# oxylusengine/Oxylus

Hardware: AMD Instinct MI355X
Metric: meshlets/s culled (higher is better)
Workload: dtype f32; 1 GPU; configs[2]: 10M meshlets + 4096^2 prior-frame HiZ (13 mips, built from an 8192^2 depth): HiZ build + early/late occlusion cull + per-triangle cull + compaction into the indirect-draw buffers (unordered_output = 1: slots allocated by atomic_add as in the reference, lists compared sorted); meshlets_per_gpu=10000000, mesh_instances=10000, meshlets_per_mesh=1000, tris_per_meshlet=64, verts_per_meshlet=64, index_form=(id << 8) | corner (visbuffer.slang:9-14), inner_reps=48, small_triangle_cull=False, async_triangles=False, unordered_output=1

## Files before the change

include/oxcull_debug.h:

```cpp
#ifndef OXCULL_DEBUG_H
#define OXCULL_DEBUG_H
#include "oxcull.h"
#ifdef __cplusplus
extern "C" {
#endif

oxc_status oxc_stream_read_probe(oxc_ctx* ctx, const void* dptr, uint64_t bytes, void* hip_stream);

enum {
  OXC_K_PREPARE = 0,
  OXC_K_MESHES_SCAN = 1,
  OXC_K_MESHES_EXPAND = 2,
  OXC_K_MESHLETS_TEST = 3,
  OXC_K_MESHLETS_EMIT = 4,
  OXC_K_TRIANGLES_TEST = 5,
  OXC_K_TRIANGLES_EMIT = 6,
  OXC_K_HIZ = 7,
  OXC_K_MESHLETS_TEST_LATE = 8,
  OXC_K_MESHLETS_EMIT_LATE = 9,
  OXC_K_TRIANGLES_TEST_LATE = 10,
  OXC_K_TRIANGLES_EMIT_LATE = 11,
  OXC_K_DRAW_VISBUFFER = 12,
  OXC_K_MESHLET_BOUNDS = 13,
  OXC_K_MULTIVIEW_SETUP = 14,
  OXC_K_VSM_UPDATE = 15,
  OXC_K_COUNT = 16
};
typedef struct oxc_kernel_times {
  double total_ms[16];
  uint32_t launches[16];
  double empty_pair_ms;
} oxc_kernel_times;
oxc_status oxc_profile_begin(oxc_ctx* ctx);
oxc_status oxc_profile_end(oxc_ctx* ctx, oxc_kernel_times* out);

oxc_status oxc_debug_decode_bounds(oxc_ctx* ctx, const void* bounds_dptr, uint32_t n, float* out10_dptr,
                                   void* hip_stream);

oxc_status oxc_debug_project_aabb(oxc_ctx* ctx, const float* mvp16_host, float near_clip, const void* boxes6_dptr, uint32_t n, float* out7_dptr,
                                  void* hip_stream);

oxc_status oxc_debug_read_u32(oxc_ctx* ctx, const void* dptr, uint32_t n, uint32_t* host_out, void* hip_stream);
uint32_t oxc_debug_shared_tests_mode(const oxc_ctx* ctx);
uint32_t oxc_debug_tri_loads_mode(const oxc_ctx* ctx);

enum { OXC_TUNE_ASYNC_MTEST_BLOCKS_PER_CU = 0, OXC_TUNE_ASYNC_TRI_BLOCKS_PER_CU = 1, OXC_TUNE_RASTER_BIG_CAPACITY = 2,
       OXC_TUNE_TRI_BLOCKS_PER_CU = 3 ,
       OXC_TUNE_TRI_LOADS = 7 ,
       OXC_TUNE_MV_EXPAND_ASYNC = 5 ,
       OXC_TUNE_VSM_DRAW_STATS = 8 ,
       OXC_TUNE_VSM_DRAW_CAPACITY = 9 ,
       OXC_TUNE_VSM_RESOLVE_STATS = 10 ,
       OXC_TUNE_CONTACT_SHADOWS_STATS = 11 ,
       OXC_TUNE_AMBIENT_OCCLUSION_STATS = 12  };
oxc_status oxc_debug_set_tuning(oxc_ctx* ctx, uint32_t knob, uint32_t value);

oxc_status oxc_debug_count_occlusion_candidates(oxc_ctx* ctx, void* counters_dptr);

oxc_status oxc_debug_raster_stats(oxc_ctx* ctx, uint32_t* host_out4, void* hip_stream);

oxc_status oxc_debug_vsm_draw_stats(oxc_ctx* ctx, uint32_t* host_out8, void* hip_stream);

oxc_status oxc_debug_vsm_resolve_stats(oxc_ctx* ctx, uint32_t* host_out8, void* hip_stream);

oxc_status oxc_debug_contact_shadows_stats(oxc_ctx* ctx, uint32_t* host_out12, void* hip_stream);

oxc_status oxc_debug_ambient_occlusion_stats(oxc_ctx* ctx, uint32_t* host_out15, void* hip_stream);

#ifdef __cplusplus
}
#endif
#endif
```

oxylus_amd/csrc/oxcull_abi.cpp:

```cpp
#include <hip/hip_runtime.h>

#include <algorithm>
#include <cmath>
#include <cstdio>
#include <cstdlib>
#include <dlfcn.h>
#include <cstring>
#include <new>
#include <string>
#include <vector>

#include "oxcull.h"
#include "oxcull_debug.h"
#include "oxcull_kernels.hpp"
#include "oxcull_types.hpp"

using namespace oxc;

namespace {
constexpr uint32_t kSlots = 8192;
constexpr uint32_t kMaxPackedInstances = 1u << 24;

inline uint32_t cdiv(uint32_t a, uint32_t b) { return (a + b - 1) / b; }
inline uint64_t align_up(uint64_t v, uint64_t a) { return (v + a - 1) / a * a; }
}

struct oxc_ctx {
  int device = 0;
  uint32_t num_cus = 256;
  std::string last_error;
  struct Lane {
    void* arena = nullptr;
    uint64_t arena_bytes = 0;
    uint32_t cap_mesh_instances = 0, cap_meshlets = 0;
    InstCache* cache = nullptr;
    InstCache* cache_alt = nullptr;
    InstCache* view_cache = nullptr;
    uint32_t cap_views = 0;
    uint32_t* mesh_counts = nullptr;
    uint32_t* mesh_offsets = nullptr;
    uint64_t* bits = nullptr;
    uint32_t* m_chunk_counts = nullptr;
    uint32_t* m_supers = nullptr;
    uint32_t* m_tickets = nullptr;
    uint32_t* m_supers_late = nullptr;
    uint32_t* m_tickets_late = nullptr;
    uint64_t* camera_test_bits = nullptr;
    uint2* step_info = nullptr;
    uint64_t* tri_masks = nullptr;
    uint32_t* t_chunk_counts = nullptr;
    uint32_t* t_supers = nullptr;
    uint32_t* t_supers_alt = nullptr;
  };
  Lane lane[kMaxBatch];
  BatchElem* batch_dev = nullptr;
  void* mv_arena = nullptr;
  uint64_t mv_arena_bytes = 0;
  float* bounds_scratch = nullptr;
  uint32_t bounds_scratch_cap = 0;
  void* raster_scratch = nullptr;
  uint32_t raster_capacity = 0;
  uint32_t raster_capacity_request = 0;
  void* raster_rows = nullptr;
  uint32_t raster_rows_cap = 0;
  void* vsm_scratch = nullptr;
  uint64_t vsm_scratch_bytes = 0;
  void* vsm_draw_scratch = nullptr;
  uint64_t vsm_draw_scratch_bytes = 0;
  uint32_t vsm_draw_capacity = 0;
  uint32_t vsm_draw_capacity_request = 0;
  bool vsm_draw_stats = false;
  uint32_t* vsm_resolve_stats = nullptr;
  bool vsm_resolve_stats_on = false;
  uint32_t* contact_shadows_stats = nullptr;
  bool contact_shadows_stats_on = false;
  uint32_t* ambient_occlusion_stats = nullptr;
  bool ambient_occlusion_stats_on = false;
  void* comm = nullptr;
  uint32_t comm_rank = 0, comm_world = 0;
  uint32_t* slots = nullptr;
  uint32_t slot_cursor = 0;
  uint32_t seed_cursor = 0;
  uint32_t* sink = nullptr;
  std::vector<uint32_t> seeded_total = std::vector<uint32_t>(kSlots, 0u);
  hipStream_t last_stream = nullptr;
  bool has_last_stream = false;
  hipEvent_t order_event = nullptr;
  hipStream_t side = nullptr;
  hipEvent_t fork_event = nullptr;
  hipStream_t mv_side = nullptr;
  hipEvent_t mv_fork = nullptr, mv_join = nullptr;
  uint32_t tri_loads = 0;
  uint32_t mv_expand_async = 4;
  struct TriPending {
    hipEvent_t done = nullptr;
    bool valid = false;
    bool late = false;
    const uint32_t* vis = nullptr;
    const void* visible = nullptr;
    unsigned long long capture_id = 0;
  };
  static constexpr uint32_t kTriRing = 4;
  TriPending tri[kTriRing];
  struct SharedTests {
    bool valid = false;
    uint32_t N = 0, n_host = 0, M = 0, flags = 0, mask_bits = 0;
    const void *meshlet_instances = nullptr, *mask = nullptr, *meshes = nullptr, *transforms = nullptr, *mesh_instances = nullptr, *vis = nullptr;
    oxc_cull_camera camera = {};
    uint64_t armed_for_call = ~0ull;
    unsigned long long capture_id = 0;
    uint32_t* late_slot = nullptr;
    uint32_t* late_t_supers = nullptr;
    InstCache* rows = nullptr;
    bool same_inputs(const SharedTests& o) const {
      return N == o.N && n_host == o.n_host && M == o.M && flags == o.flags && mask_bits == o.mask_bits && meshlet_instances == o.meshlet_instances && mask == o.mask && meshes == o.meshes &&
             transforms == o.transforms && mesh_instances == o.mesh_instances && vis == o.vis && std::memcmp(&camera, &o.camera, sizeof camera) == 0;
    }
  };
  SharedTests shared;
  uint32_t last_share_mode = 0;
  uint32_t last_tri_loads = 0;
  uint64_t call_seq = 0;
  uint32_t async_mtest_per_cu = kAsyncMeshletBlocksPerCU, async_tri_per_cu = kAsyncTriangleBlocksPerCU;
  uint32_t tri_blocks_per_cu = kTriangleBlocksPerCU;
  uint32_t* dbg_occlusion = nullptr;
  bool profiling = false;
  struct Rec {
    int id;
    hipEvent_t a, b;
  };
  std::vector<Rec> recs;
};

namespace {

oxc_status fail(oxc_ctx* ctx, oxc_status st, const char* what, hipError_t e = hipSuccess) {
  if (ctx) {
    ctx->last_error = what;
    if (e != hipSuccess) {
      ctx->last_error += ": ";
      ctx->last_error += hipGetErrorString(e);
    }
  }
  return st;
}

#define OXC_ORDER(ctx, stream)                                            \
  do {                                                                    \
    oxc_status _o = order_stream(ctx, static_cast<hipStream_t>(stream)); \
    if (_o != OXC_OK) return _o;                                          \
  } while (0)

#define OXC_HIP(ctx, expr)                                        \
  do {                                                            \
    hipError_t _e = (expr);                                       \
    if (_e != hipSuccess) return fail(ctx, OXC_HIP_ERROR, #expr, _e); \
  } while (0)

bool stream_is_capturing(hipStream_t s);
unsigned long long stream_capture_id(hipStream_t s);

oxc_status order_stream(oxc_ctx* ctx, hipStream_t s) {
  if (ctx->has_last_stream && ctx->last_stream != s && !stream_is_capturing(s) && !stream_is_capturing(ctx->last_stream)) {
    if (!ctx->order_event) OXC_HIP(ctx, hipEventCreateWithFlags(&ctx->order_event, hipEventDisableTiming));
    if (hipEventRecord(ctx->order_event, ctx->last_stream) == hipSuccess)
      OXC_HIP(ctx, hipStreamWaitEvent(s, ctx->order_event, 0));
    else
      (void)hipGetLastError();
  }
  ctx->last_stream = s;
  ctx->has_last_stream = true;
  return OXC_OK;
}

unsigned long long stream_capture_id(hipStream_t s) {
  hipStreamCaptureStatus st = hipStreamCaptureStatusNone;
  unsigned long long id = 0;
  if (hipStreamGetCaptureInfo(s, &st, &id) != hipSuccess) {
    (void)hipGetLastError();
    return 0;
  }
  return st == hipStreamCaptureStatusNone ? 0ull : (id ? id : ~0ull);
}

bool stream_is_capturing(hipStream_t s) {
  hipStreamCaptureStatus st = hipStreamCaptureStatusNone;
  if (hipStreamIsCapturing(s, &st) != hipSuccess) {
    (void)hipGetLastError();
    return false;
  }
  return st != hipStreamCaptureStatusNone;
}

oxc_status ensure_capacity(oxc_ctx* ctx, uint32_t mesh_instances, uint32_t meshlets, uint32_t views = 0, uint32_t lane_index = 0, hipStream_t s = nullptr) {
  oxc_ctx::Lane* L = &ctx->lane[lane_index];
  if (mesh_instances <= L->cap_mesh_instances && meshlets <= L->cap_meshlets && views <= L->cap_views && L->arena) return OXC_OK;
  if (stream_is_capturing(s))
    return fail(ctx, OXC_INVALID_ARG, "scratch memory must grow but the stream is being captured: call oxc_reserve (or one un-captured call of this size) first");
  const uint32_t Vw = std::max(views, L->cap_views);
  uint32_t M = std::max(std::max(mesh_instances, L->cap_mesh_instances), 1u);
  uint32_t N = std::max(std::max(meshlets, L->cap_meshlets), 1u);
  const uint32_t m_chunks = cdiv(N, 64u), t_chunks = cdiv(N, kTriChunk);
  uint64_t off = 0;
  auto carve = [&](uint64_t bytes) {
    uint64_t o = off;
    off = align_up(off + bytes, 256);
    return o;
  };
  const uint64_t o_cache = carve((uint64_t)M * sizeof(InstCache));
  const uint64_t o_cache_alt = carve((uint64_t)M * sizeof(InstCache));
  const uint64_t o_vcache = carve((uint64_t)M * Vw * sizeof(InstCache) + 64);
  const uint64_t o_counts = carve((uint64_t)M * 4);
  const uint64_t o_offsets = carve((uint64_t)M * 4);
  const uint64_t o_bits = carve((uint64_t)cdiv(N, 64) * 8);
  const uint64_t o_mcc = carve((uint64_t)m_chunks * 4);
  const uint64_t o_msup = carve((uint64_t)cdiv(m_chunks, kChunksPerSuper) * 4 * kSuperStride);
  const uint64_t o_mtick = carve((uint64_t)kTicketCounters * 4 * kSuperStride);
  const uint64_t o_msup_late = carve((uint64_t)cdiv(m_chunks, kChunksPerSuper) * 4 * kSuperStride);
  const uint64_t o_mtick_late = carve((uint64_t)kTicketCounters * 4 * kSuperStride);
  const uint64_t o_fb = carve((uint64_t)cdiv(N, 64) * 8);
  const uint64_t o_si = carve((uint64_t)m_chunks * 8);
  const uint64_t o_tm = carve((uint64_t)N * 16);
  const uint64_t o_tcc = carve((uint64_t)t_chunks * 4);
  const uint64_t o_tsup = carve((uint64_t)cdiv(t_chunks, kChunksPerSuper) * 4 * kSuperStride);
  const uint64_t o_tsup_alt = carve((uint64_t)cdiv(t_chunks, kChunksPerSuper) * 4 * kSuperStride);
  OXC_HIP(ctx, hipDeviceSynchronize());
  for (auto& tp : ctx->tri) tp.valid = false;
  if (lane_index == 0) ctx->shared.valid = false;
  if (L->arena) OXC_HIP(ctx, hipFree(L->arena));
  L->arena = nullptr;
  hipError_t e = hipMalloc(&L->arena, off);
  if (e != hipSuccess) {
    L->cap_mesh_instances = L->cap_meshlets = 0;
    return fail(ctx, OXC_OUT_OF_MEMORY, "hipMalloc(scratch arena)", e);
  }
  L->arena_bytes = off;
  char* b = static_cast<char*>(L->arena);
  L->cache = reinterpret_cast<InstCache*>(b + o_cache);
  L->cache_alt = reinterpret_cast<InstCache*>(b + o_cache_alt);
  L->view_cache = reinterpret_cast<InstCache*>(b + o_vcache);
  L->cap_views = Vw;
  L->mesh_counts = reinterpret_cast<uint32_t*>(b + o_counts);
  L->mesh_offsets = reinterpret_cast<uint32_t*>(b + o_offsets);
  L->bits = reinterpret_cast<uint64_t*>(b + o_bits);
  L->m_chunk_counts = reinterpret_cast<uint32_t*>(b + o_mcc);
  L->m_supers = reinterpret_cast<uint32_t*>(b + o_msup);
  L->m_tickets = reinterpret_cast<uint32_t*>(b + o_mtick);
  L->m_supers_late = reinterpret_cast<uint32_t*>(b + o_msup_late);
  L->m_tickets_late = reinterpret_cast<uint32_t*>(b + o_mtick_late);
  L->camera_test_bits = reinterpret_cast<uint64_t*>(b + o_fb);
  L->step_info = reinterpret_cast<uint2*>(b + o_si);
  L->tri_masks = reinterpret_cast<uint64_t*>(b + o_tm);
  L->t_chunk_counts = reinterpret_cast<uint32_t*>(b + o_tcc);
  L->t_supers = reinterpret_cast<uint32_t*>(b + o_tsup);
  L->t_supers_alt = reinterpret_cast<uint32_t*>(b + o_tsup_alt);
  L->cap_mesh_instances = M;
  L->cap_meshlets = N;
  return OXC_OK;
}

uint32_t* next_slot(oxc_ctx* ctx) {
  uint32_t* s = ctx->slots + (size_t)(ctx->slot_cursor % (kSlots / 2)) * SLOT_U32S;
  ctx->slot_cursor++;
  return s;
}
uint32_t* next_seed_slot(oxc_ctx* ctx) {
  uint32_t* s = ctx->slots + (size_t)(kSlots / 2 + ctx->seed_cursor % (kSlots / 2)) * SLOT_U32S;
  ctx->seed_cursor++;
  return s;
}

template <class Pred>
oxc_status wait_triangles(oxc_ctx* ctx, hipStream_t s, Pred needed, bool retire = false) {
  const unsigned long long cid = stream_capture_id(s);
  for (auto& tp : ctx->tri) {
    if (!tp.valid) continue;
    if (tp.capture_id != cid) {
      if (cid == 0 && !(ctx->side && stream_capture_id(ctx->side) == tp.capture_id)) tp.valid = false;
      continue;
    }
    if (!needed(tp)) continue;
    OXC_HIP(ctx, hipStreamWaitEvent(s, tp.done, 0));
    if (retire) tp.valid = false;
  }
  return OXC_OK;
}
oxc_status join_triangles(oxc_ctx* ctx, hipStream_t s) {
  return wait_triangles(ctx, s, [](const oxc_ctx::TriPending&) { return true; }, true);
}
#define OXC_JOIN(ctx, stream)                                               \
  do {                                                                      \
    oxc_status _j = join_triangles(ctx, static_cast<hipStream_t>(stream));  \
    if (_j != OXC_OK) return _j;                                            \
  } while (0)

struct KernelTimer {
  oxc_ctx* ctx;
  hipStream_t s;
  oxc_ctx::Rec r;
  bool on;
  KernelTimer(oxc_ctx* c, int id, hipStream_t st) : ctx(c), s(st), on(c->profiling) {
    if (!on) return;
    r.id = id;
    if (hipEventCreate(&r.a) != hipSuccess || hipEventCreate(&r.b) != hipSuccess) {
      on = false;
      return;
    }
    (void)hipEventRecord(r.a, s);
  }
  ~KernelTimer() {
    if (!on) return;
    (void)hipEventRecord(r.b, s);
    ctx->recs.push_back(r);
  }
};

bool image_ok(const oxc_image& im) { return im.dptr && im.width && im.height && im.levels >= 1 && im.levels <= 13; }

}

struct CallInfo {
  uint32_t stages, M, N, views;
  bool do_meshes, do_meshlets, do_tris, occl, late;
};

static oxc_status check_call(oxc_ctx* ctx, const oxc_prepared_frame* f, const oxc_cull_geometry_context* c, CallInfo& ci) {
  if (!f || !c || c->struct_size != sizeof(oxc_cull_geometry_context)) return fail(ctx, OXC_INVALID_ARG, "cull_geometry: bad frame/context struct");
  const uint32_t stages = c->stages ? c->stages : (uint32_t)OXC_STAGE_ALL;
  const uint32_t M = f->mesh_instance_count, N = f->max_meshlet_instance_count;
  const bool do_meshes = c->init_cull_meshes && (stages & OXC_STAGE_MESHES);
  const bool do_meshlets = (stages & OXC_STAGE_MESHLETS) != 0;
  const bool do_tris = (stages & OXC_STAGE_TRIANGLES) != 0;
  if (c->cull_camera.mesh_instance_count != M) return fail(ctx, OXC_INVALID_ARG, "cull_geometry: cull_camera.mesh_instance_count != frame.mesh_instance_count");
  if (M && (!f->meshes_buffer.dptr || !f->transforms_world_buffer.dptr || !f->mesh_instances_buffer.dptr))
    return fail(ctx, OXC_INVALID_ARG, "cull_geometry: meshes/transforms/mesh_instances buffer missing");
  if (f->mesh_instances_buffer.bytes < (uint64_t)M * sizeof(GpuMeshInstance)) return fail(ctx, OXC_INVALID_ARG, "cull_geometry: mesh_instances_buffer too small");
  if (N && (!f->meshlet_instances_buffer.dptr || f->meshlet_instances_buffer.bytes < (uint64_t)N * 8))
    return fail(ctx, OXC_INVALID_ARG, "cull_geometry: meshlet_instances_buffer missing or < 8*N bytes");
  if (do_meshlets && N && (!f->visible_meshlet_instances_indices_buffer.dptr || f->visible_meshlet_instances_indices_buffer.bytes < (uint64_t)N * 4))
    return fail(ctx, OXC_INVALID_ARG, "cull_geometry: visible_meshlet_instances_indices_buffer missing or < 4*N bytes");
  if (do_tris && N) {
    if (c->wide_triangle_index > 2u) return fail(ctx, OXC_INVALID_ARG, "cull_geometry: wide_triangle_index must be 0, 1 or 2");
    const uint64_t tris_per_meshlet = c->wide_triangle_index ? 128u : 64u, index_bytes = c->wide_triangle_index == 2u ? 8u : 4u;
    if (!f->reordered_indices_buffer.dptr || f->reordered_indices_buffer.bytes < (uint64_t)N * tris_per_meshlet * 3 * index_bytes)
      return fail(ctx, OXC_INVALID_ARG, "cull_geometry: reordered_indices_buffer missing or < N*64*3*4 bytes (N*128*3*4 with wide_triangle_index = 1, N*128*3*8 with 2)");
    if (c->wide_triangle_index != 2u && N > (c->wide_triangle_index ? kMaxPackedInstances / 2 : kMaxPackedInstances))
      return fail(ctx, OXC_INVALID_ARG, "cull_geometry: too many meshlet instances for the packed index (2^24, visbuffer.slang:9-14; 2^23 with wide_triangle_index = 1; pairs, wide_triangle_index = 2, have no limit)");
  }
  const bool occl = (c->cull_flags & OXC_CULL_TEST_OCCLUSION) != 0;
  const bool late = (c->cull_flags & OXC_CULL_LATE_PASS) != 0;
  if (c->use_hiz && do_meshlets) {
    if (!image_ok(c->hiz_attachment)) return fail(ctx, OXC_INVALID_ARG, "cull_geometry: use_hiz without a hiz_attachment");
    if (occl && N && (!f->meshlet_instance_visibility_mask_buffer.dptr || f->meshlet_instance_visibility_mask_buffer.bytes < (uint64_t)cdiv(N, 32u) * 4u))
      return fail(ctx, OXC_INVALID_ARG, "cull_geometry: visibility mask buffer missing or < ceil(N/32)*4 bytes");
  }
  if (c->small_triangle_cull > 1u) return fail(ctx, OXC_INVALID_ARG, "cull_geometry: small_triangle_cull must be 0 or 1");
  if (c->share_pass_tests > 1u || c->unordered_output > 1u) return fail(ctx, OXC_INVALID_ARG, "cull_geometry: share_pass_tests must be 0 or 1, unordered_output 0 or 1");
  if (c->implicit_meshlet_instances > 1u || c->_reserved1 != 0u) return fail(ctx, OXC_INVALID_ARG, "cull_geometry: implicit_meshlet_instances must be 0 or 1, _reserved1 0");
  if (c->meshlet_instance_runs_buffer.dptr && c->meshlet_instance_runs_buffer.bytes < (uint64_t)M * 8u)
    return fail(ctx, OXC_INVALID_ARG, "cull_geometry: meshlet_instance_runs_buffer < 8 bytes per mesh instance");
  if (c->implicit_meshlet_instances && (!c->meshlet_instance_runs_buffer.dptr || do_tris || !do_meshes))
    return fail(ctx, OXC_INVALID_ARG, "cull_geometry: implicit_meshlet_instances needs meshlet_instance_runs_buffer, cull_meshes in the call and no triangle stage");
  const uint32_t views = c->use_hpb ? c->vsm_clipmap_count : 0u;
  if (c->use_hpb && do_meshlets) {
    if (c->use_hiz) return fail(ctx, OXC_INVALID_ARG, "cull_geometry: use_hiz and use_hpb are exclusive (CullGeometry.cpp:129,199)");
    if (views == 0 || views > 16) return fail(ctx, OXC_INVALID_ARG, "cull_geometry: vsm_clipmap_count must be 1..16");
    if (!c->vsm_clipmaps_buffer.dptr || c->vsm_clipmaps_buffer.bytes < (uint64_t)views * sizeof(oxc_virtual_clipmap) || !c->vsm_clipmap_dirty_flags_buffer.dptr ||
        c->vsm_clipmap_dirty_flags_buffer.bytes < (uint64_t)views * 4u)
      return fail(ctx, OXC_INVALID_ARG, "cull_geometry: use_hpb needs vsm_clipmaps_buffer (76 B per clipmap) / vsm_clipmap_dirty_flags_buffer (4 B per clipmap)");
    const oxc_image_array_u8& h = c->hpb_attachment;
    if (!h.dptr || !h.width || !h.height || h.layers < views || h.levels < 1 || h.levels > 13)
      return fail(ctx, OXC_INVALID_ARG, "cull_geometry: use_hpb without a valid hpb_attachment (layers >= clipmaps, 1..13 levels)");
    for (uint32_t k = 0; k < h.levels; k++) {
      const uint64_t mw = std::max(1u, h.width >> k), mh = std::max(1u, h.height >> k);
      if (h.level_offset[k] + (uint64_t)h.layers * mw * mh > 0xFFFFFFFFull)
        return fail(ctx, OXC_INVALID_ARG, "cull_geometry: hpb_attachment larger than 4 GiB (the reference's is 64 x 64 pages x 10 clipmaps, Shadowmaps.cpp:84-98)");
    }
  }
  if (!c->init_cull_meshes && (!c->visibility_buffer.dptr || !c->cull_meshlets_cmd_buffer.dptr))
    return fail(ctx, OXC_INVALID_ARG, "cull_geometry: init_cull_meshes=false needs the visibility/cull_meshlets_cmd buffers of the sequence");


  ci.stages = stages;
  ci.M = M;
  ci.N = N;
  ci.views = views;
  ci.do_meshes = do_meshes;
  ci.do_meshlets = do_meshlets;
  ci.do_tris = do_tris;
  ci.occl = occl;
  ci.late = late;
  return OXC_OK;
}

extern "C" {

uint32_t oxc_abi_version(void) { return OXC_ABI_VERSION; }

oxc_status oxc_create(int device, oxc_ctx** out) {
  if (!out) return OXC_INVALID_ARG;
  *out = nullptr;
  oxc_ctx* ctx = new (std::nothrow) oxc_ctx();
  if (!ctx) return OXC_OUT_OF_MEMORY;
  ctx->device = device;
  hipError_t e = hipSetDevice(device);
  if (e != hipSuccess) {
    delete ctx;
    return OXC_HIP_ERROR;
  }
  hipDeviceProp_t prop;
  if (hipGetDeviceProperties(&prop, device) == hipSuccess && prop.multiProcessorCount > 0)
    ctx->num_cus = (uint32_t)prop.multiProcessorCount;
  e = hipMalloc(reinterpret_cast<void**>(&ctx->slots), (size_t)kSlots * SLOT_U32S * 4 + 256);
  if (e != hipSuccess) {
    delete ctx;
    return OXC_OUT_OF_MEMORY;
  }
  (void)hipMemset(ctx->slots, 0, (size_t)kSlots * SLOT_U32S * 4 + 256);
  (void)hipDeviceSynchronize();
  ctx->sink = ctx->slots + (size_t)kSlots * SLOT_U32S;
  *out = ctx;
  return OXC_OK;
}

void oxc_destroy(oxc_ctx* ctx) {
  if (!ctx) return;
  (void)hipSetDevice(ctx->device);
  (void)hipDeviceSynchronize();
  for (auto& ln : ctx->lane)
    if (ln.arena) (void)hipFree(ln.arena);
  if (ctx->batch_dev) (void)hipFree(ctx->batch_dev);
  if (ctx->mv_arena) (void)hipFree(ctx->mv_arena);
  if (ctx->bounds_scratch) (void)hipFree(ctx->bounds_scratch);
  if (ctx->raster_scratch) (void)hipFree(ctx->raster_scratch);
  if (ctx->raster_rows) (void)hipFree(ctx->raster_rows);
  if (ctx->vsm_scratch) (void)hipFree(ctx->vsm_scratch);
  if (ctx->vsm_draw_scratch) (void)hipFree(ctx->vsm_draw_scratch);
  if (ctx->vsm_resolve_stats) (void)hipFree(ctx->vsm_resolve_stats);
  if (ctx->contact_shadows_stats) (void)hipFree(ctx->contact_shadows_stats);
  if (ctx->ambient_occlusion_stats) (void)hipFree(ctx->ambient_occlusion_stats);
  if (ctx->comm) (void)oxc_comm_destroy(ctx);
  if (ctx->slots) (void)hipFree(ctx->slots);
  if (ctx->order_event) (void)hipEventDestroy(ctx->order_event);
  if (ctx->fork_event) (void)hipEventDestroy(ctx->fork_event);
  if (ctx->mv_side) (void)hipStreamDestroy(ctx->mv_side);
  if (ctx->mv_fork) (void)hipEventDestroy(ctx->mv_fork);
  if (ctx->mv_join) (void)hipEventDestroy(ctx->mv_join);
  for (auto& tp : ctx->tri)
    if (tp.done) (void)hipEventDestroy(tp.done);
  if (ctx->side) (void)hipStreamDestroy(ctx->side);
  delete ctx;
}

const char* oxc_last_error(const oxc_ctx* ctx) { return ctx ? ctx->last_error.c_str() : "null context"; }

oxc_status oxc_reserve(oxc_ctx* ctx, uint32_t max_mesh_instances, uint32_t max_meshlet_instances) {
  if (!ctx) return OXC_INVALID_ARG;
  OXC_HIP(ctx, hipSetDevice(ctx->device));
  return ensure_capacity(ctx, max_mesh_instances, max_meshlet_instances);
}

oxc_status oxc_generate_hiz(oxc_ctx* ctx, const oxc_main_geometry_context* c, void* hip_stream) {
  if (!ctx) return OXC_INVALID_ARG;
  if (!c || c->struct_size != sizeof(oxc_main_geometry_context)) return fail(ctx, OXC_INVALID_ARG, "generate_hiz: bad context struct");
  const oxc_image& d = c->depth_attachment;
  const oxc_image& h = c->hiz_attachment;
  if (!d.dptr || !d.width || !d.height) return fail(ctx, OXC_INVALID_ARG, "generate_hiz: depth_attachment missing");
  if (!image_ok(h)) return fail(ctx, OXC_INVALID_ARG, "generate_hiz: hiz_attachment missing or levels not in 1..13");
  if (h.width > 4096 || h.height > 4096) return fail(ctx, OXC_INVALID_ARG, "generate_hiz: hiz extent > 4096 (13 mips) unsupported");
  HizArgs a;
  a.depth = reinterpret_cast<const float*>(static_cast<const char*>(d.dptr) + d.level_offset[0]);
  a.hiz = static_cast<float*>(h.dptr);
  a.dw = d.width;
  a.dh = d.height;
  a.w = h.width;
  a.h = h.height;
  a.levels = std::min(h.levels, 13u);
  for (uint32_t k = 0; k < 13; k++) {
    if (k < a.levels && (h.level_offset[k] & 3u)) return fail(ctx, OXC_INVALID_ARG, "generate_hiz: level offset not 4-byte aligned");
    a.level_off[k] = k < a.levels ? (uint32_t)(h.level_offset[k] / 4) : 0u;
  }
  const bool tiled = (a.w % 64 == 0) && (a.h % 64 == 0);
  if (!tiled && (uint64_t)a.w * a.h > 4096) return fail(ctx, OXC_INVALID_ARG, "generate_hiz: extent must be a multiple of 64 or <= 4096 texels");
  if (tiled && (h.level_offset[0] & 15u)) return fail(ctx, OXC_INVALID_ARG, "generate_hiz: mip 0 must be 16-byte aligned");
  OXC_HIP(ctx, hipSetDevice(ctx->device));
  OXC_ORDER(ctx, hip_stream);
  {
    KernelTimer t(ctx, OXC_K_HIZ, static_cast<hipStream_t>(hip_stream));
    launch_hiz(a, ctx->num_cus, static_cast<hipStream_t>(hip_stream));
  }
  OXC_HIP(ctx, hipGetLastError());
  return OXC_OK;
}

oxc_status oxc_seed_meshlet_instances(oxc_ctx* ctx, oxc_cull_geometry_context* c, uint32_t total, void* hip_stream) {
  if (!ctx) return OXC_INVALID_ARG;
  if (!c || c->struct_size != sizeof(oxc_cull_geometry_context)) return fail(ctx, OXC_INVALID_ARG, "seed: bad context struct");
  OXC_HIP(ctx, hipSetDevice(ctx->device));
  OXC_ORDER(ctx, hip_stream);
  uint32_t* slot = next_seed_slot(ctx);
  ctx->shared.valid = false;
  ctx->seeded_total[(slot - ctx->slots) / SLOT_U32S] = total;
  launch_seed_slot(slot, total, static_cast<hipStream_t>(hip_stream));
  OXC_HIP(ctx, hipGetLastError());
  c->visibility_buffer = {slot + SLOT_VIS, 12};
  c->cull_meshlets_cmd_buffer = {slot + SLOT_MESHLETS_CMD, 12};
  return OXC_OK;
}

oxc_status oxc_cull_geometry(oxc_ctx* ctx, const oxc_prepared_frame* f, oxc_cull_geometry_context* c, void* hip_stream) {
  if (!ctx) return OXC_INVALID_ARG;
  CallInfo ci;
  {
    oxc_status vst = check_call(ctx, f, c, ci);
    if (vst != OXC_OK) return vst;
  }
  const uint32_t M = ci.M, N = ci.N, views = ci.views;
  const bool do_meshes = ci.do_meshes, do_meshlets = ci.do_meshlets, do_tris = ci.do_tris, occl = ci.occl, late = ci.late;
  if (c->implicit_meshlet_instances)
    return fail(ctx, OXC_INVALID_ARG, "cull_geometry: implicit_meshlet_instances is accepted by oxc_cull_geometry_batch's multi-view path only (this call's meshlet test reads the records)");
  OXC_HIP(ctx, hipSetDevice(ctx->device));
  hipStream_t s = static_cast<hipStream_t>(hip_stream);
  oxc_status st = ensure_capacity(ctx, M, N, views, 0, s);
  if (st != OXC_OK) return st;
  OXC_ORDER(ctx, hip_stream);
  ctx->last_share_mode = 0;
  ctx->last_tri_loads = 0;
  if (do_meshes) ctx->shared.valid = false;

  oxc_ctx::Lane& L0 = ctx->lane[0];
  const uint64_t call_no = ctx->call_seq++;
  const bool async = c->async_triangles != 0 && do_tris;
  InstCache* cache = (call_no & 1u) ? L0.cache_alt : L0.cache;
  uint32_t* t_supers = (call_no & 1u) ? L0.t_supers_alt : L0.t_supers;
  oxc_ctx::TriPending& my_tri = ctx->tri[call_no % oxc_ctx::kTriRing];
  my_tri.valid = false;
  if (!async || do_meshes) {
    OXC_JOIN(ctx, s);
  } else if (call_no >= 2) {
    const oxc_ctx::TriPending* old = &ctx->tri[(call_no - 2) % oxc_ctx::kTriRing];
    oxc_status wst = wait_triangles(ctx, s, [old](const oxc_ctx::TriPending& tp) { return &tp == old; });
    if (wst != OXC_OK) return wst;
  }
  const uint32_t mtest_limit = (c->async_triangles && ctx->async_mtest_per_cu) ? ctx->async_mtest_per_cu * ctx->num_cus : 0u;
  const uint32_t tri_grid_cap = (async && ctx->async_tri_per_cu) ? ctx->async_tri_per_cu * ctx->num_cus : ctx->num_cus * ctx->tri_blocks_per_cu;
  const void* const visible_buf = f->visible_meshlet_instances_indices_buffer.dptr;
  auto wait_for_visible_list = [&](const uint32_t* vis_now) -> oxc_status {
    return wait_triangles(ctx, s, [&](const oxc_ctx::TriPending& tp) { return !(late && !tp.late && tp.vis == vis_now && tp.visible == visible_buf); });
  };

  uint32_t* slot = c->init_cull_meshes ? next_slot(ctx) : nullptr;
  uint32_t* vis;
  uint32_t* meshlets_cmd;
  uint32_t n_host = 0;
  if (!c->init_cull_meshes) {
    const uint32_t* v = static_cast<const uint32_t*>(c->visibility_buffer.dptr);
    if (v >= ctx->slots && v < ctx->slots + (size_t)kSlots * SLOT_U32S && ((v - ctx->slots) % SLOT_U32S) == SLOT_VIS)
      n_host = ctx->seeded_total[(v - ctx->slots) / SLOT_U32S];
    if (n_host > N) n_host = 0;
  }
  if (c->init_cull_meshes) {
    vis = slot + SLOT_VIS;
    meshlets_cmd = slot + SLOT_MESHLETS_CMD;
    c->visibility_buffer = {vis, 12};
    c->cull_meshlets_cmd_buffer = {meshlets_cmd, 12};
  } else {
    vis = static_cast<uint32_t*>(c->visibility_buffer.dptr);
    meshlets_cmd = static_cast<uint32_t*>(c->cull_meshlets_cmd_buffer.dptr);
  }
  uint32_t share_mode = 0;
  bool armed_late = false, arm_late = false;
  uint32_t* m_supers = L0.m_supers;
  uint32_t* m_tickets = L0.m_tickets;
  const uint32_t mask_bits = (uint32_t)std::min<uint64_t>(f->meshlet_instance_visibility_mask_buffer.bytes / 4u * 32u, 0xFFFFFFFEull);
  const bool unord_tris = c->unordered_output != 0u && do_tris;
  const bool unord_meshlets = do_meshlets && !c->use_hpb && !c->use_hiz && c->unordered_output != 0u;
  if (c->use_hiz && occl && c->share_pass_tests && do_meshlets && !unord_meshlets) {
    oxc_ctx::SharedTests now;
    now.N = N;
    now.n_host = n_host;
    now.M = M;
    now.flags = c->cull_flags & ~(uint32_t)OXC_CULL_LATE_PASS;
    now.mask_bits = mask_bits;
    now.meshlet_instances = f->meshlet_instances_buffer.dptr;
    now.mask = f->meshlet_instance_visibility_mask_buffer.dptr;
    now.meshes = f->meshes_buffer.dptr;
    now.transforms = f->transforms_world_buffer.dptr;
    now.mesh_instances = f->mesh_instances_buffer.dptr;
    now.vis = vis;
    now.camera = c->cull_camera;
    if (!late) {
      share_mode = 1u;
      arm_late = c->async_triangles == 0;
      now.valid = true;
      if (arm_late) {
        now.armed_for_call = call_no + 1;
        now.capture_id = stream_capture_id(s);
        now.late_slot = next_slot(ctx);
        now.late_t_supers = (call_no & 1u) ? L0.t_supers : L0.t_supers_alt;
        now.rows = cache;
      }
      ctx->shared = now;
    } else if (!do_meshes && !c->init_cull_meshes && ctx->shared.valid && ctx->shared.same_inputs(now)) {
      share_mode = 2u;
      if (ctx->shared.armed_for_call == call_no && c->async_triangles == 0 && ctx->shared.capture_id == stream_capture_id(s)) {
        armed_late = true;
        slot = ctx->shared.late_slot;
        t_supers = ctx->shared.late_t_supers;
        cache = ctx->shared.rows;
        m_supers = L0.m_supers_late;
        m_tickets = L0.m_tickets_late;
      }
      ctx->shared.valid = false;
    }
  } else if (c->use_hiz && do_meshlets && !late) {
    ctx->shared.valid = false;
  }
  if (!armed_late && ctx->shared.armed_for_call <= call_no) ctx->shared.armed_for_call = ~0ull;
  if (!slot) slot = next_slot(ctx);
  uint32_t* tri_cmd = slot + SLOT_TRI_CMD;
  uint32_t* draw_cmd = slot + SLOT_DRAW_CMD;
  c->cull_triangles_cmd_buffer = {tri_cmd, 12};
  c->draw_geometry_cmd_buffer = {draw_cmd, 20};

  const uint32_t max_grid = ctx->num_cus * 8;
  const uint32_t m_chunks = cdiv(std::max(N, 1u), kMeshletChunk), t_chunks = cdiv(std::max(N, 1u), kTriChunk);

  PrepareArgs pa;
  pa.meshes = static_cast<const GpuMesh*>(f->meshes_buffer.dptr);
  pa.transforms = static_cast<const float*>(f->transforms_world_buffer.dptr);
  pa.mesh_instances = static_cast<GpuMeshInstance*>(f->mesh_instances_buffer.dptr);
  pa.cache = cache;
  pa.mesh_counts = ctx->lane[0].mesh_counts;
  pa.slot = slot;
  pa.vis = vis;
  pa.meshlets_cmd = meshlets_cmd;
  pa.supers_meshlets = m_supers;
  pa.supers_tris = t_supers;
  pa.tickets = m_tickets;
  pa.slot_late = arm_late ? ctx->shared.late_slot : nullptr;
  pa.supers_meshlets_late = arm_late ? L0.m_supers_late : nullptr;
  pa.supers_tris_late = arm_late ? ctx->shared.late_t_supers : nullptr;
  pa.tickets_late = arm_late ? L0.m_tickets_late : nullptr;
  pa.n_supers_meshlets = cdiv(cdiv(std::max(N, 1u), 64u), kChunksPerSuper);
  pa.n_supers_tris = cdiv(t_chunks, kChunksPerSuper);
  pa.mesh_instance_count = M;
  pa.cull_flags = c->cull_flags;
  pa.do_cull_meshes = do_meshes ? 1u : 0u;
  pa.init_vis = c->init_cull_meshes ? 1u : 0u;
  pa.seed_total = 0;
  pa.cam = c->cull_camera;
  pa.clipmaps = static_cast<const oxc_virtual_clipmap*>(c->vsm_clipmaps_buffer.dptr);
  pa.view_cache = ctx->lane[0].view_cache;
  const uint32_t prep_threads = std::max(std::max(M * 8u, pa.n_supers_tris), 1u);
  if (!armed_late) {
    KernelTimer t(ctx, OXC_K_PREPARE, s);
    launch_prepare(pa, std::min(cdiv(prep_threads, 256), max_grid), (c->use_hpb && do_meshlets) ? views : 0u, s);
  }
  if (do_meshes) {
    {
      KernelTimer t(ctx, OXC_K_MESHES_SCAN, s);
      launch_scan_mesh_counts(ctx->lane[0].mesh_counts, ctx->lane[0].mesh_offsets, M, N, vis, meshlets_cmd, s);
    }
    KernelTimer t(ctx, OXC_K_MESHES_EXPAND, s);
    launch_expand(ctx->lane[0].mesh_counts, ctx->lane[0].mesh_offsets, M, N, f->meshlet_instances_buffer.dptr, std::max(std::min(cdiv(M, 4), max_grid), 1u), s);
  }

  if (do_meshlets && c->use_hpb) {
    HpbTestArgs ha;
    std::memset(&ha, 0, sizeof ha);
    ha.cache = cache;
    ha.view_cache = ctx->lane[0].view_cache;
    ha.meshlet_instances = static_cast<const GpuMeshletInstance*>(f->meshlet_instances_buffer.dptr);
    ha.vis = vis;
    ha.bits = ctx->lane[0].bits;
    ha.chunk_counts = ctx->lane[0].m_chunk_counts;
    ha.supers = ctx->lane[0].m_supers;
    ha.tickets = ctx->lane[0].m_tickets;
    ha.clipmaps = static_cast<const oxc_virtual_clipmap*>(c->vsm_clipmaps_buffer.dptr);
    ha.dirty = static_cast<const uint32_t*>(c->vsm_clipmap_dirty_flags_buffer.dptr);
    ha.clipmap_count = views;
    ha.mesh_instance_count = M;
    ha.n_cap = N;
    const oxc_image_array_u8& h = c->hpb_attachment;
    ha.hpb_data = static_cast<const uint8_t*>(h.dptr);
    ha.hpb_w = h.width;
    ha.hpb_h = h.height;
    ha.hpb_layers = h.layers;
    ha.hpb_levels = h.levels;
    for (uint32_t k = 0; k < h.levels && k < 13; k++) ha.hpb_level_off[k] = (uint32_t)h.level_offset[k];
    std::memcpy(ha.light_dir, c->cull_camera.position, 12);
    {
      KernelTimer t(ctx, OXC_K_MESHLETS_TEST, s);
      launch_hpb_test(ha, std::min(m_chunks, max_grid), s);
    }
    MeshletEmitArgs ea;
    ea.n_host = 0;
    ea.n_cap = N;
    ea.count_meshlets = 64u * kGroupsPerWave;
    ea.bits = ctx->lane[0].bits;
    ea.chunk_counts = ctx->lane[0].m_chunk_counts;
    ea.supers = ctx->lane[0].m_supers;
    ea.vis = vis;
    ea.tri_cmd = tri_cmd;
    ea.out = static_cast<uint32_t*>(f->visible_meshlet_instances_indices_buffer.dptr);
    {
      oxc_status wst = wait_for_visible_list(vis);
      if (wst != OXC_OK) return wst;
    }
    KernelTimer t(ctx, OXC_K_MESHLETS_EMIT, s);
    launch_meshlets_emit(ea, false, false, std::min(cdiv(std::max(N, 1u), kMeshletSpan), max_grid), s);
  } else if (do_meshlets) {
    MeshletTestArgs ta;
    std::memset(&ta, 0, sizeof ta);
    ta.n_host = n_host;
    ta.n_cap = N;
    ta.mask_bits = mask_bits;
    ta.cache = cache;
    ta.meshlet_instances = static_cast<const GpuMeshletInstance*>(f->meshlet_instances_buffer.dptr);
    ta.vis = vis;
    ta.mask = static_cast<uint32_t*>(f->meshlet_instance_visibility_mask_buffer.dptr);
    ta.bits = ctx->lane[0].bits;
    ta.chunk_counts = ctx->lane[0].m_chunk_counts;
    ta.supers = m_supers;
    if (c->use_hiz) {
      ta.tickets = m_tickets;
      const oxc_image& h = c->hiz_attachment;
      ta.hiz_data = static_cast<const float*>(h.dptr);
      ta.hiz_w = h.width;
      ta.hiz_h = h.height;
      ta.hiz_levels = h.levels;
      for (uint32_t k = 0; k < h.levels && k < 13; k++) ta.hiz_level_off[k] = (uint32_t)(h.level_offset[k] / 4);
      uint32_t first = h.levels, used = 0;
      while (first > 0) {
        const uint64_t n = (uint64_t)std::max(1u, h.width >> (first - 1)) * std::max(1u, h.height >> (first - 1));
        if (used + n > kHizLdsTexels) break;
        used += (uint32_t)n;
        first--;
      }
      ta.hiz_lds_first = first;
      uint32_t off = 0;
      for (uint32_t k = first; k < h.levels; k++) {
        ta.hiz_lds_off[k] = off;
        off += std::max(1u, h.width >> k) * std::max(1u, h.height >> k);
      }
    }
    ta.near_clip = c->cull_camera.near_clip;
    std::memcpy(ta.cam_pos, c->cull_camera.position, 12);
    ta.dbg_occlusion = ctx->dbg_occlusion;
    if (share_mode) {
      ta.share = share_mode;
      ta.camera_test_bits = ctx->lane[0].camera_test_bits;
      ta.step_info = ctx->lane[0].step_info;
    }
    ctx->last_share_mode = armed_late ? 3u : ta.share;
    if (unord_meshlets) {
      ta.out = static_cast<uint32_t*>(f->visible_meshlet_instances_indices_buffer.dptr);
      ta.count_a = tri_cmd;
      oxc_status wst = wait_for_visible_list(vis);
      if (wst != OXC_OK) return wst;
      KernelTimer t(ctx, late ? OXC_K_MESHLETS_TEST_LATE : OXC_K_MESHLETS_TEST, s);
      launch_meshlets_test(ta, c->use_hiz != 0, occl, late, std::min(m_chunks, max_grid), ctx->num_cus, mtest_limit, s);
    } else {
      {
        KernelTimer t(ctx, late ? OXC_K_MESHLETS_TEST_LATE : OXC_K_MESHLETS_TEST, s);
        launch_meshlets_test(ta, c->use_hiz != 0, occl, late, std::min(m_chunks, max_grid), ctx->num_cus, mtest_limit, s);
      }
      MeshletEmitArgs ea;
      ea.n_host = n_host;
      ea.n_cap = N;
      ea.count_meshlets = c->use_hiz ? 64u * kHizGroupsPerWave : 64u * kPlainGroups;
      ea.bits = ctx->lane[0].bits;
      ea.chunk_counts = ctx->lane[0].m_chunk_counts;
      ea.supers = m_supers;
      ea.vis = vis;
      ea.tri_cmd = tri_cmd;
      ea.out = static_cast<uint32_t*>(f->visible_meshlet_instances_indices_buffer.dptr);
      {
        oxc_status wst = wait_for_visible_list(vis);
        if (wst != OXC_OK) return wst;
      }
      KernelTimer t(ctx, late ? OXC_K_MESHLETS_EMIT_LATE : OXC_K_MESHLETS_EMIT, s);
      launch_meshlets_emit(ea, c->use_hiz != 0, late, std::min(cdiv(std::max(N, 1u), kMeshletSpan), max_grid), s);
    }
  }

  if (do_tris) {
    hipStream_t ts = s;
    if (async) {
      if (!ctx->side) OXC_HIP(ctx, hipStreamCreateWithFlags(&ctx->side, hipStreamNonBlocking));
      if (!ctx->fork_event) OXC_HIP(ctx, hipEventCreateWithFlags(&ctx->fork_event, hipEventDisableTiming));
      OXC_HIP(ctx, hipEventRecord(ctx->fork_event, s));
      OXC_HIP(ctx, hipStreamWaitEvent(ctx->side, ctx->fork_event, 0));
      ts = ctx->side;
    }
    TriTestArgs tt;
    tt.cache = cache;
    tt.meshlet_instances = static_cast<const GpuMeshletInstance*>(f->meshlet_instances_buffer.dptr);
    tt.visible = static_cast<const uint32_t*>(f->visible_meshlet_instances_indices_buffer.dptr);
    tt.vis = vis;
    tt.tri_cmd = tri_cmd;
    tt.tri_masks = ctx->lane[0].tri_masks;
    tt.chunk_counts = ctx->lane[0].t_chunk_counts;
    tt.supers = t_supers;
    tt.resolution[0] = c->cull_camera.resolution[0];
    tt.resolution[1] = c->cull_camera.resolution[1];
    tt.draw_cmd = draw_cmd;
    tt.out = static_cast<uint32_t*>(f->reordered_indices_buffer.dptr);
    tt.ticket = t_supers;
    tt.ticket_count = std::max(pa.n_supers_tris, 1u);
    const uint64_t mesh_records = f->meshes_buffer.bytes / sizeof(GpuMesh);
    const bool cached_loads = ctx->tri_loads == 2u || (ctx->tri_loads == 0u && mesh_records != 0u && (uint64_t)M >= 4u * mesh_records);
    ctx->last_tri_loads = (cached_loads && !c->small_triangle_cull) ? 2u : 1u;
    if (unord_tris) {
      KernelTimer t(ctx, late ? OXC_K_TRIANGLES_TEST_LATE : OXC_K_TRIANGLES_TEST, ts);
      const bool default_cap = !(async && ctx->async_tri_per_cu) && ctx->tri_blocks_per_cu == kTriangleBlocksPerCU;
      launch_tris_fused(tt, late, c->wide_triangle_index, c->small_triangle_cull != 0, cached_loads, std::min(cdiv(std::max(N, 1u), kFusedTriSpan), tri_grid_cap),
                        default_cap ? ctx->num_cus : 0u, ts);
    } else {
    {
      KernelTimer t(ctx, late ? OXC_K_TRIANGLES_TEST_LATE : OXC_K_TRIANGLES_TEST, ts);
      const bool default_cap = !(async && ctx->async_tri_per_cu) && ctx->tri_blocks_per_cu == kTriangleBlocksPerCU;
      launch_tris_test(tt, late, c->wide_triangle_index != 0, c->small_triangle_cull != 0, cached_loads, std::min(t_chunks, (default_cap && !c->wide_triangle_index) ? ctx->num_cus * 32u : tri_grid_cap), ts);
    }
    TriEmitArgs te;
    te.tri_masks = ctx->lane[0].tri_masks;
    te.visible = tt.visible;
    te.vis = vis;
    te.tri_cmd = tri_cmd;
    te.chunk_counts = ctx->lane[0].t_chunk_counts;
    te.supers = t_supers;
    te.draw_cmd = draw_cmd;
    te.out = static_cast<uint32_t*>(f->reordered_indices_buffer.dptr);
    {
      KernelTimer t(ctx, late ? OXC_K_TRIANGLES_EMIT_LATE : OXC_K_TRIANGLES_EMIT, ts);
      launch_tris_emit(te, late, c->wide_triangle_index, std::min(cdiv(std::max(N, 1u), kTriSpan), tri_grid_cap), ts);
    }
    }
    if (async) {
      if (!my_tri.done) OXC_HIP(ctx, hipEventCreateWithFlags(&my_tri.done, hipEventDisableTiming));
      OXC_HIP(ctx, hipEventRecord(my_tri.done, ts));
      my_tri.valid = true;
      my_tri.late = late;
      my_tri.vis = vis;
      my_tri.visible = visible_buf;
      my_tri.capture_id = stream_capture_id(s);
    }
  }
  OXC_HIP(ctx, hipGetLastError());
  return OXC_OK;
}

oxc_status oxc_join_triangles(oxc_ctx* ctx, void* hip_stream) {
  if (!ctx) return OXC_INVALID_ARG;
  OXC_HIP(ctx, hipSetDevice(ctx->device));
  OXC_ORDER(ctx, hip_stream);
  return join_triangles(ctx, static_cast<hipStream_t>(hip_stream));
}

oxc_status oxc_cull_geometry_batch(oxc_ctx* ctx, uint32_t count, const oxc_prepared_frame* frames, oxc_cull_geometry_context* contexts,
                                   void* hip_stream) {
  if (!ctx) return OXC_INVALID_ARG;
  if (count == 0) return OXC_OK;
  if (!frames || !contexts) return fail(ctx, OXC_INVALID_ARG, "cull_geometry_batch: null frames/contexts");
  CallInfo ci[kMaxBatch];
  bool fusable = count > 1 && count <= kMaxBatch;
  for (uint32_t e = 0; fusable && e < count; e++) {
    oxc_status vst = check_call(ctx, &frames[e], &contexts[e], ci[e]);
    if (vst != OXC_OK) return vst;
    const oxc_cull_geometry_context& c = contexts[e];
    fusable = !c.use_hiz && !c.use_hpb && !c.wide_triangle_index && !c.small_triangle_cull && !ci[e].late && ci[e].stages == ci[0].stages && ci[e].do_meshes == ci[0].do_meshes &&
              (c.init_cull_meshes != 0) == (contexts[0].init_cull_meshes != 0);
  }
  if (!fusable) {
    for (uint32_t e = 0; e < count; e++) {
      oxc_status st = oxc_cull_geometry(ctx, &frames[e], &contexts[e], hip_stream);
      if (st != OXC_OK) return st;
    }
    return OXC_OK;
  }
  bool multiview = ci[0].do_meshes && ci[0].do_meshlets && ci[0].M > 0;
  bool same_pos = true;
  for (uint32_t e = 1; multiview && e < count; e++) {
    multiview = ci[e].M == ci[0].M && frames[e].meshes_buffer.dptr == frames[0].meshes_buffer.dptr &&
                frames[e].transforms_world_buffer.dptr == frames[0].transforms_world_buffer.dptr && contexts[e].cull_flags == contexts[0].cull_flags;
    same_pos = same_pos && std::memcmp(contexts[e].cull_camera.position, contexts[0].cull_camera.position, 12) == 0;
  }
  uint32_t n_implicit = 0;
  for (uint32_t e = 0; e < count; e++) n_implicit += contexts[e].implicit_meshlet_instances ? 1u : 0u;
  if (n_implicit && (n_implicit != count || !multiview || ci[0].do_tris))
    return fail(ctx, OXC_INVALID_ARG, "cull_geometry_batch: implicit_meshlet_instances must be set on every element of a multi-view batch (same scene, cull_meshes in every element, no triangle stage)");
  const bool implicit_lists = n_implicit != 0;
  OXC_HIP(ctx, hipSetDevice(ctx->device));
  ctx->shared.valid = false;
  for (uint32_t e = 0; e < count; e++) {
    oxc_status st = ensure_capacity(ctx, ci[e].M, ci[e].N, 0, e, static_cast<hipStream_t>(hip_stream));
    if (st != OXC_OK) return st;
  }
  OXC_ORDER(ctx, hip_stream);
  OXC_JOIN(ctx, hip_stream);
  if (!ctx->batch_dev) {
    if (stream_is_capturing(static_cast<hipStream_t>(hip_stream)))
      return fail(ctx, OXC_INVALID_ARG, "cull_geometry_batch: the first batched call allocates its argument block; make one un-captured call first");
    hipError_t e = hipMalloc(reinterpret_cast<void**>(&ctx->batch_dev), sizeof(BatchElem) * kMaxBatch);
    if (e != hipSuccess) return fail(ctx, OXC_OUT_OF_MEMORY, "hipMalloc(batch argument block)", e);
    OXC_HIP(ctx, hipMemset(ctx->batch_dev, 0, sizeof(BatchElem) * kMaxBatch));
    OXC_HIP(ctx, hipDeviceSynchronize());
  }
// ... 1067 lines not shown
Rccl* rccl() {
  static Rccl r;
  static bool tried = false;
  if (!tried) {
    tried = true;
    r.lib = dlopen("librccl.so", RTLD_NOW | RTLD_GLOBAL);
    if (!r.lib) r.lib = dlopen("librccl.so.1", RTLD_NOW | RTLD_GLOBAL);
    if (r.lib) {
      r.GetUniqueId = reinterpret_cast<decltype(r.GetUniqueId)>(dlsym(r.lib, "ncclGetUniqueId"));
      r.CommInitRank = reinterpret_cast<decltype(r.CommInitRank)>(dlsym(r.lib, "ncclCommInitRank"));
      r.CommDestroy = reinterpret_cast<decltype(r.CommDestroy)>(dlsym(r.lib, "ncclCommDestroy"));
      r.AllGather = reinterpret_cast<decltype(r.AllGather)>(dlsym(r.lib, "ncclAllGather"));
      r.Broadcast = reinterpret_cast<decltype(r.Broadcast)>(dlsym(r.lib, "ncclBroadcast"));
      r.GetErrorString = reinterpret_cast<decltype(r.GetErrorString)>(dlsym(r.lib, "ncclGetErrorString"));
    }
  }
  return (r.lib && r.GetUniqueId && r.CommInitRank && r.CommDestroy && r.AllGather && r.Broadcast) ? &r : nullptr;
}
oxc_status rccl_fail(oxc_ctx* ctx, const char* what, int code) {
  static thread_local std::string msg;
  Rccl* r = rccl();
  msg = std::string(what) + ": " + ((r && r->GetErrorString) ? r->GetErrorString(code) : "RCCL error");
  ctx->last_error = msg;
  return OXC_RCCL_ERROR;
}
constexpr int kNcclUint8 = 1, kNcclUint32 = 3;
}

oxc_status oxc_comm_unique_id(oxc_ctx* ctx, void* id128_host_out) {
  if (!ctx) return OXC_INVALID_ARG;
  if (!id128_host_out) return fail(ctx, OXC_INVALID_ARG, "comm_unique_id: null output");
  Rccl* r = rccl();
  if (!r) return fail(ctx, OXC_RCCL_ERROR, "librccl.so could not be loaded (needed only for the multi-GPU exchange)");
  OXC_HIP(ctx, hipSetDevice(ctx->device));
  int rc = r->GetUniqueId(id128_host_out);
  return rc == 0 ? OXC_OK : rccl_fail(ctx, "ncclGetUniqueId", rc);
}

oxc_status oxc_comm_init(oxc_ctx* ctx, const void* id128_host, uint32_t rank, uint32_t world) {
  if (!ctx) return OXC_INVALID_ARG;
  if (!id128_host || world == 0 || rank >= world) return fail(ctx, OXC_INVALID_ARG, "comm_init: null id or rank >= world");
  if (ctx->comm) return fail(ctx, OXC_INVALID_ARG, "comm_init: the context already has a communicator");
  Rccl* r = rccl();
  if (!r) return fail(ctx, OXC_RCCL_ERROR, "librccl.so could not be loaded (needed only for the multi-GPU exchange)");
  OXC_HIP(ctx, hipSetDevice(ctx->device));
  OxcRcclId id;
  std::memcpy(&id, id128_host, sizeof id);
  int rc = r->CommInitRank(&ctx->comm, (int)world, id, (int)rank);
  if (rc != 0) {
    ctx->comm = nullptr;
    return rccl_fail(ctx, "ncclCommInitRank", rc);
  }
  ctx->comm_rank = rank;
  ctx->comm_world = world;
  return OXC_OK;
}

oxc_status oxc_comm_destroy(oxc_ctx* ctx) {
  if (!ctx) return OXC_INVALID_ARG;
  if (ctx->comm) {
    Rccl* r = rccl();
    if (r) (void)r->CommDestroy(ctx->comm);
    ctx->comm = nullptr;
    ctx->comm_world = 0;
  }
  return OXC_OK;
}

oxc_status oxc_pack_counters(oxc_ctx* ctx, const oxc_cull_geometry_context* c, void* counts4_dptr, void* hip_stream) {
  if (!ctx) return OXC_INVALID_ARG;
  if (!c || c->struct_size != sizeof(oxc_cull_geometry_context) || !counts4_dptr) return fail(ctx, OXC_INVALID_ARG, "pack_counters: bad context struct or null output");
  if (!c->visibility_buffer.dptr || !c->cull_triangles_cmd_buffer.dptr || !c->draw_geometry_cmd_buffer.dptr)
    return fail(ctx, OXC_INVALID_ARG, "pack_counters: the context has no counter buffers yet (no cull_geometry call has filled them in)");
  OXC_HIP(ctx, hipSetDevice(ctx->device));
  OXC_ORDER(ctx, hip_stream);
  OXC_JOIN(ctx, hip_stream);
  launch_pack_counters(static_cast<const uint32_t*>(c->visibility_buffer.dptr), static_cast<const uint32_t*>(c->cull_triangles_cmd_buffer.dptr),
                       static_cast<const uint32_t*>(c->draw_geometry_cmd_buffer.dptr), static_cast<uint32_t*>(counts4_dptr), static_cast<hipStream_t>(hip_stream));
  OXC_HIP(ctx, hipGetLastError());
  return OXC_OK;
}

oxc_status oxc_pack_counters_batch(oxc_ctx* ctx, uint32_t count, const oxc_cull_geometry_context* cs, void* counts4_dptr, void* hip_stream) {
  if (!ctx) return OXC_INVALID_ARG;
  if (!cs || !counts4_dptr || count == 0 || count > kMaxBatch) return fail(ctx, OXC_INVALID_ARG, "pack_counters_batch: 1..16 contexts and an output buffer");
  PackBlob b;
  std::memset(&b, 0, sizeof b);
  b.count = count;
  for (uint32_t e = 0; e < count; e++) {
    if (cs[e].struct_size != sizeof(oxc_cull_geometry_context)) return fail(ctx, OXC_INVALID_ARG, "pack_counters_batch: bad context struct");
    if (!cs[e].visibility_buffer.dptr || !cs[e].cull_triangles_cmd_buffer.dptr || !cs[e].draw_geometry_cmd_buffer.dptr)
      return fail(ctx, OXC_INVALID_ARG, "pack_counters_batch: a context has no counter buffers yet (no cull_geometry call has filled them in)");
    b.vis[e] = static_cast<const uint32_t*>(cs[e].visibility_buffer.dptr);
    b.tri_cmd[e] = static_cast<const uint32_t*>(cs[e].cull_triangles_cmd_buffer.dptr);
    b.draw_cmd[e] = static_cast<const uint32_t*>(cs[e].draw_geometry_cmd_buffer.dptr);
  }
  OXC_HIP(ctx, hipSetDevice(ctx->device));
  OXC_ORDER(ctx, hip_stream);
  OXC_JOIN(ctx, hip_stream);
  launch_pack_counters_batch(b, static_cast<uint32_t*>(counts4_dptr), static_cast<hipStream_t>(hip_stream));
  OXC_HIP(ctx, hipGetLastError());
  return OXC_OK;
}

oxc_status oxc_exchange_counts(oxc_ctx* ctx, const void* counts4_dptr, void* all_counts_dptr, void* hip_stream) {
  if (!ctx) return OXC_INVALID_ARG;
  if (!ctx->comm) return fail(ctx, OXC_INVALID_ARG, "exchange_counts: oxc_comm_init has not been called");
  if (!counts4_dptr || !all_counts_dptr) return fail(ctx, OXC_INVALID_ARG, "exchange_counts: null buffer");
  OXC_HIP(ctx, hipSetDevice(ctx->device));
  OXC_ORDER(ctx, hip_stream);
  int rc = rccl()->AllGather(counts4_dptr, all_counts_dptr, 4, kNcclUint32, ctx->comm, static_cast<hipStream_t>(hip_stream));
  return rc == 0 ? OXC_OK : rccl_fail(ctx, "ncclAllGather", rc);
}

oxc_status oxc_broadcast_hiz(oxc_ctx* ctx, const oxc_image* hiz, uint64_t total_bytes, uint32_t root, void* hip_stream) {
  if (!ctx) return OXC_INVALID_ARG;
  if (!ctx->comm) return fail(ctx, OXC_INVALID_ARG, "broadcast_hiz: oxc_comm_init has not been called");
  if (!hiz || !hiz->dptr || total_bytes == 0 || root >= ctx->comm_world) return fail(ctx, OXC_INVALID_ARG, "broadcast_hiz: null image, zero size or bad root");
  OXC_HIP(ctx, hipSetDevice(ctx->device));
  OXC_ORDER(ctx, hip_stream);
  int rc = rccl()->Broadcast(hiz->dptr, hiz->dptr, (size_t)total_bytes, kNcclUint8, (int)root, ctx->comm, static_cast<hipStream_t>(hip_stream));
  return rc == 0 ? OXC_OK : rccl_fail(ctx, "ncclBroadcast", rc);
}

oxc_status oxc_broadcast_hiz_levels(oxc_ctx* ctx, const oxc_image* hiz, uint32_t first_level, uint64_t total_bytes, uint32_t root, void* hip_stream) {
  if (!ctx) return OXC_INVALID_ARG;
  if (!ctx->comm) return fail(ctx, OXC_INVALID_ARG, "broadcast_hiz_levels: oxc_comm_init has not been called");
  if (!hiz || !hiz->dptr || first_level >= hiz->levels || hiz->levels > 13 || root >= ctx->comm_world) return fail(ctx, OXC_INVALID_ARG, "broadcast_hiz_levels: null image, bad level or bad root");
  const uint64_t begin = hiz->level_offset[first_level];
  if (total_bytes <= begin) return fail(ctx, OXC_INVALID_ARG, "broadcast_hiz_levels: total_bytes does not reach first_level");
  OXC_HIP(ctx, hipSetDevice(ctx->device));
  OXC_ORDER(ctx, hip_stream);
  char* p = static_cast<char*>(hiz->dptr) + begin;
  int rc = rccl()->Broadcast(p, p, (size_t)(total_bytes - begin), kNcclUint8, (int)root, ctx->comm, static_cast<hipStream_t>(hip_stream));
  return rc == 0 ? OXC_OK : rccl_fail(ctx, "ncclBroadcast", rc);
}

oxc_status oxc_debug_project_aabb(oxc_ctx* ctx, const float* mvp16_host, float near_clip, const void* boxes6_dptr, uint32_t n, float* out7_dptr, void* hip_stream) {
  if (!ctx) return OXC_INVALID_ARG;
  if (!mvp16_host || !boxes6_dptr || !out7_dptr) return fail(ctx, OXC_INVALID_ARG, "debug_project_aabb: null pointer");
  OXC_HIP(ctx, hipSetDevice(ctx->device));
  DebugProjectArgs a;
  std::memcpy(a.mvp, mvp16_host, 64);
  a.near_clip = near_clip;
  a.n = n;
  a.boxes6 = static_cast<const float*>(boxes6_dptr);
  a.out7 = out7_dptr;
  launch_debug_project_aabb(a, static_cast<hipStream_t>(hip_stream));
  OXC_HIP(ctx, hipGetLastError());
  return OXC_OK;
}

uint32_t oxc_debug_shared_tests_mode(const oxc_ctx* ctx) { return ctx ? ctx->last_share_mode : 0u; }
uint32_t oxc_debug_tri_loads_mode(const oxc_ctx* ctx) { return ctx ? ctx->last_tri_loads : 0u; }

oxc_status oxc_debug_set_tuning(oxc_ctx* ctx, uint32_t knob, uint32_t value) {
  if (!ctx) return OXC_INVALID_ARG;
  switch (knob) {
    case OXC_TUNE_ASYNC_MTEST_BLOCKS_PER_CU: ctx->async_mtest_per_cu = value; return OXC_OK;
    case OXC_TUNE_ASYNC_TRI_BLOCKS_PER_CU: ctx->async_tri_per_cu = value; return OXC_OK;
    case OXC_TUNE_TRI_BLOCKS_PER_CU:
      if (value == 0) return fail(ctx, OXC_INVALID_ARG, "set_tuning: the triangle grid needs at least one block per CU");
      ctx->tri_blocks_per_cu = value;
      return OXC_OK;
    case OXC_TUNE_MV_EXPAND_ASYNC: ctx->mv_expand_async = value; return OXC_OK;
    case OXC_TUNE_TRI_LOADS:
      if (value > 2u) return fail(ctx, OXC_INVALID_ARG, "set_tuning: OXC_TUNE_TRI_LOADS is 0 (by the scene), 1 (nt) or 2 (plain)");
      ctx->tri_loads = value;
      return OXC_OK;
    case OXC_TUNE_RASTER_BIG_CAPACITY:
      if (ctx->raster_scratch) return fail(ctx, OXC_INVALID_ARG, "set_tuning: the raster scratch is allocated by the first oxc_draw_visbuffer; set its capacity before");
      ctx->raster_capacity_request = value;
      return OXC_OK;
    case OXC_TUNE_VSM_DRAW_STATS: ctx->vsm_draw_stats = value != 0u; return OXC_OK;
    case OXC_TUNE_VSM_RESOLVE_STATS: ctx->vsm_resolve_stats_on = value != 0u; return OXC_OK;
    case OXC_TUNE_CONTACT_SHADOWS_STATS: ctx->contact_shadows_stats_on = value != 0u; return OXC_OK;
    case OXC_TUNE_AMBIENT_OCCLUSION_STATS: ctx->ambient_occlusion_stats_on = value != 0u; return OXC_OK;
    case OXC_TUNE_VSM_DRAW_CAPACITY:
      if (ctx->vsm_draw_scratch) return fail(ctx, OXC_INVALID_ARG, "set_tuning: the shadow draw's scratch is allocated by the first oxc_draw_physical_pages; set its capacity before");
      ctx->vsm_draw_capacity_request = value;
      return OXC_OK;
    default: return fail(ctx, OXC_INVALID_ARG, "set_tuning: unknown knob");
  }
}

oxc_status oxc_debug_count_occlusion_candidates(oxc_ctx* ctx, void* counters_dptr) {
  if (!ctx) return OXC_INVALID_ARG;
  ctx->dbg_occlusion = static_cast<uint32_t*>(counters_dptr);
  return OXC_OK;
}

oxc_status oxc_debug_read_u32(oxc_ctx* ctx, const void* dptr, uint32_t n, uint32_t* host_out, void* hip_stream) {
  if (!ctx) return OXC_INVALID_ARG;
  if (!dptr || !host_out) return fail(ctx, OXC_INVALID_ARG, "debug_read_u32: null pointer");
  OXC_HIP(ctx, hipSetDevice(ctx->device));
  hipStream_t s = static_cast<hipStream_t>(hip_stream);
  OXC_HIP(ctx, hipMemcpyAsync(host_out, dptr, (size_t)n * 4u, hipMemcpyDeviceToHost, s));
  OXC_HIP(ctx, hipStreamSynchronize(s));
  return OXC_OK;
}

oxc_status oxc_debug_raster_stats(oxc_ctx* ctx, uint32_t* host_out4, void* hip_stream) {
  if (!ctx) return OXC_INVALID_ARG;
  if (!host_out4) return fail(ctx, OXC_INVALID_ARG, "debug_raster_stats: null pointer");
  if (!ctx->raster_scratch) return fail(ctx, OXC_INVALID_ARG, "debug_raster_stats: no oxc_draw_visbuffer call on this context yet");
  OXC_HIP(ctx, hipSetDevice(ctx->device));
  OXC_ORDER(ctx, hip_stream);
  hipStream_t s = static_cast<hipStream_t>(hip_stream);
  std::vector<uint32_t> h(kRasterHeaderBytes / 4);
  OXC_HIP(ctx, hipMemcpyAsync(h.data(), ctx->raster_scratch, kRasterHeaderBytes, hipMemcpyDeviceToHost, s));
  OXC_HIP(ctx, hipStreamSynchronize(s));
  const uint32_t seg_cap = ctx->raster_capacity / kBigSegs;
  uint64_t big = 0;
  uint32_t overflowed = 0;
  for (uint32_t k = 0; k < kBigSegs; k++) {
    const uint32_t c = h[64 + k * kBigSegStride];
    big += c;
    overflowed += c > seg_cap ? 1u : 0u;
  }
  host_out4[0] = (uint32_t)std::min<uint64_t>(big, 0xFFFFFFFFull);
  host_out4[1] = h[0];
  host_out4[2] = h[32];
  host_out4[3] = overflowed;
  return OXC_OK;
}

oxc_status oxc_debug_vsm_draw_stats(oxc_ctx* ctx, uint32_t* host_out8, void* hip_stream) {
  if (!ctx) return OXC_INVALID_ARG;
  if (!host_out8) return fail(ctx, OXC_INVALID_ARG, "debug_vsm_draw_stats: null pointer");
  if (!ctx->vsm_draw_scratch) return fail(ctx, OXC_INVALID_ARG, "debug_vsm_draw_stats: no oxc_draw_physical_pages call on this context yet");
  OXC_HIP(ctx, hipSetDevice(ctx->device));
  OXC_ORDER(ctx, hip_stream);
  hipStream_t s = static_cast<hipStream_t>(hip_stream);
  std::vector<uint32_t> h(kVsmDrawHeaderBytes / 4);
  OXC_HIP(ctx, hipMemcpyAsync(h.data(), ctx->vsm_draw_scratch, kVsmDrawHeaderBytes, hipMemcpyDeviceToHost, s));
  OXC_HIP(ctx, hipStreamSynchronize(s));
  const uint32_t cap = ctx->vsm_draw_capacity;
  auto beyond = [](uint32_t count, uint32_t capacity) { return count > capacity ? count - capacity : 0u; };
  host_out8[0] = h[128];
  host_out8[1] = h[160];
  host_out8[2] = h[32];
  host_out8[3] = beyond(h[32], cap);
  host_out8[4] = h[64];
  host_out8[5] = beyond(h[64], cap * 2u);
  host_out8[6] = h[96];
  host_out8[7] = beyond(h[96], cap);
  return OXC_OK;
}

oxc_status oxc_debug_vsm_resolve_stats(oxc_ctx* ctx, uint32_t* host_out8, void* hip_stream) {
  if (!ctx) return OXC_INVALID_ARG;
  if (!host_out8) return fail(ctx, OXC_INVALID_ARG, "debug_vsm_resolve_stats: null pointer");
  if (!ctx->vsm_resolve_stats) return fail(ctx, OXC_INVALID_ARG, "debug_vsm_resolve_stats: no counting oxc_resolve_shadowmap call on this context yet");
  OXC_HIP(ctx, hipSetDevice(ctx->device));
  OXC_ORDER(ctx, hip_stream);
  hipStream_t s = static_cast<hipStream_t>(hip_stream);
  OXC_HIP(ctx, hipMemcpyAsync(host_out8, ctx->vsm_resolve_stats, 32, hipMemcpyDeviceToHost, s));
  OXC_HIP(ctx, hipStreamSynchronize(s));
  return OXC_OK;
}

oxc_status oxc_debug_contact_shadows_stats(oxc_ctx* ctx, uint32_t* host_out12, void* hip_stream) {
  if (!ctx) return OXC_INVALID_ARG;
  if (!host_out12) return fail(ctx, OXC_INVALID_ARG, "debug_contact_shadows_stats: null pointer");
  if (!ctx->contact_shadows_stats) return fail(ctx, OXC_INVALID_ARG, "debug_contact_shadows_stats: no counting oxc_contact_shadows call on this context yet");
  OXC_HIP(ctx, hipSetDevice(ctx->device));
  OXC_ORDER(ctx, hip_stream);
  hipStream_t s = static_cast<hipStream_t>(hip_stream);
  OXC_HIP(ctx, hipMemcpyAsync(host_out12, ctx->contact_shadows_stats, 48, hipMemcpyDeviceToHost, s));
  OXC_HIP(ctx, hipStreamSynchronize(s));
  return OXC_OK;
}

oxc_status oxc_debug_ambient_occlusion_stats(oxc_ctx* ctx, uint32_t* host_out15, void* hip_stream) {
  if (!ctx) return OXC_INVALID_ARG;
  if (!host_out15) return fail(ctx, OXC_INVALID_ARG, "debug_ambient_occlusion_stats: null pointer");
  if (!ctx->ambient_occlusion_stats) return fail(ctx, OXC_INVALID_ARG, "debug_ambient_occlusion_stats: no counting oxc_generate_ambient_occlusion call on this context yet");
  OXC_HIP(ctx, hipSetDevice(ctx->device));
  OXC_ORDER(ctx, hip_stream);
  hipStream_t s = static_cast<hipStream_t>(hip_stream);
  OXC_HIP(ctx, hipMemcpyAsync(host_out15, ctx->ambient_occlusion_stats, 60, hipMemcpyDeviceToHost, s));
  OXC_HIP(ctx, hipStreamSynchronize(s));
  return OXC_OK;
}

}
```

oxylus_amd/csrc/oxcull_device.hpp:

```cpp
#pragma once
#include <hip/hip_runtime.h>

#include <cstdint>

#pragma clang fp contract(off)

namespace oxc {

#define OXC_DEV __device__ __forceinline__

OXC_DEV float asf(uint32_t u) { return __builtin_bit_cast(float, u); }
OXC_DEV uint32_t asu(float f) { return __builtin_bit_cast(uint32_t, f); }
OXC_DEV int lane_id() { return (int)__builtin_amdgcn_mbcnt_hi(~0u, __builtin_amdgcn_mbcnt_lo(~0u, 0u)); }
OXC_DEV uint32_t readlane_u(uint32_t v, int l) { return (uint32_t)__builtin_amdgcn_readlane((int)v, l); }
OXC_DEV float readlane_f(uint32_t v, int l) { return asf(readlane_u(v, l)); }
OXC_DEV uint32_t readfirst_u(uint32_t v) { return (uint32_t)__builtin_amdgcn_readfirstlane((int)v); }
OXC_DEV float bperm_f(int src_lane, float v) {
  return asf((uint32_t)__builtin_amdgcn_ds_bpermute(src_lane << 2, (int)asu(v)));
}

template <typename T>
OXC_DEV T __attribute__((address_space(1))) * gptr(T* p) {
  return (T __attribute__((address_space(1)))*)p;
}
// ... 84 lines not shown
  }
  float t[6][4];
#pragma unroll
  for (int c = 0; c < 4; c++) {
    t[0][c] = r3[c] + r0[c];
    t[1][c] = r3[c] - r0[c];
    t[2][c] = r3[c] + r1[c];
    t[3][c] = r3[c] - r1[c];
    t[4][c] = r2[c];
    t[5][c] = r3[c] - r2[c];
  }
#pragma unroll
  for (int i = 0; i < 6; i++) {
    float l = len3(t[i][0], t[i][1], t[i][2]);
#pragma unroll
    for (int c = 0; c < 4; c++) pl[i * 4 + c] = t[i][c] / l;
  }
}

OXC_DEV bool test_frustum_planes(const float* pl2, const float* sg2, float cx, float cy, float cz, float ex, float ey, float ez) {
  const f2 hxy = f2{ex, ey} * splat(0.5f);
  const float hz = ez * 0.5f;
  bool inside = true;
#pragma unroll
  for (int p = 0; p < 3; p++) {
    const float* n = pl2 + p * 8;
    const float* sg = sg2 + p * 6;
    const f2 qx = splat(cx) + splat(hxy.x) * f2{sg[0], sg[1]};
    const f2 qy = splat(cy) + splat(hxy.y) * f2{sg[2], sg[3]};
    const f2 qz = splat(cz) + splat(hz) * f2{sg[4], sg[5]};
    const f2 d = (qx * f2{n[0], n[1]} + qy * f2{n[2], n[3]}) + qz * f2{n[4], n[5]};
    inside = inside & !(d.x <= -n[6]) & !(d.y <= -n[7]);
  }
  return inside;
}

OXC_DEV void frustum_plane_dots(const float* pl2, const float* sg2, float cx, float cy, float cz, float ex, float ey, float ez, f2* d ) {
  const f2 hxy = f2{ex, ey} * splat(0.5f);
  const float hz = ez * 0.5f;
#pragma unroll
  for (int p = 0; p < 3; p++) {
    const float* n = pl2 + p * 8;
    const float* sg = sg2 + p * 6;
    const f2 qx = splat(cx) + splat(hxy.x) * f2{sg[0], sg[1]};
    const f2 qy = splat(cy) + splat(hxy.y) * f2{sg[2], sg[3]};
    const f2 qz = splat(cz) + splat(hz) * f2{sg[4], sg[5]};
    d[p] = (qx * f2{n[0], n[1]} + qy * f2{n[2], n[3]}) + qz * f2{n[4], n[5]};
  }
}

OXC_DEV bool frustum_pair_inside(const float* n, const float* sg, float cx, float cy, float cz, float ex, float ey, float ez) {
  const f2 hxy = f2{ex, ey} * splat(0.5f);
  const float hz = ez * 0.5f;
  const f2 qx = splat(cx) + splat(hxy.x) * f2{sg[0], sg[1]};
  const f2 qy = splat(cy) + splat(hxy.y) * f2{sg[2], sg[3]};
  const f2 qz = splat(cz) + splat(hz) * f2{sg[4], sg[5]};
  const f2 d = (qx * f2{n[0], n[1]} + qy * f2{n[2], n[3]}) + qz * f2{n[4], n[5]};
  return !(d.x <= -n[6]) & !(d.y <= -n[7]);
}

OXC_DEV void normal_matrix(const float* w, float* nm) {
  float b[3][3];
#pragma unroll
  for (int j = 0; j < 3; j++)
#pragma unroll
    for (int k = 0; k < 3; k++) b[j][k] = OXC_M(w, k, j);
  const int a1[3] = {1, 2, 0}, a2[3] = {2, 0, 1};
#pragma unroll
  for (int k = 0; k < 3; k++) {
    const float* u = b[a1[k]];
    const float* v = b[a2[k]];
    nm[k * 3 + 0] = u[1] * v[2] - v[1] * u[2];
    nm[k * 3 + 1] = u[2] * v[0] - v[2] * u[0];
    nm[k * 3 + 2] = u[0] * v[1] - v[0] * u[1];
  }
}

struct ConeU {
  float nm[9];
  float w2[3][2];
  float wt2[2];
  float wr2[4];
  float scale_max;
};

OXC_DEV bool cone_visible(const ConeU& u, float camx, float camy, float camz, float cx, float cy, float cz, float ex, float ey, float ez,
                          float ax, float ay, float az, float cutoff) {
  const float* nm = u.nm;
  float nx = (nm[0] * ax + nm[3] * ay) + nm[6] * az;
  float ny = (nm[1] * ax + nm[4] * ay) + nm[7] * az;
  float nz = (nm[2] * ax + nm[5] * ay) + nm[8] * az;
  float l = len3(nx, ny, nz);
  float kx = nx / l, ky = ny / l, kz = nz / l;
  float wx = ((u.w2[0][0] * cx + u.w2[1][0] * cy) + u.w2[2][0] * cz) + u.wt2[0];
  float wy = ((u.w2[0][1] * cx + u.w2[1][1] * cy) + u.w2[2][1] * cz) + u.wt2[1];
  float wz = ((u.wr2[0] * cx + u.wr2[1] * cy) + u.wr2[2] * cz) + u.wr2[3];
  float radius = len3(ex * 0.5f, ey * 0.5f, ez * 0.5f) * u.scale_max;
  float dx = wx - camx, dy = wy - camy, dz = wz - camz;
  bool culled = dot3(dx, dy, dz, kx, ky, kz) >= cutoff * len3(dx, dy, dz) + radius;
  return cutoff >= 1.0f || !culled;
}

constexpr float kConeMargin = 1.6e-5f;
OXC_DEV int cone_visible_fast(const ConeU& u, float camx, float camy, float camz, float cx, float cy, float cz, float ex, float ey, float ez,
                              float ax, float ay, float az, float cutoff) {
  const float* nm = u.nm;
  const f2 nxy = (f2{nm[0], nm[1]} * splat(ax) + f2{nm[3], nm[4]} * splat(ay)) + f2{nm[6], nm[7]} * splat(az);
  const float nz = (nm[2] * ax + nm[5] * ay) + nm[8] * az;
  const f2 wxy = ((f2{u.w2[0][0], u.w2[0][1]} * splat(cx) + f2{u.w2[1][0], u.w2[1][1]} * splat(cy)) + f2{u.w2[2][0], u.w2[2][1]} * splat(cz)) +
                 f2{u.wt2[0], u.wt2[1]};
  const float wz = ((u.wr2[0] * cx + u.wr2[1] * cy) + u.wr2[2] * cz) + u.wr2[3];
  const f2 dxy = wxy - f2{camx, camy};
  const float dz = wz - camz;
  const f2 hxy = f2{ex, ey} * splat(0.5f);
  const float hz = ez * 0.5f;
  const f2 nn = nxy * nxy, dd = dxy * dxy, dn = dxy * nxy, hh = hxy * hxy;
  float inv_l = __builtin_amdgcn_rsqf((nn.x + nn.y) + nz * nz);
  float dlen = __builtin_amdgcn_sqrtf((dd.x + dd.y) + dz * dz);
  float radius = __builtin_amdgcn_sqrtf((hh.x + hh.y) + hz * hz) * u.scale_max;
  float L = ((dn.x + dn.y) + dz * nz) * inv_l;
  float R = cutoff * dlen + radius;
  float T = kConeMargin * (dlen + radius);
  float diff = L - R;
  if (diff > T) return 0;
  if (diff < -T) return 1;
  return 2;
}

struct HizView {
  const float* data;
  uint32_t width, height, levels;
  const float* lds;
  const uint32_t* lds_off;
  uint32_t lds_first;
  float inv_width, inv_height;
};
OXC_DEV float exact_reciprocal_or_zero(uint32_t d) { return (d != 0u && (d & (d - 1u)) == 0u) ? 1.0f / (float)d : 0.0f; }

OXC_DEV uint32_t mip_dim(uint32_t d, uint32_t mip) {
  uint32_t v = d >> mip;
  return v ? v : 1u;
}

OXC_DEV float min0_finite(float x) {
  float r;
  asm("v_min_f32 %0, 0, %1" : "=v"(r) : "v"(x));
  return r;
}
OXC_DEV float max0_finite(float x) {
  float r;
  asm("v_max_f32 %0, 0, %1" : "=v"(r) : "v"(x));
  return r;
}
template <bool TRY_AFFINE = false, bool NEED_Z = true>
OXC_DEV bool project_aabb(const float* mvp, float near_clip, float cx, float cy, float cz, float ex, float ey, float ez, float* out) {
  float SX[4], SY[4], SZ[4], P[8][4];
  float p0x = cx - ex * 0.5f, p0y = cy - ey * 0.5f, p0z = cz - ez * 0.5f;
  if (TRY_AFFINE && asu(OXC_M(mvp, 3, 0)) == 0u && asu(OXC_M(mvp, 3, 1)) == 0u && asu(OXC_M(mvp, 3, 2)) == 0u &&
      asu(OXC_M(mvp, 3, 3)) == 0x3F800000u) {
    float lo[3] = {0.f, 0.f, 0.f}, hi[3] = {0.f, 0.f, 0.f}, P0[3] = {0.f, 0.f, 0.f}, S[3][3] = {{0.f, 0.f, 0.f}, {0.f, 0.f, 0.f}, {0.f, 0.f, 0.f}};
    bool finite = true;
#pragma unroll
    for (int i = 0; i < (NEED_Z ? 3 : 2); i++) {
      S[i][0] = OXC_M(mvp, i, 0) * ex, S[i][1] = OXC_M(mvp, i, 1) * ey, S[i][2] = OXC_M(mvp, i, 2) * ez;
      P0[i] = ((OXC_M(mvp, i, 0) * p0x + OXC_M(mvp, i, 1) * p0y) + OXC_M(mvp, i, 2) * p0z) + OXC_M(mvp, i, 3);
      finite = finite && ((__builtin_fabsf(P0[i]) + __builtin_fabsf(S[i][0])) + (__builtin_fabsf(S[i][1]) + __builtin_fabsf(S[i][2]))) <= 1.329227995784916e36f;
    }
    if (__builtin_amdgcn_ballot_w64(!finite) == 0) {
#pragma unroll
      for (int i = 0; i < (NEED_Z ? 3 : 2); i++) {
        lo[i] = ((P0[i] + min0_finite(S[i][0])) + min0_finite(S[i][1])) + min0_finite(S[i][2]);
        hi[i] = ((P0[i] + max0_finite(S[i][0])) + max0_finite(S[i][1])) + max0_finite(S[i][2]);
      }
      if (1.0f < near_clip) return false;
      out[0] = lo[0] * 0.5f + 0.5f;
      out[1] = lo[1] * 0.5f + 0.5f;
      out[2] = lo[2];
      out[3] = hi[0] * 0.5f + 0.5f;
      out[4] = hi[1] * 0.5f + 0.5f;
      out[5] = hi[2];
      return true;
    }
  }
#pragma unroll
  for (int i = 0; i < 4; i++) {
    SX[i] = OXC_M(mvp, i, 0) * ex;
    SY[i] = OXC_M(mvp, i, 1) * ey;
    SZ[i] = OXC_M(mvp, i, 2) * ez;
    P[0][i] = ((OXC_M(mvp, i, 0) * p0x + OXC_M(mvp, i, 1) * p0y) + OXC_M(mvp, i, 2) * p0z) + OXC_M(mvp, i, 3);
  }
#pragma unroll
  for (int i = 0; i < 4; i++) {
    P[1][i] = P[0][i] + SZ[i];
    P[2][i] = P[0][i] + SY[i];
    P[3][i] = P[2][i] + SZ[i];
    P[4][i] = P[0][i] + SX[i];
    P[5][i] = P[4][i] + SZ[i];
    P[6][i] = P[4][i] + SY[i];
    P[7][i] = P[6][i] + SZ[i];
  }
  float depth = P[7][3];
#pragma unroll
  for (int k = 6; k >= 0; k--) depth = fminf(P[k][3], depth);
  if (depth < near_clip) return false;
  float vmin[3], vmax[3];
  float amax = 0.0f, zmin = 3.402823466e+38f, wmax = 0.0f;
#pragma unroll
  for (int k = 0; k < 8; k++) {
    amax = fmaxf(amax, fmaxf(fmaxf(__builtin_fabsf(P[k][0]), __builtin_fabsf(P[k][1])), __builtin_fabsf(P[k][2])));
    zmin = fminf(zmin, __builtin_fabsf(P[k][2]));
    wmax = fmaxf(wmax, P[k][3]);
  }
  const bool in_window = amax <= 1.152921504606846976e18f && zmin >= 8.673617379884035e-19f && depth >= 9.313225746154785e-10f &&
                         wmax <= 1.152921504606846976e18f;
  if (__builtin_amdgcn_ballot_w64(!in_window) == 0) {
    float lo[3] = {0.f, 0.f, 0.f}, hi[3] = {0.f, 0.f, 0.f};
#pragma unroll
    for (int k = 7; k >= 0; k--) {
      const float w = P[k][3];
      const float r0 = __builtin_amdgcn_rcpf(w);
      const float e = __builtin_fmaf(-w, r0, 1.0f);
      const float r = __builtin_fmaf(e, r0, r0);
      const f2 n = {P[k][0], P[k][1]};
      const f2 nw = splat(-w), rr = splat(r);
      f2 q = n * rr;
      f2 e1 = __builtin_elementwise_fma(nw, q, n);
      q = __builtin_elementwise_fma(e1, rr, q);
      e1 = __builtin_elementwise_fma(nw, q, n);
      q = __builtin_elementwise_fma(e1, rr, q);
      const float nz = P[k][2];
      float z = nz * r;
      float ez = __builtin_fmaf(-w, z, nz);
      z = __builtin_fmaf(ez, r, z);
      ez = __builtin_fmaf(-w, z, nz);
      z = __builtin_fmaf(ez, r, z);
      if (k == 7) {
        lo[0] = hi[0] = q.x;
        lo[1] = hi[1] = q.y;
        lo[2] = hi[2] = z;
      } else {
        lo[0] = fminf(q.x, lo[0]);
        hi[0] = fmaxf(q.x, hi[0]);
        lo[1] = fminf(q.y, lo[1]);
        hi[1] = fmaxf(q.y, hi[1]);
        lo[2] = fminf(z, lo[2]);
        hi[2] = fmaxf(z, hi[2]);
      }
    }
#pragma unroll
    for (int j = 0; j < 3; j++) {
      vmin[j] = lo[j];
      vmax[j] = hi[j];
    }
  } else {
#pragma unroll
    for (int j = 0; j < 3; j++) {
      float lo = P[7][j] / P[7][3];
      float hi = lo;
#pragma unroll
      for (int k = 6; k >= 0; k--) {
        float d = P[k][j] / P[k][3];
        lo = fminf(d, lo);
        hi = fmaxf(d, hi);
      }
      vmin[j] = lo;
      vmax[j] = hi;
    }
  }
  out[0] = vmin[0] * 0.5f + 0.5f;
  out[1] = vmin[1] * 0.5f + 0.5f;
  out[2] = vmin[2];
  out[3] = vmax[0] * 0.5f + 0.5f;
  out[4] = vmax[1] * 0.5f + 0.5f;
  out[5] = vmax[2];
  return true;
}

OXC_DEV bool aabb_occluded(const float* mvp, float near_clip, float cx, float cy, float cz, float ex, float ey, float ez,
                           const HizView& hiz, const uint32_t* level_off, bool active) {
  float sa[6];
  if (!active) return false;
  if (!project_aabb(mvp, near_clip, cx, cy, cz, ex, ey, ez, sa)) return false;
  const float minu = sa[0], minv = sa[1], maxu = sa[3], maxv = sa[4], maxz = sa[5];

  float sw = (float)hiz.width, sh = (float)hiz.height;
  uint32_t minx = cvt_u32_sat(fmaxf(minu * sw, 0.0f));
  uint32_t miny = cvt_u32_sat(fmaxf(minv * sh, 0.0f));
  uint32_t maxx = cvt_u32_sat(fminf(maxu * sw, sw - 1.0f));
  uint32_t maxy = cvt_u32_sat(fminf(maxv * sh, sh - 1.0f));
  uint32_t szx = maxx - minx, szy = maxy - miny;
  uint32_t ms = szx > szy ? szx : szy;
  uint32_t mip = ms <= 1u ? 0u : 32u - (uint32_t)__builtin_clz(ms - 1u);
  uint32_t top = hiz.levels - 1u;
  mip = mip > top ? top : mip;
  const float uc = ((float)minx + (float)maxx) * 0.5f, vc = ((float)miny + (float)maxy) * 0.5f;
  float u = hiz.inv_width != 0.0f ? uc * hiz.inv_width : uc / sw;
  float v = hiz.inv_height != 0.0f ? vc * hiz.inv_height : vc / sh;

  uint32_t mw = mip_dim(hiz.width, mip), mh = mip_dim(hiz.height, mip);
  int32_t mxx = (int32_t)mw - 1, mxy = (int32_t)mh - 1;
  int32_t bx = cvt_i32_sat(floorf(u * (float)mw - 0.5f));
  int32_t by = cvt_i32_sat(floorf(v * (float)mh - 0.5f));
  int32_t bx1 = (int32_t)((uint32_t)bx + 1u), by1 = (int32_t)((uint32_t)by + 1u);
  int32_t x0 = min(max(bx, 0), mxx), y0 = min(max(by, 0), mxy);
  int32_t x1 = min(max(bx1, 0), mxx), y1 = min(max(by1, 0), mxy);
  float p00, p10, p01, p11;
  if (mip >= hiz.lds_first) {
    const float* lvl = hiz.lds + hiz.lds_off[mip];
    p00 = lvl[y0 * (int32_t)mw + x0];
    p10 = lvl[y0 * (int32_t)mw + x1];
    p01 = lvl[y1 * (int32_t)mw + x0];
    p11 = lvl[y1 * (int32_t)mw + x1];
  } else {
    const float* lvl = hiz.data + level_off[mip];
    p00 = lvl[(size_t)y0 * mw + x0];
    p10 = lvl[(size_t)y0 * mw + x1];
    p01 = lvl[(size_t)y1 * mw + x0];
    p11 = lvl[(size_t)y1 * mw + x1];
  }
  float d = fminf(fminf(p00, p10), fminf(p01, p11));
  return maxz <= d - 1e-7f;
}

struct HpbView {
  const uint8_t* data;
  uint32_t width, height, layers, levels;
};

OXC_DEV uint32_t ceil_log2f_clamped(float x, uint32_t levels) {
  const uint32_t b = asu(x);
  int32_t c = (int32_t)((b >> 23) & 0xFFu) - 127 + ((b & 0x7FFFFFu) ? 1 : 0);
  c = min(max(c, 0), (int32_t)levels - 1);
  return (x > 0.0f) ? (uint32_t)c : 0u;
}
OXC_DEV float fract_f(float x) { return x - floorf(x); }

OXC_DEV bool test_vsm_page(const float* a, const HpbView& h, const uint32_t* level_off, uint32_t layer, int32_t pox_i, int32_t poy_i) {
  float sw = (float)h.width, sh = (float)h.height;
  float pox = (float)pox_i / sw, poy = (float)poy_i / sh;
  float box_w = (a[3] - a[0]) * sw, box_h = (a[4] - a[1]) * sh;
  uint32_t mip = ceil_log2f_clamped(fmaxf(box_w, box_h), h.levels);
  const uint32_t mw = mip_dim(h.width, mip), mh = mip_dim(h.height, mip);
  const float fw = (float)mw, fh = (float)mh;
  auto texel = [](float t, float extent_f, uint32_t extent) { return (uint32_t)min(cvt_i32_sat(t * extent_f), (int32_t)extent - 1); };
  const uint32_t x0 = texel(fract_f(a[0] + pox), fw, mw), x1 = texel(fract_f(a[3] + pox), fw, mw);
  const uint32_t y0 = texel(fract_f(a[1] + poy), fh, mh), y1 = texel(fract_f(a[4] + poy), fh, mh);
  const uint32_t base = level_off[mip] + layer * mw * mh, r0 = base + y0 * mw, r1 = base + y1 * mw;
  const uint32_t tl = h.data[r0 + x0], tr = h.data[r0 + x1], bl = h.data[r1 + x0], br = h.data[r1 + x1];
  return (tl | tr | bl | br) != 0u;
}

OXC_DEV bool cone_visible_directional(const float* nm, float dirx, float diry, float dirz, float ax, float ay, float az, float cutoff) {
  float nx = (nm[0] * ax + nm[3] * ay) + nm[6] * az;
  float ny = (nm[1] * ax + nm[4] * ay) + nm[7] * az;
  float nz = (nm[2] * ax + nm[5] * ay) + nm[8] * az;
  float l = len3(nx, ny, nz);
  float kx = nx / l, ky = ny / l, kz = nz / l;
  bool culled = dot3(kx, ky, kz, dirx, diry, dirz) >= cutoff;
  return cutoff >= 1.0f || !culled;
}

}
```

oxylus_amd/csrc/oxcull_kernels.hip:

```cpp
#include <hip/hip_runtime.h>

#include <algorithm>
#include <cstdlib>

#include "oxcull_device.hpp"
#include "oxcull_kernels.hpp"
#include "oxcull_types.hpp"

#pragma clang fp contract(off)

namespace oxc {

OXC_DEV uint32_t wave_sum(uint32_t v) {
#pragma unroll
  for (int o = 32; o > 0; o >>= 1) v += __shfl_xor(v, o, 64);
  return v;
}
OXC_DEV uint32_t wave_incl_scan(uint32_t v, int lane) {
#pragma unroll
  for (int o = 1; o < 64; o <<= 1) {
    uint32_t t = __shfl_up(v, o, 64);
    if (lane >= o) v += t;
  }
  return v;
// ... 358 lines not shown
        }
      }
    }
    rem &= ~run;
  }
}

typedef const uint32_t __attribute__((address_space(4))) * kconst32p;
OXC_DEV kconst32p const_row(const InstCache* cache, uint32_t mi) { return (kconst32p)(reinterpret_cast<uint64_t>(cache + mi)); }

#define OXC_LOAD_MLI load_stream_u2
#define OXC_LOAD_BND load_stream_u4
template <int G, bool UNORD = false, uint32_t kWaves = kPlainBlockWaves>
OXC_DEV void meshlets_plain_body(const MeshletTestArgs& a) {
  set_half_denorm_flush();
  constexpr uint32_t kStep = kWaves * G * 64;
  const int lane = threadIdx.x & 63, wave = threadIdx.x >> 6;
  const uint32_t N = a.n_host ? a.n_host : min(gptr(a.vis)[0], a.n_cap);
  const uint32_t nwords = (N + 63u) / 64u;
  const uint32_t nchunks = (N + kStep - 1) / kStep;
  const uint64_t mlis = reinterpret_cast<uint64_t>(a.meshlet_instances);
  const uint32_t last_index = N ? N - 1u : 0u;
  const float camx = a.cam_pos[0], camy = a.cam_pos[1], camz = a.cam_pos[2];

  for (uint32_t chunk = blockIdx.x; chunk < nchunks; chunk += gridDim.x) {
    const uint32_t group0 = (chunk * kWaves + wave) * G;
    uint2 rec[G];
    uint32_t st[G];
#pragma unroll
    for (int j = 0; j < G; j++) rec[j] = OXC_LOAD_MLI(mlis, min((group0 + j) * 64 + lane, last_index));
#pragma unroll
    for (int j = 0; j < G; j++) st[j] = ((group0 + j) * 64 + lane < N) ? 1u : 0u;

    for (;;) {
      uint32_t mi_u = 0;
      bool found = false;
#pragma unroll
      for (int j = 0; j < G; j++) {
        const uint64_t p = __builtin_amdgcn_ballot_w64((st[j] & 1u) != 0u);
        if (!found && p) {
          mi_u = readlane_u(rec[j].x, __ffsll((unsigned long long)p) - 1);
          found = true;
        }
      }
      if (!found) break;
      const kconst32p row = const_row(a.cache, mi_u);
      const uint64_t bounds = (uint64_t)row[kRowBounds] | ((uint64_t)row[kRowBounds + 1] << 32);
      uint4 bnd[G];
      bool mine[G];
#pragma unroll
      for (int j = 0; j < G; j++) {
        mine[j] = (st[j] & 1u) != 0u && rec[j].x == mi_u;
        bnd[j] = OXC_LOAD_BND(bounds, mine[j] ? rec[j].y : 0u);
      }
      float cx[G], cy[G], cz[G], ex[G], ey[G], ez[G];
      uint32_t need[G];
      uint64_t any_need = 0;
      {
        float pl[24], sg[18];
#pragma unroll
        for (int k = 0; k < 24; k++) pl[k] = asf(row[kRowPlanes + k]);
#pragma unroll
        for (int k = 0; k < 18; k++) sg[k] = asf(row[kRowSigns + k]);
#pragma unroll
        for (int j = 0; j < G; j++) {
          const uint4 b = bnd[j];
          cx[j] = dequantize_half(b.x & 0xFFFFu), cy[j] = dequantize_half(b.x >> 16), cz[j] = dequantize_half(b.y & 0xFFFFu);
          ex[j] = dequantize_half(b.z & 0xFFFFu), ey[j] = dequantize_half(b.z >> 16), ez[j] = dequantize_half(b.w & 0xFFFFu);
          const bool vis = mine[j] & test_frustum_planes(pl, sg, cx[j], cy[j], cz[j], ex[j], ey[j], ez[j]);
          const bool nc = vis & (((int32_t)b.w >> 24) != 127);
          need[j] = nc ? 1u : 0u;
          any_need |= __builtin_amdgcn_ballot_w64(nc);
          st[j] = mine[j] ? (vis ? 2u : 0u) : st[j];
          if (j == 1) __builtin_amdgcn_sched_barrier(0);
        }
      }
      if (any_need) {
        ConeU cu;
#pragma unroll
        for (int k = 0; k < 9; k++) cu.nm[k] = asf(row[kRowNm + k]);
#pragma unroll
        for (int k = 0; k < 6; k++) cu.w2[k >> 1][k & 1] = asf(row[kRowWorld2 + k]);
#pragma unroll
        for (int k = 0; k < 2; k++) cu.wt2[k] = asf(row[kRowWorldT2 + k]);
#pragma unroll
        for (int k = 0; k < 4; k++) cu.wr2[k] = asf(row[kRowWorldR2 + k]);
        cu.scale_max = asf(row[kRowScale]);
#pragma unroll
        for (int j = 0; j < G; j++) {
          if (__builtin_amdgcn_ballot_w64(need[j] != 0u) == 0) continue;
          uint4 b = bnd[j];
          asm volatile("" : "+v"(b.x), "+v"(b.y), "+v"(b.z), "+v"(b.w));
          const float qx = dequantize_half(b.x & 0xFFFFu), qy = dequantize_half(b.x >> 16), qz = dequantize_half(b.y & 0xFFFFu);
          const float rx = dequantize_half(b.z & 0xFFFFu), ry = dequantize_half(b.z >> 16), rz = dequantize_half(b.w & 0xFFFFu);
          const f2 axy = s8_over_127_x2((int32_t)(b.y << 8) >> 24, (int32_t)b.y >> 24);
          const f2 azc = s8_over_127_x2((int32_t)(b.w << 8) >> 24, (int32_t)b.w >> 24);
          const int tier1 = cone_visible_fast(cu, camx, camy, camz, qx, qy, qz, rx, ry, rz, axy.x, axy.y, azc.x, azc.y);
          bool cone_ok = tier1 == 1;
          if (__builtin_amdgcn_ballot_w64(need[j] != 0u && tier1 == 2)) {
            const bool exact = cone_visible(cu, camx, camy, camz, qx, qy, qz, rx, ry, rz, axy.x, axy.y, azc.x, azc.y);
            cone_ok = tier1 == 2 ? exact : cone_ok;
          }
          st[j] = (need[j] != 0u && !cone_ok) ? 0u : st[j];
        }
      }
    }
    if constexpr (UNORD) {
      __shared__ uint32_t s_cnt[2][kWaves];
      __shared__ uint32_t s_base[2];
      const uint32_t par = ((chunk - blockIdx.x) / gridDim.x) & 1u;
      uint64_t bits[G];
      uint32_t cnt = 0;
#pragma unroll
      for (int j = 0; j < G; j++) {
        bits[j] = __builtin_amdgcn_ballot_w64((st[j] & 2u) != 0u);
        cnt += (uint32_t)__popcll((unsigned long long)bits[j]);
      }
      if (lane == 0) s_cnt[par][wave] = cnt;
      __syncthreads();
      const uint32_t incl = wave_incl_scan((uint32_t)lane < kWaves ? s_cnt[par][(uint32_t)lane < kWaves ? lane : 0] : 0u, lane);
      const uint32_t total = readlane_u(incl, (int)kWaves - 1);
      if (threadIdx.x == 0) s_base[par] = total ? __hip_atomic_fetch_add(gptr(a.count_a), total, __ATOMIC_RELAXED, __HIP_MEMORY_SCOPE_AGENT) : 0u;
      __syncthreads();
      uint32_t at = s_base[par] + (wave ? readlane_u(incl, wave - 1) : 0u);
#pragma unroll
      for (int j = 0; j < G; j++) {
        if ((bits[j] >> lane) & 1ull)
          gptr(a.out)[at + __builtin_amdgcn_mbcnt_hi((uint32_t)(bits[j] >> 32), __builtin_amdgcn_mbcnt_lo((uint32_t)bits[j], 0u))] = (group0 + j) * 64 + (uint32_t)lane;
        at += (uint32_t)__popcll((unsigned long long)bits[j]);
      }
    } else {
    uint32_t cnt = 0;
#pragma unroll
    for (int j = 0; j < G; j++) {
      if (group0 + j >= nwords) continue;
      const uint64_t bits = __builtin_amdgcn_ballot_w64((st[j] & 2u) != 0u);
      if (lane == 0) gptr(a.bits)[group0 + j] = bits;
      cnt += (uint32_t)__popcll((unsigned long long)bits);
    }
    if (lane == 0 && group0 < nwords) {
      const uint32_t wchunk = chunk * kWaves + wave;
      gptr(a.chunk_counts)[wchunk] = cnt;
      if (cnt) __hip_atomic_fetch_add(gptr(a.supers) + (wchunk / kChunksPerSuper) * kSuperStride, cnt, __ATOMIC_RELAXED, __HIP_MEMORY_SCOPE_AGENT);
    }
    }
  }
}

constexpr uint32_t kTicketRun = 4;
OXC_DEV uint32_t OXC_TICKET_STEP(uint32_t t, uint32_t K, uint32_t x) { return ((t / kTicketRun) * K + x) * kTicketRun + t % kTicketRun; }
template <bool OCCL, bool LATE, int G, int SHARE = 0, bool COUNT = false>
OXC_DEV void meshlets_hiz_body(const MeshletTestArgs& a) {
  static_assert(SHARE == 0 || (OCCL && G == 4 && (SHARE == 1) == !LATE), "sharing: early call writes, late call reads");
  set_half_denorm_flush();
  constexpr int kWaves = 16 / G;
  constexpr bool OCCL_OR_LATE = OCCL || LATE;
  __shared__ uint32_t s_level_off[13];
  __shared__ uint32_t s_lds_off[13];
  __shared__ float s_hiz_top[kHizLdsTexels];
  __shared__ uint4 s_strip[OCCL_OR_LATE ? kWaves : 1][G * 64];
  __shared__ uint32_t s_flags[OCCL_OR_LATE ? kWaves : 1][G * 64];
  const int lane = threadIdx.x & 63, wave = threadIdx.x >> 6;
  const uint32_t N = a.n_host ? a.n_host : min(gptr(a.vis)[0], a.n_cap);
  const uint32_t nwords = (N + 63u) / 64u;
  const uint32_t nchunks = (N + kMeshletChunk - 1) / kMeshletChunk;
  if (threadIdx.x < 13) {
    s_level_off[threadIdx.x] = a.hiz_level_off[threadIdx.x];
    s_lds_off[threadIdx.x] = a.hiz_lds_off[threadIdx.x];
  }
  for (uint32_t k = a.hiz_lds_first; k < a.hiz_levels; k++) {
    const uint32_t n = mip_dim(a.hiz_w, k) * mip_dim(a.hiz_h, k);
    const float* src = a.hiz_data + a.hiz_level_off[k];
    float* dst = s_hiz_top + a.hiz_lds_off[k];
    for (uint32_t i = threadIdx.x; i < n; i += blockDim.x) dst[i] = src[i];
  }
  __syncthreads();
  HizView hiz;
  hiz.data = a.hiz_data;
  hiz.width = a.hiz_w;
  hiz.height = a.hiz_h;
  hiz.levels = a.hiz_levels;
  hiz.lds = s_hiz_top;
  hiz.lds_off = s_lds_off;
  hiz.lds_first = a.hiz_lds_first;
  hiz.inv_width = exact_reciprocal_or_zero(a.hiz_w);
  hiz.inv_height = exact_reciprocal_or_zero(a.hiz_h);
  const uint64_t mlis = reinterpret_cast<uint64_t>(a.meshlet_instances);
  const uint32_t last_index = N ? N - 1u : 0u;
  const float camx = a.cam_pos[0], camy = a.cam_pos[1], camz = a.cam_pos[2];

  const uint32_t nsteps = nchunks * kWaves;
  const uint32_t K = min(kTicketCounters, gridDim.x), kx = blockIdx.x % K;
  uint32_t* const ticket = a.tickets ? a.tickets + kx * kSuperStride : nullptr;
  auto draw_ticket = [&]() -> uint32_t {
    uint32_t t = 0;
    if (lane == 0) t = __hip_atomic_fetch_add(ticket, 1u, __ATOMIC_RELAXED, __HIP_MEMORY_SCOPE_AGENT);
    return t;
  };
  uint32_t step = blockIdx.x * kWaves + wave;
  if (ticket) step = OXC_TICKET_STEP(readlane_u(draw_ticket(), 0), K, kx);
  while (step < nsteps) {
    const uint32_t group0 = step * G;
    uint2 rec[G];
    uint32_t st[G];
    uint32_t mask_idx[G];
    bool quick = false;
    uint32_t fbit[G];
#pragma unroll
    for (int j = 0; j < G; j++) fbit[j] = 0u;
    if constexpr (SHARE == 2) {
      uint64_t any = 0;
#pragma unroll
      for (int j = 0; j < G; j++) {
        const uint64_t w = group0 + j < nwords ? gptr(a.camera_test_bits)[group0 + j] : 0ull;
        any |= w;
        fbit[j] = ((w >> lane) & 1ull) != 0ull ? 8u : 0u;
      }
      const uint2 info = load_global_u2(reinterpret_cast<uint64_t>(a.step_info), step);
      quick = any == 0ull && info.y != 0u;
      if (quick) {
#pragma unroll
        for (int j = 0; j < G; j++) {
          st[j] = 0u;
          mask_idx[j] = info.x + 64u * (uint32_t)j + (uint32_t)lane;
          rec[j] = make_uint2(0u, 0u);
        }
      }
    }
    if (!quick) {
#pragma unroll
      for (int j = 0; j < G; j++) rec[j] = OXC_LOAD_MLI(mlis, min((group0 + j) * 64 + lane, last_index));
    }
    const uint32_t next_ticket = ticket ? draw_ticket() : 0u;
    if (!quick) {
#pragma unroll
      for (int j = 0; j < G; j++) {
        st[j] = (((group0 + j) * 64 + lane < N) ? 1u : 0u) | fbit[j];
        mask_idx[j] = 0;
      }
    }
    for (;;) {
      uint32_t mi_u = 0;
      bool found = false;
#pragma unroll
      for (int j = 0; j < G; j++) {
        const uint64_t p = __builtin_amdgcn_ballot_w64((st[j] & 1u) != 0u);
        if (!found && p) {
          mi_u = readlane_u(rec[j].x, __ffsll((unsigned long long)p) - 1);
          found = true;
        }
      }
      if (!found) break;
      const kconst32p row = const_row(a.cache, mi_u);
      const uint64_t bounds = (uint64_t)row[kRowBounds] | ((uint64_t)row[kRowBounds + 1] << 32);
      const uint32_t vis_offset = row[kRowVisOffset];
      uint4 bnd[G];
      bool mine[G];
      uint32_t mword[G];
#pragma unroll
      for (int j = 0; j < G; j++) {
        mine[j] = (st[j] & 1u) != 0u && rec[j].x == mi_u;
        const bool fetch = SHARE == 2 ? (mine[j] && (st[j] & 8u) != 0u) : mine[j];
        bnd[j] = OXC_LOAD_BND(bounds, fetch ? rec[j].y : 0u);
        mword[j] = 0xFFFFFFFFu;
        if (OCCL) {
          uint32_t mi_bit = vis_offset + (mine[j] ? rec[j].y : 0u);
          const bool in_mask = mi_bit < a.mask_bits;
          mi_bit = in_mask ? mi_bit : 0u;
          mask_idx[j] = mine[j] ? (in_mask ? mi_bit : kMaskNone) : mask_idx[j];
          mword[j] = load_global_u32(reinterpret_cast<uint64_t>(a.mask), mi_bit >> 5) >> (mi_bit & 31u);
          mword[j] = in_mask ? mword[j] : 0u;
        }
      }
      float cx[G], cy[G], cz[G], ex[G], ey[G], ez[G];
      uint32_t need[G];
      uint64_t any_need = 0;
      {
        float pl[24], sg[18];
#pragma unroll
        for (int k = 0; k < 24; k++) pl[k] = asf(row[kRowPlanes + k]);
#pragma unroll
        for (int k = 0; k < 18; k++) sg[k] = asf(row[kRowSigns + k]);
#pragma unroll
        for (int j = 0; j < G; j++) {
          const uint4 b = bnd[j];
          const bool was_visible = (mword[j] & 1u) != 0u;
          if constexpr (SHARE == 2) {
            const bool vis = mine[j] & ((st[j] & 8u) != 0u);
            cx[j] = cy[j] = cz[j] = ex[j] = ey[j] = ez[j] = 0.0f;
            need[j] = 0u;
            st[j] = mine[j] ? ((vis ? 2u : 0u) | (was_visible ? 4u : 0u)) : st[j];
            continue;
          }
          if (!LATE && SHARE == 0 && __builtin_amdgcn_ballot_w64(mine[j] && was_visible) == 0) {
            cx[j] = cy[j] = cz[j] = ex[j] = ey[j] = ez[j] = 0.0f;
            need[j] = 0u;
            st[j] = mine[j] ? 0u : st[j];
            continue;
          }
          cx[j] = dequantize_half(b.x & 0xFFFFu), cy[j] = dequantize_half(b.x >> 16), cz[j] = dequantize_half(b.y & 0xFFFFu);
          ex[j] = dequantize_half(b.z & 0xFFFFu), ey[j] = dequantize_half(b.z >> 16), ez[j] = dequantize_half(b.w & 0xFFFFu);
          const bool inside = mine[j] & test_frustum_planes(pl, sg, cx[j], cy[j], cz[j], ex[j], ey[j], ez[j]);
          const bool vis = inside & ((LATE || SHARE == 1) ? true : was_visible);
          const bool nc = vis & (((int32_t)b.w >> 24) != 127);
          need[j] = nc ? 1u : 0u;
          any_need |= __builtin_amdgcn_ballot_w64(nc);
          st[j] = mine[j] ? ((vis ? 2u : 0u) | (was_visible ? 4u : 0u)) : st[j];
        }
      }
      if constexpr (OCCL_OR_LATE) {
        uint64_t vb[G];
        uint32_t base[G + 1];
        base[0] = 0;
#pragma unroll
        for (int j = 0; j < G; j++) {
          vb[j] = __builtin_amdgcn_ballot_w64(mine[j] && (st[j] & 2u) != 0u);
          base[j + 1] = base[j] + (uint32_t)__popcll((unsigned long long)vb[j]);
        }
        const uint32_t total = base[G];
        if (total) {
          uint4* strip = s_strip[wave];
          uint32_t* flg = s_flags[wave];
          uint32_t slot[G];
#pragma unroll
          for (int j = 0; j < G; j++) {
            slot[j] = base[j] + __builtin_amdgcn_mbcnt_hi((uint32_t)(vb[j] >> 32), __builtin_amdgcn_mbcnt_lo((uint32_t)vb[j], 0u));
            if ((vb[j] >> lane) & 1ull) {
              if constexpr (SHARE == 2) {
                strip[slot[j]] = make_uint4(bnd[j].x, bnd[j].y, bnd[j].z, (bnd[j].w & 0x00FFFFFFu) | (slot[j] << 24));
                flg[slot[j]] = 1u;
              } else {
                strip[slot[j]] = bnd[j];
                if constexpr (SHARE == 1) flg[slot[j]] = st[j] & 4u;
              }
            }
          }
          asm volatile("s_waitcnt lgkmcnt(0)" ::: "memory");
          uint32_t nb = SHARE == 2 ? total : 0u;
          if constexpr (SHARE != 2) {
          ConeU cu;
#pragma unroll
          for (int k = 0; k < 9; k++) cu.nm[k] = asf(row[kRowNm + k]);
#pragma unroll
          for (int k = 0; k < 6; k++) cu.w2[k >> 1][k & 1] = asf(row[kRowWorld2 + k]);
#pragma unroll
          for (int k = 0; k < 2; k++) cu.wt2[k] = asf(row[kRowWorldT2 + k]);
#pragma unroll
          for (int k = 0; k < 4; k++) cu.wr2[k] = asf(row[kRowWorldR2 + k]);
          cu.scale_max = asf(row[kRowScale]);
          for (uint32_t t0 = 0; t0 < total; t0 += 64) {
            const uint32_t t = t0 + (uint32_t)lane;
            const bool act = t < total;
            const uint4 b = strip[act ? t : total - 1u];
            bool ok = act;
            const bool nc = act && ((int32_t)b.w >> 24) != 127;
            if (__builtin_amdgcn_ballot_w64(nc)) {
              const float qx = dequantize_half(b.x & 0xFFFFu), qy = dequantize_half(b.x >> 16), qz = dequantize_half(b.y & 0xFFFFu);
              const float rx = dequantize_half(b.z & 0xFFFFu), ry = dequantize_half(b.z >> 16), rz = dequantize_half(b.w & 0xFFFFu);
              const f2 axy = s8_over_127_x2((int32_t)(b.y << 8) >> 24, (int32_t)b.y >> 24);
              const f2 azc = s8_over_127_x2((int32_t)(b.w << 8) >> 24, (int32_t)b.w >> 24);
              const int tier1 = cone_visible_fast(cu, camx, camy, camz, qx, qy, qz, rx, ry, rz, axy.x, axy.y, azc.x, azc.y);
              bool cone_ok = tier1 == 1;
              if (__builtin_amdgcn_ballot_w64(nc && tier1 == 2)) {
                const bool exact = cone_visible(cu, camx, camy, camz, qx, qy, qz, rx, ry, rz, axy.x, axy.y, azc.x, azc.y);
                cone_ok = tier1 == 2 ? exact : cone_ok;
              }
              ok = nc ? cone_ok : ok;
            }
            const bool okv = SHARE == 1 ? (ok && (flg[act ? t : 0u] & 4u) != 0u) : ok;
            const uint64_t okb = __builtin_amdgcn_ballot_w64(okv);
            const uint32_t rank = __builtin_amdgcn_mbcnt_hi((uint32_t)(okb >> 32), __builtin_amdgcn_mbcnt_lo((uint32_t)okb, 0u));
            if (act) flg[t] = SHARE == 1 ? ((ok ? 1u : 0u) | (okv ? 2u : 0u)) : (ok ? 1u : 0u);
            if (okv) strip[nb + rank] = make_uint4(b.x, b.y, b.z, (b.w & 0x00FFFFFFu) | (t << 24));
            nb += (uint32_t)__popcll((unsigned long long)okb);
          }
          }
          asm volatile("s_waitcnt lgkmcnt(0)" ::: "memory");
          if constexpr (COUNT) {
            if (nb && lane == 0) __hip_atomic_fetch_add(gptr(a.dbg_occlusion) + (step & 255u) * kSuperStride, nb, __ATOMIC_RELAXED, __HIP_MEMORY_SCOPE_AGENT);
          }
          if (nb) {
            float mvp[16];
#pragma unroll
            for (int k = 0; k < 16; k++) mvp[k] = asf(row[kRowMvp + k]);
            for (uint32_t u0 = 0; u0 < nb; u0 += 64) {
              const uint32_t u = u0 + (uint32_t)lane;
              const bool act = u < nb;
              const uint4 b = strip[act ? u : nb - 1u];
              const float qx = dequantize_half(b.x & 0xFFFFu), qy = dequantize_half(b.x >> 16), qz = dequantize_half(b.y & 0xFFFFu);
              const float rx = dequantize_half(b.z & 0xFFFFu), ry = dequantize_half(b.z >> 16), rz = dequantize_half(b.w & 0xFFFFu);
              const bool occluded = aabb_occluded(mvp, a.near_clip, qx, qy, qz, rx, ry, rz, hiz, s_level_off, act);
              if (act && occluded) flg[b.w >> 24] = SHARE == 1 ? 1u : 0u;
            }
            asm volatile("s_waitcnt lgkmcnt(0)" ::: "memory");
          }
#pragma unroll
          for (int j = 0; j < G; j++) {
            if ((vb[j] >> lane) & 1ull) {
              const uint32_t f = flg[slot[j]];
              if constexpr (SHARE == 1)
                st[j] = (st[j] & ~2u) | (f & 2u) | ((f & 1u) << 3);
              else
                st[j] = f ? st[j] : (st[j] & ~2u);
            }
          }
          asm volatile("s_waitcnt lgkmcnt(0)" ::: "memory");
        }
      } else if (any_need) {
        ConeU cu;
#pragma unroll
        for (int k = 0; k < 9; k++) cu.nm[k] = asf(row[kRowNm + k]);
#pragma unroll
        for (int k = 0; k < 6; k++) cu.w2[k >> 1][k & 1] = asf(row[kRowWorld2 + k]);
#pragma unroll
        for (int k = 0; k < 2; k++) cu.wt2[k] = asf(row[kRowWorldT2 + k]);
#pragma unroll
        for (int k = 0; k < 4; k++) cu.wr2[k] = asf(row[kRowWorldR2 + k]);
        cu.scale_max = asf(row[kRowScale]);
#pragma unroll
        for (int j = 0; j < G; j++) {
          if (__builtin_amdgcn_ballot_w64(need[j] != 0u) == 0) continue;
          uint4 b = bnd[j];
          asm volatile("" : "+v"(b.x), "+v"(b.y), "+v"(b.z), "+v"(b.w));
          const float qx = dequantize_half(b.x & 0xFFFFu), qy = dequantize_half(b.x >> 16), qz = dequantize_half(b.y & 0xFFFFu);
          const float rx = dequantize_half(b.z & 0xFFFFu), ry = dequantize_half(b.z >> 16), rz = dequantize_half(b.w & 0xFFFFu);
          const f2 axy = s8_over_127_x2((int32_t)(b.y << 8) >> 24, (int32_t)b.y >> 24);
          const f2 azc = s8_over_127_x2((int32_t)(b.w << 8) >> 24, (int32_t)b.w >> 24);
          const int tier1 = cone_visible_fast(cu, camx, camy, camz, qx, qy, qz, rx, ry, rz, axy.x, axy.y, azc.x, azc.y);
          bool cone_ok = tier1 == 1;
          if (__builtin_amdgcn_ballot_w64(need[j] != 0u && tier1 == 2)) {
            const bool exact = cone_visible(cu, camx, camy, camz, qx, qy, qz, rx, ry, rz, axy.x, axy.y, azc.x, azc.y);
            cone_ok = tier1 == 2 ? exact : cone_ok;
          }
          st[j] = (need[j] != 0u && !cone_ok) ? (st[j] & ~2u) : st[j];
        }
      }
    }
    bool step_run = false;
    uint32_t run_first = 0;
    if constexpr (OCCL && G == 4) {
      if ((group0 + G) * 64u <= N) {
        const uint32_t d0 = readfirst_u(mask_idx[0]);
        run_first = d0;
        uint64_t bad = 0;
#pragma unroll
        for (int j = 0; j < G; j++) bad |= __builtin_amdgcn_ballot_w64(mask_idx[j] != d0 + 64u * (uint32_t)j + (uint32_t)lane);
        if (bad == 0ull && d0 <= 0xFFFFFFFFu - 64u * G) {
          step_run = true;
          uint32_t* row8 = s_flags[wave];
#pragma unroll
          for (int j = 0; j < G; j++) {
            const uint64_t vb = __builtin_amdgcn_ballot_w64((st[j] & 2u) != 0u);
            if (lane == 0) {
              row8[2 * j] = (uint32_t)vb;
              row8[2 * j + 1] = (uint32_t)(vb >> 32);
            }
          }
          asm volatile("s_waitcnt lgkmcnt(0)" ::: "memory");
          const uint32_t cur = lane < 2 * G ? row8[lane] : 0u;
          const uint32_t prev = (lane >= 1 && lane <= 2 * G) ? row8[lane - 1] : 0u;
          const uint32_t sh = d0 & 31u, w0 = d0 >> 5;
          if (sh == 0u) {
            if (lane < 2 * G) a.mask[w0 + (uint32_t)lane] = cur;
          } else {
            const uint32_t word = __builtin_amdgcn_alignbit(cur, prev, 32u - sh);
            if (lane >= 1 && lane < 2 * G) {
              a.mask[w0 + (uint32_t)lane] = word;
            } else if (lane == 0 || lane == 2 * G) {
              const uint32_t own = lane == 0 ? (0xFFFFFFFFu << sh) : (0xFFFFFFFFu >> (32u - sh));
              const uint32_t zero = own & ~word;
              if (zero) atomicAnd(&a.mask[w0 + (uint32_t)lane], ~zero);
              if (word) atomicOr(&a.mask[w0 + (uint32_t)lane], word);
            }
          }
          asm volatile("s_waitcnt lgkmcnt(0)" ::: "memory");
        }
      }
    }
    if constexpr (SHARE == 1) {
#pragma unroll
      for (int j = 0; j < G; j++) {
        const uint64_t w = __builtin_amdgcn_ballot_w64((st[j] & 8u) != 0u);
        if (lane == 0 && group0 + j < nwords) gptr(a.camera_test_bits)[group0 + j] = w;
      }
      if (lane == 0) {
        uint32_t* info = reinterpret_cast<uint32_t*>(a.step_info + step);
        gptr(info)[0] = run_first;
        gptr(info)[1] = step_run ? 1u : 0u;
      }
    }
    uint32_t cnt = 0;
#pragma unroll
    for (int j = 0; j < G; j++) {
      if (group0 + j >= nwords) continue;
      const bool visible = (st[j] & 2u) != 0u;
      if (OCCL && !step_run) update_visibility_mask(a.mask, mask_idx[j], visible, (group0 + j) * 64 + lane < N && mask_idx[j] != kMaskNone, lane);
      const bool emit = visible && (!LATE || (st[j] & 4u) == 0u);
      const uint64_t bits = __builtin_amdgcn_ballot_w64(emit);
      if (lane == 0) gptr(a.bits)[group0 + j] = bits;
      cnt += (uint32_t)__popcll((unsigned long long)bits);
    }
    if (lane == 0 && group0 < nwords) {
      gptr(a.chunk_counts)[step] = cnt;
      if (cnt) __hip_atomic_fetch_add(gptr(a.supers) + (step / kChunksPerSuper) * kSuperStride, cnt, __ATOMIC_RELAXED, __HIP_MEMORY_SCOPE_AGENT);
    }
    step = ticket ? OXC_TICKET_STEP(readlane_u(next_ticket, 0), K, kx) : step + gridDim.x * kWaves;
  }
}

constexpr int kHpbWaves = 6;
__global__ __launch_bounds__(256, kHpbWaves) void k_cull_meshlets_hpb_test(HpbTestArgs a) {
  set_half_denorm_flush();
  __shared__ uint32_t s_level_off[13];
  constexpr int G = (int)kGroupsPerWave;
  constexpr uint32_t kWaves = 4;
  __shared__ uint4 s_strip[kWaves][G * 64];
  __shared__ uint32_t s_strip2[kWaves][G * 64];
  __shared__ uint32_t s_seen[kWaves][G * 64];
  __shared__ uint64_t s_in[kWaves][16][G];
  const int lane = threadIdx.x & 63, wave = threadIdx.x >> 6;
  const uint32_t N = min(a.vis[0], a.n_cap);
  const uint32_t nwords = (N + 63u) / 64u;
  const uint32_t nchunks = (N + kMeshletChunk - 1) / kMeshletChunk;
  if (threadIdx.x < 13) s_level_off[threadIdx.x] = a.hpb_level_off[threadIdx.x];
  __syncthreads();
  const uint64_t dirty_mask = __builtin_amdgcn_ballot_w64((uint32_t)lane < a.clipmap_count && a.dirty[(uint32_t)lane < a.clipmap_count ? lane : 0] != 0u);
  HpbView hpb;
  hpb.data = a.hpb_data;
  hpb.width = a.hpb_w;
  hpb.height = a.hpb_h;
  hpb.layers = a.hpb_layers;
  hpb.levels = a.hpb_levels;
  const uint64_t mlis = reinterpret_cast<uint64_t>(a.meshlet_instances);
  const uint32_t last_index = N ? N - 1u : 0u;

  const uint32_t nsteps = nchunks * kWaves;
  const uint32_t K = min(kTicketCounters, gridDim.x), kx = blockIdx.x % K;
  uint32_t* const ticket = a.tickets + kx * kSuperStride;
  auto draw_ticket = [&]() -> uint32_t {
    uint32_t t = 0;
    if (lane == 0) t = __hip_atomic_fetch_add(ticket, 1u, __ATOMIC_RELAXED, __HIP_MEMORY_SCOPE_AGENT);
    return t;
  };
  uint4* const strip = s_strip[wave];
  uint32_t* const strip2 = s_strip2[wave];
  uint32_t* const seen = s_seen[wave];
  uint32_t step = OXC_TICKET_STEP(readlane_u(draw_ticket(), 0), K, kx);
// ... 584 lines not shown
  float q[2][2];
#pragma unroll
  for (int r = 0; r < 2; r++)
#pragma unroll
    for (int c = 0; c < 2; c++)
      q[r][c] = fminf(fminf(m[2 * r][2 * c], m[2 * r][2 * c + 1]), fminf(m[2 * r + 1][2 * c], m[2 * r + 1][2 * c + 1]));
  {
    float* mip1 = a.hiz + a.level_off[1];
    const uint32_t w1 = W >> 1;
#pragma unroll
    for (int r = 0; r < 2; r++) {
      *reinterpret_cast<float2*>(mip1 + (size_t)((y0 >> 1) + r) * w1 + (x0 >> 1)) = make_float2(q[r][0], q[r][1]);
    }
  }
  if (a.levels <= 2) return;
  float d = fminf(fminf(q[0][0], q[0][1]), fminf(q[1][0], q[1][1]));
  (a.hiz + a.level_off[2])[(size_t)(y0 >> 2) * (W >> 2) + (x0 >> 2)] = d;
  s_a[ty * 16 + tx] = d;
  if (a.levels <= 3) return;
  __syncthreads();
  if (threadIdx.x < 64) {
    uint32_t px = threadIdx.x & 7, py = threadIdx.x >> 3;
    float v = fminf(fminf(s_a[(2 * py) * 16 + 2 * px], s_a[(2 * py) * 16 + 2 * px + 1]),
                    fminf(s_a[(2 * py + 1) * 16 + 2 * px], s_a[(2 * py + 1) * 16 + 2 * px + 1]));
    (a.hiz + a.level_off[3])[(size_t)(blockIdx.y * 8 + py) * (W >> 3) + blockIdx.x * 8 + px] = v;
    s_b[py * 8 + px] = v;
  }
  if (a.levels <= 4) return;
  __syncthreads();
  if (threadIdx.x < 16) {
    uint32_t px = threadIdx.x & 3, py = threadIdx.x >> 2;
    float v = fminf(fminf(s_b[(2 * py) * 8 + 2 * px], s_b[(2 * py) * 8 + 2 * px + 1]),
                    fminf(s_b[(2 * py + 1) * 8 + 2 * px], s_b[(2 * py + 1) * 8 + 2 * px + 1]));
    (a.hiz + a.level_off[4])[(size_t)(blockIdx.y * 4 + py) * (W >> 4) + blockIdx.x * 4 + px] = v;
    s_a[py * 4 + px] = v;
  }
  if (a.levels <= 5) return;
  __syncthreads();
  if (threadIdx.x < 4) {
    uint32_t px = threadIdx.x & 1, py = threadIdx.x >> 1;
    float v = fminf(fminf(s_a[(2 * py) * 4 + 2 * px], s_a[(2 * py) * 4 + 2 * px + 1]),
                    fminf(s_a[(2 * py + 1) * 4 + 2 * px], s_a[(2 * py + 1) * 4 + 2 * px + 1]));
    (a.hiz + a.level_off[5])[(size_t)(blockIdx.y * 2 + py) * (W >> 5) + blockIdx.x * 2 + px] = v;
    s_b[py * 2 + px] = v;
  }
  if (a.levels <= 6) return;
  __syncthreads();
  if (threadIdx.x == 0) {
    float v = fminf(fminf(s_b[0], s_b[1]), fminf(s_b[2], s_b[3]));
    (a.hiz + a.level_off[6])[(size_t)blockIdx.y * (W >> 6) + blockIdx.x] = v;
  }
}

__global__ __launch_bounds__(256) void k_hiz_mip0_generic(HizArgs a) {
  const uint32_t n = a.w * a.h;
  const float invx = 1.0f / (float)a.w, invy = 1.0f / (float)a.h;
  float* mip0 = a.hiz + a.level_off[0];
  for (uint32_t i = blockIdx.x * blockDim.x + threadIdx.x; i < n; i += gridDim.x * blockDim.x) {
    uint32_t x = i % a.w, y = i / a.w;
    mip0[i] = hiz_point_sample(a.depth, a.dw, a.dh, x, y, invx, invy);
  }
}

__global__ __launch_bounds__(1024) void k_hiz_tail(HizArgs a, uint32_t start) {
  __shared__ float s_buf[2][4096];
  uint32_t pw = mip_dim(a.w, start), ph = mip_dim(a.h, start);
  const float* src = a.hiz + a.level_off[start];
  for (uint32_t i = threadIdx.x; i < pw * ph; i += blockDim.x) s_buf[0][i] = src[i];
  __syncthreads();
  int cur = 0;
  for (uint32_t k = start + 1; k < a.levels; k++) {
    uint32_t cw = mip_dim(a.w, k), ch = mip_dim(a.h, k);
    float* dst = a.hiz + a.level_off[k];
    for (uint32_t i = threadIdx.x; i < cw * ch; i += blockDim.x) {
      uint32_t x = i % cw, y = i / cw;
      uint32_t xa = 2 * x, ya = 2 * y;
      uint32_t xb = xa + 1 < pw ? xa + 1 : pw - 1, yb = ya + 1 < ph ? ya + 1 : ph - 1;
      float v = fminf(fminf(s_buf[cur][ya * pw + xa], s_buf[cur][ya * pw + xb]),
                      fminf(s_buf[cur][yb * pw + xa], s_buf[cur][yb * pw + xb]));
      s_buf[cur ^ 1][i] = v;
      dst[i] = v;
    }
    __syncthreads();
    cur ^= 1;
    pw = cw;
    ph = ch;
  }
}

__global__ __launch_bounds__(256) void k_seed_slot(uint32_t* slot, uint32_t total) {
  if (threadIdx.x == 0 && blockIdx.x == 0) {
    slot[SLOT_VIS + 0] = total;
    slot[SLOT_VIS + 1] = 0;
    slot[SLOT_VIS + 2] = 0;
    slot[SLOT_MESHLETS_CMD + 0] = (total + 63u) / 64u;
    slot[SLOT_MESHLETS_CMD + 1] = 1;
    slot[SLOT_MESHLETS_CMD + 2] = 1;
  }
}

__global__ __launch_bounds__(64) void k_pack_counters(const uint32_t* vis, const uint32_t* tri_cmd, const uint32_t* draw_cmd, uint32_t* out4) {
  if (threadIdx.x == 0) {
    out4[0] = tri_cmd ? tri_cmd[0] : 0u;
    out4[1] = vis ? vis[1] : 0u;
    out4[2] = vis ? vis[2] : 0u;
    out4[3] = draw_cmd ? draw_cmd[0] : 0u;
  }
}

__global__ __launch_bounds__(256) void k_stream_read(const uint4* __restrict__ p, uint64_t n16, uint32_t* sink) {
  uint32_t acc = 0;
  const uint64_t tiles = n16 / 1024;
  for (uint64_t t = blockIdx.x; t < tiles; t += gridDim.x) {
    const uint4* q = p + t * 1024 + threadIdx.x;
    uint4 a = q[0], b = q[256], c = q[512], d = q[768];
    acc ^= a.x ^ a.y ^ a.z ^ a.w ^ b.x ^ b.y ^ b.z ^ b.w ^ c.x ^ c.y ^ c.z ^ c.w ^ d.x ^ d.y ^ d.z ^ d.w;
  }
  for (uint64_t i = tiles * 1024 + (uint64_t)blockIdx.x * 256 + threadIdx.x; i < n16; i += (uint64_t)gridDim.x * 256) {
    uint4 v = p[i];
    acc ^= v.x ^ v.y ^ v.z ^ v.w;
  }
  if (acc == 0x9E3779B9u) *sink = acc;
}

__global__ __launch_bounds__(256) void k_debug_decode_bounds(const uint4* __restrict__ bounds, uint32_t n, float* __restrict__ out10) {
  set_half_denorm_flush();
  for (uint32_t i = blockIdx.x * blockDim.x + threadIdx.x; i < n; i += gridDim.x * blockDim.x) {
    const uint4 b = bounds[i];
    float* o = out10 + (size_t)i * 10;
    o[0] = dequantize_half(b.x & 0xFFFFu);
    o[1] = dequantize_half(b.x >> 16);
    o[2] = dequantize_half(b.y & 0xFFFFu);
    o[3] = dequantize_half(b.z & 0xFFFFu);
    o[4] = dequantize_half(b.z >> 16);
    o[5] = dequantize_half(b.w & 0xFFFFu);
    o[6] = s8_over_127((int32_t)(b.y << 8) >> 24);
    o[7] = s8_over_127((int32_t)b.y >> 24);
    o[8] = s8_over_127((int32_t)(b.w << 8) >> 24);
    o[9] = s8_over_127((int32_t)b.w >> 24);
  }
}

__global__ __launch_bounds__(256) void k_prepare_instances(PrepareArgs a) { prepare_body(a, blockIdx.y); }
__global__ __launch_bounds__(1024) void k_scan_mesh_counts(ScanArgs a) { scan_body(a); }
__global__ __launch_bounds__(256) void k_expand_meshlet_instances(ExpandArgs a) { expand_body(a); }
template <bool HIZ, bool OCCL, bool LATE, int G = (int)kGroupsPerWave>
__global__ __launch_bounds__(1024 / G, (HIZ && (OCCL || LATE)) ? 5 : 1) void k_cull_meshlets_test(MeshletTestArgs a) {
  if constexpr (!HIZ)
    meshlets_plain_body<G>(a);
  else
    meshlets_hiz_body<OCCL, LATE, G>(a);
}
__global__ __launch_bounds__(64 * kUnordBlockWaves) void k_cull_meshlets_test_unordered(MeshletTestArgs a) { meshlets_plain_body<(int)kGroupsPerWave, true, kUnordBlockWaves>(a); }
template <bool LATE>
__global__ __launch_bounds__(1024 / kHizGroupsPerWave, 5) void k_cull_meshlets_test_shared(MeshletTestArgs a) {
  meshlets_hiz_body<true, LATE, (int)kHizGroupsPerWave, LATE ? 2 : 1>(a);
}
template <bool LATE, int SHARE>
__global__ __launch_bounds__(1024 / kHizGroupsPerWave, 4) void k_cull_meshlets_test_counting(MeshletTestArgs a) {
  meshlets_hiz_body<true, LATE, (int)kHizGroupsPerWave, SHARE, true>(a);
}
template <bool HIZ, bool LATE>
__global__ __launch_bounds__(256) void k_cull_meshlets_emit(MeshletEmitArgs a) {
  meshlets_emit_body<HIZ, LATE>(a);
}
constexpr int kTriWaves = 8;
constexpr int kTriWideWaves = 4;
template <bool LATE, bool WIDE, bool SMALL>
__global__ __launch_bounds__(256, WIDE ? kTriWideWaves : (SMALL ? 6 : kTriWaves)) void k_cull_triangles_test(TriTestArgs a) {
  tris_test_body<LATE, WIDE, SMALL>(a);
}
template <bool LATE, bool WIDE>
__global__ __launch_bounds__(256) void k_cull_triangles_emit(TriEmitArgs a) {
  tris_emit_body<LATE, WIDE>(a);
}
template <bool LATE, bool WIDE, bool SMALL>
__global__ __launch_bounds__(256, WIDE ? kTriWideWaves : (SMALL ? 6 : kTriWaves)) void k_cull_triangles_fused(TriTestArgs a) {
  tris_fused_body<LATE, WIDE, SMALL>(a);
}
template <bool LATE, bool SMALL>
__global__ __launch_bounds__(256, kTriWideWaves) void k_cull_triangles_fused_pairs(TriTestArgs a) {
  tris_fused_body<LATE, true, SMALL, true>(a);
}
template <bool LATE>
__global__ __launch_bounds__(256) void k_cull_triangles_emit_pairs(TriEmitArgs a) {
  tris_emit_body<LATE, true, true>(a);
}
template <bool LATE, int INDEX>
__global__ __launch_bounds__(256, INDEX ? kTriWideWaves : kTriWaves) void k_cull_triangles_fused_cached(TriTestArgs a) {
  tris_fused_body<LATE, INDEX != 0, false, INDEX == 2, true>(a);
}
template <bool LATE, bool WIDE>
__global__ __launch_bounds__(256, WIDE ? kTriWideWaves : kTriWaves) void k_cull_triangles_test_cached(TriTestArgs a) {
  tris_test_body<LATE, WIDE, false, true>(a);
}

__global__ __launch_bounds__(256) void k_prepare_batch(BatchBlob blob, BatchElem* __restrict__ dev) {
#define OXC_PREPARE_CASE(i)                                                                             \
  case i: {                                                                                             \
    if (blockIdx.x == 0 && threadIdx.x == 0) expand_batch_core(blob.core[i], dev[blob.first + i]);      \
    PrepareArgs pa;                                                                                     \
    prepare_args_of(blob.core[i], pa);                                                                  \
    prepare_body(pa, 0u);                                                                               \
  } break;
  switch (blockIdx.y) {
    OXC_PREPARE_CASE(0)
    OXC_PREPARE_CASE(1)
    OXC_PREPARE_CASE(2)
    OXC_PREPARE_CASE(3)
    OXC_PREPARE_CASE(4)
    OXC_PREPARE_CASE(5)
    OXC_PREPARE_CASE(6)
    OXC_PREPARE_CASE(7)
    OXC_PREPARE_CASE(8)
    OXC_PREPARE_CASE(9)
    OXC_PREPARE_CASE(10)
    OXC_PREPARE_CASE(11)
    OXC_PREPARE_CASE(12)
    OXC_PREPARE_CASE(13)
    OXC_PREPARE_CASE(14)
    default: {
      if (blockIdx.x == 0 && threadIdx.x == 0) expand_batch_core(blob.core[15], dev[blob.first + 15]);
      PrepareArgs pa;
      prepare_args_of(blob.core[15], pa);
      prepare_body(pa, 0u);
    } break;
  }
#undef OXC_PREPARE_CASE
  static_assert(kBatchPerPrepare == 16, "one case per element core of the blob");
}
__global__ __launch_bounds__(1024) void k_scan_batch(const BatchElem* __restrict__ dev) { scan_body(dev[blockIdx.y].scan); }
__global__ __launch_bounds__(256) void k_expand_batch(const BatchElem* __restrict__ dev) { expand_body(dev[blockIdx.y].expand); }
__global__ __launch_bounds__(64 * kPlainBlockWaves) void k_cull_meshlets_test_batch(const BatchElem* __restrict__ dev) {
  meshlets_plain_body<(int)kGroupsPerWave>(dev[blockIdx.y].test);
}
__global__ __launch_bounds__(256) void k_cull_meshlets_emit_batch(const BatchElem* __restrict__ dev) {
  meshlets_emit_body<false, false>(dev[blockIdx.y].emit);
}
__global__ __launch_bounds__(256, 8) void k_cull_triangles_test_batch(const BatchElem* __restrict__ dev) {
  tris_test_body<false, false, false>(dev[blockIdx.y].ttest);
}
__global__ __launch_bounds__(256) void k_cull_triangles_emit_batch(const BatchElem* __restrict__ dev) {
  tris_emit_body<false, false>(dev[blockIdx.y].temit);
}

constexpr uint32_t kMvChunk = 256;

__global__ __launch_bounds__(256) void k_mv_group(MvArgs a, MvBlob blob) {
  static_assert(kMaxBatch == 16, "one lane per view in a 16-lane segment");
  const uint32_t tid = blockIdx.x * blockDim.x + threadIdx.x, nthreads = gridDim.x * blockDim.x;
  const int lane = threadIdx.x & 63;
  const uint32_t v = (uint32_t)lane & 15u, seg = (uint32_t)lane & ~15u;
  const MvView* const table = blob.v;
  if (tid < a.views) a.dev[tid] = table[tid];
  for (uint32_t u = 0; u < a.views; u++)
    for (uint32_t i = tid; i < table[u].n_supers; i += nthreads) table[u].supers[i * kSuperStride] = 0;
  if (tid < kTicketCounters) a.tickets[tid * kSuperStride] = 0;
  const uint32_t per_round = nthreads >> 4, rounds = (a.M + per_round - 1) / per_round;
  for (uint32_t r = 0; r < rounds; r++) {
    const uint32_t mi = r * per_round + (tid >> 4);
    const bool live = mi < a.M && v < a.views;
    uint64_t kb = 0;
    uint32_t kt = 0, cnt = 0;
    if (live) {
      const MvView& w = table[v];
      const uint32_t c = w.mesh_counts[mi], off = w.mesh_offsets[mi];
      cnt = off >= w.n_cap ? 0u : min(c, w.n_cap - off);
      const InstCache* row = w.rows + mi;
      kb = row->bounds;
      kt = row->transform_index;
      w.vchunks[mi] = (cnt + kMvChunk - 1) / kMvChunk;
      if (w.runs) {
        w.runs[2 * mi] = cnt ? off : 0u;
        w.runs[2 * mi + 1] = cnt;
      }
    }
    uint32_t same = 0;
#pragma unroll
    for (uint32_t u = 0; u < 16; u++) {
      const uint32_t lo = (uint32_t)__shfl((int)(uint32_t)kb, (int)(seg + u), 64), hi = (uint32_t)__shfl((int)(uint32_t)(kb >> 32), (int)(seg + u), 64);
      const uint32_t tu = (uint32_t)__shfl((int)kt, (int)(seg + u), 64), cu = (uint32_t)__shfl((int)cnt, (int)(seg + u), 64);
      if (cnt != 0u && cu == cnt && tu == kt && (((uint64_t)hi << 32) | lo) == kb) same |= 1u << u;
    }
    const bool leader = cnt != 0u && (uint32_t)__builtin_ctz(same | 0x10000u) == v;
    bool eq = cnt != 0u;
    if (eq) {
      const uint32_t lead = (uint32_t)__builtin_ctz(same | 0x10000u) & 15u;
      const uint4* mine = reinterpret_cast<const uint4*>(table[v].rows + mi);
      const uint4* theirs = reinterpret_cast<const uint4*>(table[lead].rows + mi);
#pragma unroll
      for (int q = 0; q < 6; q++) {
        const uint4 x = mine[q], y = theirs[q];
        eq = eq && x.x == y.x && x.y == y.y && ((q & 1) || (x.z == y.z && x.w == y.w));
      }
    }
    const uint32_t nsame = (uint32_t)(__ballot(eq) >> seg) & same & 0xFFFFu;
    const uint32_t leaders = (uint32_t)(__ballot(leader) >> seg) & 0xFFFFu;
    const uint32_t g = (uint32_t)__popc(leaders & ((1u << v) - 1u)), ngroups = (uint32_t)__popc(leaders);
    uint32_t chunks = leader ? (cnt + kMvChunk - 1) / kMvChunk : 0u;
#pragma unroll
    for (int o = 8; o > 0; o >>= 1) chunks += (uint32_t)__shfl_xor((int)chunks, o, 64);
    if (mi < a.M) {
      MvGroup* out = a.groups + (size_t)mi * a.views;
      if (leader) out[g] = MvGroup{kb, cnt, same | (nsame << 16)};
      if (v >= ngroups && v < a.views) out[v] = MvGroup{0, 0, 0};
      if (v == 0) a.grp_chunks[mi] = chunks;
    }
  }
}
// ... 145 lines not shown
          const uint4 bj = SAME_POS ? load_global_u4(bounds, min(k0 + (uint32_t)j * 64u + (uint32_t)lane, count - 1u)) : bnd[j];
          OXC_MV_DECODE(bj);
          bits[j] = __builtin_amdgcn_ballot_w64(test_frustum_planes(pl, sg, cxj, cyj, czj, exj, eyj, ezj)) & okb[j];
        }
      }
      uint32_t cnt = 0;
#pragma unroll
      for (int j = 0; j < G; j++) {
        cnt += (uint32_t)__popcll((unsigned long long)bits[j]);
        const bool here = (uint32_t)lane == v * (uint32_t)G + (uint32_t)j;
        blo = here ? (uint32_t)bits[j] : blo;
        bhi = here ? (uint32_t)(bits[j] >> 32) : bhi;
      }
      cnts = (uint32_t)lane == v ? cnt : cnts;
    }
#undef OXC_MV_DECODE
    {
      static_assert(G == 4 && kMaxBatch == 16, "one ballot word per lane");
      const uint32_t vv = (uint32_t)lane >> 2, jj = (uint32_t)lane & 3u;
      const uint32_t pv = (uint32_t)__shfl((int)lp, (int)vv, 64);
      if ((vmask >> vv) & 1u) gptr(a.dev[vv].bits)[(size_t)pv * G + jj] = (uint64_t)blo | ((uint64_t)bhi << 32);
      if ((uint32_t)lane < 16u && ((vmask >> lane) & 1u)) {
        const MvView* w = a.dev + lane;
        gptr(w->counts)[lp] = cnts;
        gptr(w->idbase)[lp] = lid0;
        if (cnts) __hip_atomic_fetch_add(gptr(w->supers) + (lp / kChunksPerSuper) * kSuperStride, cnts, __ATOMIC_RELAXED, __HIP_MEMORY_SCOPE_AGENT);
      }
    }
    step = OXC_TICKET_STEP(readlane_u(next_ticket, 0), K, kx);
  }
}

__global__ __launch_bounds__(256) void k_mv_emit(MvArgs a) {
  const int lane = threadIdx.x & 63, wave = threadIdx.x >> 6;
  const MvView& w = a.dev[blockIdx.y];
  uint32_t* const out = w.out;
  const uint64_t* const wbits = w.bits;
  const uint32_t *const widbase = w.idbase, *const wsupers = w.supers, *const wcounts = w.counts;
  uint32_t* const wtri_cmd = w.tri_cmd;
  const uint32_t nchunks = gptr(w.scan_total)[0];
  const uint32_t nwords = nchunks * 4u;
  const uint32_t nspans = (nchunks + 15u) / 16u;
  if (nspans == 0u && blockIdx.x == 0 && threadIdx.x == 0) gptr(wtri_cmd)[0] = 0u;
  for (uint32_t span = blockIdx.x * 4u + (uint32_t)wave; span < nspans; span += gridDim.x * 4u) {
    const uint32_t wd = span * 64u + (uint32_t)lane;
    const uint32_t wc = min(wd, nwords - 1u);
    uint64_t bits = gptr(wbits)[wc];
    const uint32_t idb = gptr(widbase)[wc >> 2] + (wc & 3u) * 64u;
    const uint32_t c0 = span * 16u, sup = c0 / kChunksPerSuper;
    uint32_t acc = 0;
    for (uint32_t i0 = (uint32_t)lane; i0 < sup; i0 += 512u) {
      uint32_t part[8];
#pragma unroll
      for (uint32_t u = 0; u < 8u; u++) part[u] = gptr(wsupers)[min(i0 + 64u * u, sup - 1u) * kSuperStride];
#pragma unroll
      for (uint32_t u = 0; u < 8u; u++) acc += i0 + 64u * u < sup ? part[u] : 0u;
    }
    const uint32_t j = sup * kChunksPerSuper + (uint32_t)lane;
    if (j < c0) acc += gptr(wcounts)[j];
    const uint32_t base = wave_sum(acc);
    if (wd >= nwords) bits = 0ull;
    const uint32_t cnt = (uint32_t)__popcll((unsigned long long)bits);
    const uint32_t incl = wave_incl_scan(cnt, lane);
    const uint32_t off = base + incl - cnt;
    if (lane == 63 && span == nspans - 1u) gptr(wtri_cmd)[0] = base + incl;
    const uint32_t blo = (uint32_t)bits, bhi = (uint32_t)(bits >> 32);
#pragma unroll 4
    for (int k = 0; k < 64; k++) {
      const uint64_t bk = (uint64_t)readlane_u(blo, k) | ((uint64_t)readlane_u(bhi, k) << 32);
      if (bk == 0ull) continue;
      const uint32_t ok = readlane_u(off, k), ik = readlane_u(idb, k);
      if ((bk >> lane) & 1ull) gptr(out)[ok + __builtin_amdgcn_mbcnt_hi((uint32_t)(bk >> 32), __builtin_amdgcn_mbcnt_lo((uint32_t)bk, 0u))] = ik + (uint32_t)lane;
    }
  }
}

void launch_mv_setup(const MvArgs& a, const MvBlob& blob, uint32_t grid, hipStream_t s) {
  hipLaunchKernelGGL(k_mv_group, dim3(grid), dim3(256), 0, s, a, blob);
  hipLaunchKernelGGL(k_mv_scan, dim3(1, a.views + 1), dim3(1024), 0, s, a);
  hipLaunchKernelGGL(k_mv_steps, dim3(std::max(1u, std::min((a.M + 3u) / 4u, grid))), dim3(256), 0, s, a);
}
void launch_mv_test(const MvArgs& a, uint32_t num_cus, hipStream_t s) {
  if (a.same_pos)
    hipLaunchKernelGGL(k_mv_test<true>, dim3(num_cus * 8u), dim3(256), 0, s, a);
  else
    hipLaunchKernelGGL(k_mv_test<false>, dim3(num_cus * 8u), dim3(256), 0, s, a);
}
void launch_mv_emit(const MvArgs& a, uint32_t max_chunks_per_view, uint32_t max_grid, hipStream_t s) {
  const uint32_t blocks = std::max(1u, ((max_chunks_per_view + 15u) / 16u + 3u) / 4u);
  hipLaunchKernelGGL(k_mv_emit, dim3(std::min(blocks, std::max(max_grid / std::max(1u, a.views), max_grid / 4u)), a.views), dim3(256), 0, s, a);
}

void launch_prepare(const PrepareArgs& a, uint32_t grid, uint32_t views, hipStream_t s) {
  hipLaunchKernelGGL(k_prepare_instances, dim3(grid, 1 + views), dim3(256), 0, s, a);
}

void launch_scan_mesh_counts(const uint32_t* counts, uint32_t* offsets, uint32_t n, uint32_t cap, uint32_t* vis, uint32_t* cmd, hipStream_t s) {
  ScanArgs a{counts, offsets, n, cap, vis, cmd};
  hipLaunchKernelGGL(k_scan_mesh_counts, dim3(1), dim3(1024), 0, s, a);
}
void launch_expand(const uint32_t* counts, const uint32_t* offsets, uint32_t n, uint32_t cap, void* out, uint32_t grid, hipStream_t s) {
  ExpandArgs a{counts, offsets, n, cap, reinterpret_cast<GpuMeshletInstance*>(out)};
  hipLaunchKernelGGL(k_expand_meshlet_instances, dim3(grid), dim3(256), 0, s, a);
}
void launch_prepare_batch(const BatchBlob& blob, BatchElem* dev, uint32_t grid, hipStream_t s) {
  hipLaunchKernelGGL(k_prepare_batch, dim3(grid, blob.count), dim3(256), 0, s, blob, dev);
}
void launch_scan_batch(const BatchElem* dev, uint32_t count, hipStream_t s) { hipLaunchKernelGGL(k_scan_batch, dim3(1, count), dim3(1024), 0, s, dev); }
void launch_expand_batch(const BatchElem* dev, uint32_t count, uint32_t grid, hipStream_t s) {
  hipLaunchKernelGGL(k_expand_batch, dim3(grid, count), dim3(256), 0, s, dev);
}
void launch_meshlets_test_batch(const BatchElem* dev, uint32_t count, uint32_t grid, hipStream_t s) {
  hipLaunchKernelGGL(k_cull_meshlets_test_batch, dim3(grid * (4 / kPlainBlockWaves), count), dim3(64 * kPlainBlockWaves), 0, s, dev);
}
void launch_meshlets_emit_batch(const BatchElem* dev, uint32_t count, uint32_t grid, hipStream_t s) {
  hipLaunchKernelGGL(k_cull_meshlets_emit_batch, dim3(grid, count), dim3(256), 0, s, dev);
}
void launch_tris_test_batch(const BatchElem* dev, uint32_t count, uint32_t grid, hipStream_t s) {
  hipLaunchKernelGGL(k_cull_triangles_test_batch, dim3(grid, count), dim3(256), 0, s, dev);
}
void launch_tris_emit_batch(const BatchElem* dev, uint32_t count, uint32_t grid, hipStream_t s) {
  hipLaunchKernelGGL(k_cull_triangles_emit_batch, dim3(grid, count), dim3(256), 0, s, dev);
}

constexpr int kHizGroups = (int)kHizGroupsPerWave;
template <class K>
static uint32_t resident_grid(K kernel, uint32_t block, uint32_t num_cus) {
  int per_cu = 0;
  if (hipOccupancyMaxActiveBlocksPerMultiprocessor(&per_cu, kernel, (int)block, 0) != hipSuccess || per_cu <= 0) return num_cus * 8u;
  return (uint32_t)per_cu * num_cus;
}
void launch_meshlets_test(const MeshletTestArgs& a, bool hiz, bool occl, bool late, uint32_t grid, uint32_t num_cus, uint32_t grid_limit, hipStream_t s) {
  constexpr uint32_t hb = 1024 / kHizGroups;
  if (hiz && grid_limit) grid = std::min(grid, grid_limit);
  if (a.out) {
    hipLaunchKernelGGL(k_cull_meshlets_test_unordered, dim3((grid * 4 + kUnordBlockWaves - 1) / kUnordBlockWaves), dim3(64 * kUnordBlockWaves), 0, s, a);
    return;
  }
  if (hiz && occl && a.dbg_occlusion) {
    const dim3 g(std::min(grid, num_cus * 4u)), b(hb);
    if (a.share == 2)
      hipLaunchKernelGGL((k_cull_meshlets_test_counting<true, 2>), g, b, 0, s, a);
    else if (a.share == 1)
      hipLaunchKernelGGL((k_cull_meshlets_test_counting<false, 1>), g, b, 0, s, a);
    else if (late)
      hipLaunchKernelGGL((k_cull_meshlets_test_counting<true, 0>), g, b, 0, s, a);
    else
      hipLaunchKernelGGL((k_cull_meshlets_test_counting<false, 0>), g, b, 0, s, a);
    return;
  }
  if (!hiz) {
    hipLaunchKernelGGL((k_cull_meshlets_test<false, false, false>), dim3(grid * (4 / kPlainBlockWaves)), dim3(64 * kPlainBlockWaves), 0, s, a);
  } else if (occl && a.share) {
    if (a.share == 2) {
      static const uint32_t cap = resident_grid(k_cull_meshlets_test_shared<true>, hb, num_cus);
      hipLaunchKernelGGL((k_cull_meshlets_test_shared<true>), dim3(std::min(grid, cap)), dim3(hb), 0, s, a);
    } else {
      static const uint32_t cap = resident_grid(k_cull_meshlets_test_shared<false>, hb, num_cus);
      hipLaunchKernelGGL((k_cull_meshlets_test_shared<false>), dim3(std::min(grid, cap)), dim3(hb), 0, s, a);
    }
  } else if (occl && late) {
    static const uint32_t cap = resident_grid(k_cull_meshlets_test<true, true, true, kHizGroups>, hb, num_cus);
    hipLaunchKernelGGL((k_cull_meshlets_test<true, true, true, kHizGroups>), dim3(std::min(grid, cap)), dim3(hb), 0, s, a);
  } else if (occl) {
    static const uint32_t cap = resident_grid(k_cull_meshlets_test<true, true, false, kHizGroups>, hb, num_cus);
    hipLaunchKernelGGL((k_cull_meshlets_test<true, true, false, kHizGroups>), dim3(std::min(grid, cap)), dim3(hb), 0, s, a);
  } else if (late) {
    static const uint32_t cap = resident_grid(k_cull_meshlets_test<true, false, true, kHizGroups>, hb, num_cus);
    hipLaunchKernelGGL((k_cull_meshlets_test<true, false, true, kHizGroups>), dim3(std::min(grid, cap)), dim3(hb), 0, s, a);
  } else {
    static const uint32_t cap = resident_grid(k_cull_meshlets_test<true, false, false, kHizGroups>, hb, num_cus);
    hipLaunchKernelGGL((k_cull_meshlets_test<true, false, false, kHizGroups>), dim3(std::min(grid, cap)), dim3(hb), 0, s, a);
  }
}
void launch_hpb_test(const HpbTestArgs& a, uint32_t grid, hipStream_t s) { hipLaunchKernelGGL(k_cull_meshlets_hpb_test, dim3(grid), dim3(256), 0, s, a); }
void launch_meshlets_emit(const MeshletEmitArgs& a, bool hiz, bool late, uint32_t grid, hipStream_t s) {
  dim3 g(grid), b(256);
  if (!hiz)
    hipLaunchKernelGGL((k_cull_meshlets_emit<false, false>), g, b, 0, s, a);
  else if (late)
    hipLaunchKernelGGL((k_cull_meshlets_emit<true, true>), g, b, 0, s, a);
  else
    hipLaunchKernelGGL((k_cull_meshlets_emit<true, false>), g, b, 0, s, a);
}
void launch_tris_test(const TriTestArgs& a, bool late, bool wide, bool small_triangle_cull, bool cached, uint32_t grid, hipStream_t s) {
  dim3 g(grid), b(256);
  if (cached && !small_triangle_cull) {
    if (late && wide)
      hipLaunchKernelGGL((k_cull_triangles_test_cached<true, true>), g, b, 0, s, a);
    else if (late)
      hipLaunchKernelGGL((k_cull_triangles_test_cached<true, false>), g, b, 0, s, a);
    else if (wide)
      hipLaunchKernelGGL((k_cull_triangles_test_cached<false, true>), g, b, 0, s, a);
    else
      hipLaunchKernelGGL((k_cull_triangles_test_cached<false, false>), g, b, 0, s, a);
    return;
  }
  const int v = (late ? 4 : 0) | (wide ? 2 : 0) | (small_triangle_cull ? 1 : 0);
  switch (v) {
    case 0: hipLaunchKernelGGL((k_cull_triangles_test<false, false, false>), g, b, 0, s, a); break;
    case 1: hipLaunchKernelGGL((k_cull_triangles_test<false, false, true>), g, b, 0, s, a); break;
    case 2: hipLaunchKernelGGL((k_cull_triangles_test<false, true, false>), g, b, 0, s, a); break;
    case 3: hipLaunchKernelGGL((k_cull_triangles_test<false, true, true>), g, b, 0, s, a); break;
    case 4: hipLaunchKernelGGL((k_cull_triangles_test<true, false, false>), g, b, 0, s, a); break;
    case 5: hipLaunchKernelGGL((k_cull_triangles_test<true, false, true>), g, b, 0, s, a); break;
    case 6: hipLaunchKernelGGL((k_cull_triangles_test<true, true, false>), g, b, 0, s, a); break;
    default: hipLaunchKernelGGL((k_cull_triangles_test<true, true, true>), g, b, 0, s, a); break;
  }
}
void launch_tris_fused(const TriTestArgs& a, bool late, uint32_t wide, bool small_triangle_cull, bool cached, uint32_t grid, uint32_t resident_cus, hipStream_t s) {
  dim3 b(256);
  const int v = (late ? 4 : 0) | (wide ? 2 : 0) | (small_triangle_cull ? 1 : 0);
#define OXC_FUSED_LAUNCH(K_)                                                                                       \
  {                                                                                                                \
    static const uint32_t per_cu = resident_grid(K_, 256, 1);                                                      \
    const uint32_t g = resident_cus ? std::min(grid, per_cu * resident_cus) : grid;                                \
    hipLaunchKernelGGL(K_, dim3(std::max(g, 1u)), b, 0, s, a);                                                     \
  }
#define OXC_FUSED_CASE(i, L_, W_, S_)                                                                              \
  case i:                                                                                                          \
    OXC_FUSED_LAUNCH((k_cull_triangles_fused<L_, W_, S_>))                                                         \
    break;
  if (cached && !small_triangle_cull) {
    switch ((late ? 4 : 0) | (int)std::min(wide, 2u)) {
      case 0: OXC_FUSED_LAUNCH((k_cull_triangles_fused_cached<false, 0>)) break;
      case 1: OXC_FUSED_LAUNCH((k_cull_triangles_fused_cached<false, 1>)) break;
      case 2: OXC_FUSED_LAUNCH((k_cull_triangles_fused_cached<false, 2>)) break;
      case 4: OXC_FUSED_LAUNCH((k_cull_triangles_fused_cached<true, 0>)) break;
      case 5: OXC_FUSED_LAUNCH((k_cull_triangles_fused_cached<true, 1>)) break;
      default: OXC_FUSED_LAUNCH((k_cull_triangles_fused_cached<true, 2>)) break;
    }
    return;
  }
  if (wide == 2u) {
    switch (v & 5) {
      case 0: OXC_FUSED_LAUNCH((k_cull_triangles_fused_pairs<false, false>)) break;
      case 1: OXC_FUSED_LAUNCH((k_cull_triangles_fused_pairs<false, true>)) break;
      case 4: OXC_FUSED_LAUNCH((k_cull_triangles_fused_pairs<true, false>)) break;
      default: OXC_FUSED_LAUNCH((k_cull_triangles_fused_pairs<true, true>)) break;
    }
    return;
  }
  switch (v) {
    OXC_FUSED_CASE(0, false, false, false)
    OXC_FUSED_CASE(1, false, false, true)
    OXC_FUSED_CASE(2, false, true, false)
    OXC_FUSED_CASE(3, false, true, true)
    OXC_FUSED_CASE(4, true, false, false)
    OXC_FUSED_CASE(5, true, false, true)
    OXC_FUSED_CASE(6, true, true, false)
    default:
      OXC_FUSED_CASE(7, true, true, true)
  }
#undef OXC_FUSED_CASE
#undef OXC_FUSED_LAUNCH
}
void launch_tris_emit(const TriEmitArgs& a, bool late, uint32_t wide, uint32_t grid, hipStream_t s) {
  dim3 g(grid), b(256);
  if (wide == 2u && late)
    hipLaunchKernelGGL((k_cull_triangles_emit_pairs<true>), g, b, 0, s, a);
  else if (wide == 2u)
    hipLaunchKernelGGL((k_cull_triangles_emit_pairs<false>), g, b, 0, s, a);
  else if (late && wide)
    hipLaunchKernelGGL((k_cull_triangles_emit<true, true>), g, b, 0, s, a);
  else if (late)
    hipLaunchKernelGGL((k_cull_triangles_emit<true, false>), g, b, 0, s, a);
  else if (wide)
    hipLaunchKernelGGL((k_cull_triangles_emit<false, true>), g, b, 0, s, a);
  else
    hipLaunchKernelGGL((k_cull_triangles_emit<false, false>), g, b, 0, s, a);
}
void launch_hiz(const HizArgs& a, uint32_t num_cus, hipStream_t s) {
  if (a.w % 64 == 0 && a.h % 64 == 0) {
    (void)num_cus;
    hipLaunchKernelGGL(k_hiz_tile, dim3(a.w / 64, a.h / 64), dim3(256), 0, s, a);
    if (a.levels > 7) hipLaunchKernelGGL(k_hiz_tail, dim3(1), dim3(1024), 0, s, a, 6u);
  } else {
    uint32_t n = a.w * a.h;
    hipLaunchKernelGGL(k_hiz_mip0_generic, dim3((n + 255) / 256), dim3(256), 0, s, a);
    if (a.levels > 1) hipLaunchKernelGGL(k_hiz_tail, dim3(1), dim3(1024), 0, s, a, 0u);
  }
}
void launch_seed_slot(uint32_t* slot, uint32_t total, hipStream_t s) { hipLaunchKernelGGL(k_seed_slot, dim3(1), dim3(64), 0, s, slot, total); }
void launch_pack_counters(const uint32_t* vis, const uint32_t* tri_cmd, const uint32_t* draw_cmd, uint32_t* out4, hipStream_t s) {
  hipLaunchKernelGGL(k_pack_counters, dim3(1), dim3(64), 0, s, vis, tri_cmd, draw_cmd, out4);
}
__global__ __launch_bounds__(64) void k_pack_counters_batch(PackBlob b, uint32_t* out4) {
  const uint32_t e = threadIdx.x;
  if (e < b.count) {
    const uint32_t *vis = b.vis[e], *tri = b.tri_cmd[e], *draw = b.draw_cmd[e];
    out4[e * 4 + 0] = tri ? tri[0] : 0u;
    out4[e * 4 + 1] = vis ? vis[0] : 0u;
    out4[e * 4 + 2] = vis ? vis[2] : 0u;
    out4[e * 4 + 3] = draw ? draw[0] : 0u;
  }
}
void launch_pack_counters_batch(const PackBlob& blob, uint32_t* out4, hipStream_t s) { hipLaunchKernelGGL(k_pack_counters_batch, dim3(1), dim3(64), 0, s, blob, out4); }
void launch_stream_read(const void* p, uint64_t bytes, uint32_t* sink, uint32_t grid, hipStream_t s) {
  hipLaunchKernelGGL(k_stream_read, dim3(grid), dim3(256), 0, s, reinterpret_cast<const uint4*>(p), bytes / 16, sink);
}
__global__ __launch_bounds__(256) void k_debug_project_aabb(DebugProjectArgs a) {
  for (uint32_t i = blockIdx.x * blockDim.x + threadIdx.x; i < a.n; i += gridDim.x * blockDim.x) {
    const float* b = a.boxes6 + (size_t)i * 6;
    float sa[6] = {0.f, 0.f, 0.f, 0.f, 0.f, 0.f};
    const bool ok = project_aabb<false>(a.mvp, a.near_clip, b[0], b[1], b[2], b[3], b[4], b[5], sa);
    float sb[6] = {0.f, 0.f, 0.f, 0.f, 0.f, 0.f};
    const bool ok_b = project_aabb<true>(a.mvp, a.near_clip, b[0], b[1], b[2], b[3], b[4], b[5], sb);
// ... 18 lines not shown
```

oxylus_amd/csrc/oxcull_kernels.hpp:

```cpp
#pragma once
#include <hip/hip_runtime.h>

#include <cstdint>

#include "oxcull.h"
#include "oxcull_types.hpp"

namespace oxc {

struct PrepareArgs {
  const GpuMesh* meshes;
  const float* transforms;
  GpuMeshInstance* mesh_instances;
  InstCache* cache;
  uint32_t* mesh_counts;
  uint32_t* slot;
  uint32_t* vis;
  uint32_t* meshlets_cmd;
  uint32_t* supers_meshlets;
  uint32_t* supers_tris;
  uint32_t n_supers_meshlets, n_supers_tris;
  uint32_t* tickets;
  uint32_t* slot_late;
  uint32_t* supers_meshlets_late;
  uint32_t* supers_tris_late;
  uint32_t* tickets_late;
  uint32_t mesh_instance_count;
  uint32_t cull_flags;
  uint32_t do_cull_meshes;
  uint32_t init_vis;
  uint32_t seed_total;
  oxc_cull_camera cam;
  const oxc_virtual_clipmap* clipmaps;
  InstCache* view_cache;
};

struct HpbTestArgs {
  const InstCache* cache;
  const InstCache* view_cache;
  const GpuMeshletInstance* meshlet_instances;
  const uint32_t* vis;
  uint64_t* bits;
  uint32_t* chunk_counts;
  uint32_t* supers;
  uint32_t* tickets;
  const oxc_virtual_clipmap* clipmaps;
  const uint32_t* dirty;
  uint32_t clipmap_count;
  uint32_t mesh_instance_count;
  uint32_t n_cap;
  const uint8_t* hpb_data;
  uint32_t hpb_w, hpb_h, hpb_layers, hpb_levels;
  uint32_t hpb_level_off[13];
  float light_dir[3];
};

struct MeshletTestArgs {
  uint32_t n_host;
  uint32_t n_cap;
  uint32_t mask_bits;
  const InstCache* cache;
  const GpuMeshletInstance* meshlet_instances;
  const uint32_t* vis;
  uint32_t* mask;
  uint64_t* bits;
  uint32_t* chunk_counts;
  uint32_t* supers;
  uint32_t* tickets;
  uint32_t share;
  uint32_t* out;
  uint32_t* count_a;
  uint32_t* dbg_occlusion;
  uint64_t* camera_test_bits;
  uint2* step_info;
  const float* hiz_data;
  uint32_t hiz_level_off[13];
  uint32_t hiz_w, hiz_h, hiz_levels;
  uint32_t hiz_lds_first;
  uint32_t hiz_lds_off[13];
  float near_clip;
  float cam_pos[3];
};

struct MeshletEmitArgs {
  uint32_t n_host;
  uint32_t n_cap;
  uint32_t count_meshlets;
  const uint64_t* bits;
  const uint32_t* chunk_counts;
  const uint32_t* supers;
  uint32_t* vis;
  uint32_t* tri_cmd;
  uint32_t* out;
};

struct TriTestArgs {
  const InstCache* cache;
  const GpuMeshletInstance* meshlet_instances;
  const uint32_t* visible;
  const uint32_t* vis;
  const uint32_t* tri_cmd;
  uint64_t* tri_masks;
  uint32_t* chunk_counts;
  uint32_t* supers;
  float resolution[2];
  uint32_t* draw_cmd;
  uint32_t* out;
  uint32_t* ticket;
  uint32_t ticket_count;
};

struct TriEmitArgs {
  const uint64_t* tri_masks;
  const uint32_t* visible;
  const uint32_t* vis;
  const uint32_t* tri_cmd;
  const uint32_t* chunk_counts;
  const uint32_t* supers;
  uint32_t* draw_cmd;
  uint32_t* out;
};

struct ScanArgs {
  const uint32_t* counts;
  uint32_t* offsets;
  uint32_t n;
  uint32_t cap;
  uint32_t* vis;
  uint32_t* meshlets_cmd;
};

struct ExpandArgs {
  const uint32_t* counts;
  const uint32_t* offsets;
  uint32_t n;
  uint32_t cap;
  GpuMeshletInstance* out;
};

constexpr uint32_t kMaxBatch = 16;
constexpr uint32_t kBatchPerPrepare = 16;
struct BatchElem {
  PrepareArgs prep;
  ScanArgs scan;
  ExpandArgs expand;
  MeshletTestArgs test;
  MeshletEmitArgs emit;
  TriTestArgs ttest;
  TriEmitArgs temit;
};
struct BatchCore {
  const GpuMesh* meshes;
  const float* transforms;
  GpuMeshInstance* mesh_instances;
  GpuMeshletInstance* meshlet_instances;
  uint32_t* visible_out;
  uint32_t* reordered_out;
  InstCache* cache;
  InstCache* view_cache;
  uint32_t* mesh_counts;
  uint32_t* mesh_offsets;
  uint64_t* bits;
  uint32_t* m_chunk_counts;
  uint32_t* m_supers;
  uint64_t* tri_masks;
  uint32_t* t_chunk_counts;
  uint32_t* t_supers;
  uint32_t* slot;
  uint32_t* vis;
  uint32_t* meshlets_cmd;
  uint32_t n_supers_meshlets, n_supers_tris;
  uint32_t mesh_instance_count;
  uint32_t cull_flags;
  uint32_t do_cull_meshes;
  uint32_t init_vis;
  uint32_t n_host;
  uint32_t n_cap;
  uint32_t count_meshlets;
  oxc_cull_camera cam;
};
struct BatchBlob {
  BatchCore core[kBatchPerPrepare];
  uint32_t count;
  uint32_t first;
};
static_assert(sizeof(BatchBlob) <= 8000, "must fit the kernarg segment");

#if defined(__HIPCC__)
__host__ __device__
#endif
inline void prepare_args_of(const BatchCore& c, PrepareArgs& pa) {
  pa.meshes = c.meshes;
  pa.transforms = c.transforms;
  pa.mesh_instances = c.mesh_instances;
  pa.cache = c.cache;
  pa.mesh_counts = c.mesh_counts;
  pa.slot = c.slot;
  pa.vis = c.vis;
  pa.meshlets_cmd = c.meshlets_cmd;
  pa.supers_meshlets = c.m_supers;
  pa.supers_tris = c.t_supers;
  pa.tickets = nullptr;
  pa.slot_late = nullptr;
  pa.supers_meshlets_late = pa.supers_tris_late = pa.tickets_late = nullptr;
  pa.n_supers_meshlets = c.n_supers_meshlets;
  pa.n_supers_tris = c.n_supers_tris;
  pa.mesh_instance_count = c.mesh_instance_count;
  pa.cull_flags = c.cull_flags;
  pa.do_cull_meshes = c.do_cull_meshes;
  pa.init_vis = c.init_vis;
  pa.seed_total = 0;
  pa.cam = c.cam;
  pa.clipmaps = nullptr;
  pa.view_cache = c.view_cache;
}
#if defined(__HIPCC__)
__host__ __device__
#endif
inline void expand_batch_core(const BatchCore& c, BatchElem& e) {
  uint32_t* tri_cmd = c.slot + SLOT_TRI_CMD;
  uint32_t* draw_cmd = c.slot + SLOT_DRAW_CMD;
  prepare_args_of(c, e.prep);
  e.scan = ScanArgs{c.mesh_counts, c.mesh_offsets, c.mesh_instance_count, c.n_cap, c.vis, c.meshlets_cmd};
  e.expand = ExpandArgs{c.mesh_counts, c.mesh_offsets, c.mesh_instance_count, c.n_cap, c.meshlet_instances};
  MeshletTestArgs& ta = e.test;
  ta.n_host = c.n_host;
  ta.n_cap = c.n_cap;
// ... 323 lines not shown
```

oxylus_amd/lib.py:

```python
from __future__ import annotations

import ctypes as C
import os
import subprocess

_HERE = os.path.dirname(os.path.abspath(__file__))
LIB_PATH = os.path.join(_HERE, "liboxcull.so")
CSRC_DIR = os.path.join(_HERE, "csrc")

OXC_OK, OXC_INVALID_ARG, OXC_HIP_ERROR, OXC_RCCL_ERROR, OXC_OUT_OF_MEMORY = range(5)
ABI_VERSION = 5

CULL_TEST_FRUSTUM = 1
CULL_SELECT_LOD = 2
CULL_TEST_OCCLUSION = 4
CULL_LATE_PASS = 8
CULL_TEST_ALL = 7

STAGE_MESHES = 1
STAGE_MESHLETS = 2
STAGE_TRIANGLES = 4
STAGE_ALL = 7

TUNE_ASYNC_MTEST_BLOCKS_PER_CU, TUNE_ASYNC_TRI_BLOCKS_PER_CU, TUNE_RASTER_BIG_CAPACITY, TUNE_TRI_BLOCKS_PER_CU, TUNE_MV_EXPAND_ASYNC, TUNE_TRI_LOADS = 0, 1, 2, 3, 5, 7
# ... 216 lines not shown
        ("depth_extent", C.c_int32 * 2),
        ("first_clipmap_width", C.c_float),
        ("clipmap_selection_bias", C.c_float),
        ("virtual_extent", C.c_float),
        ("dirty_mesh_instance_count", C.c_uint32),
        ("inv_projection_view", C.c_float * 16),
        ("resolution", C.c_float * 2),
        ("virtual_page_table", Buffer),
        ("vsm_clipmaps_buffer", Buffer),
        ("depth_attachment", Image),
        ("dirty_mesh_instance_indices", Buffer),
        ("mesh_instances_buffer", Buffer),
        ("meshes_buffer", Buffer),
        ("transforms_world_buffer", Buffer),
        ("transforms_previous_buffer", Buffer),
        ("vsm_clipmap_dirty_flags_buffer", Buffer),
        ("dirty_physical_pages_buffer", Buffer),
        ("clear_cmd_buffer", Buffer),
        ("counters_buffer", Buffer),
        ("hpb_attachment", ImageArrayU8),
        ("physical_page_image", Image),
    ]


class VsmDrawContext(C.Structure):
    _fields_ = [
        ("struct_size", C.c_uint32),
        ("wide_triangle_index", C.c_uint32),
        ("page_size", C.c_int32),
        ("page_table_size", C.c_int32),
        ("physical_page_table_size", C.c_int32),
        ("clipmap_count", C.c_int32),
        ("draw_geometry_cmd_buffer", Buffer),
        ("virtual_page_table", Buffer),
        ("vsm_clipmaps_buffer", Buffer),
        ("vsm_clipmap_dirty_flags_buffer", Buffer),
        ("physical_page_image", Image),
        ("draw_commands_buffer", Buffer),
        ("draw_count_buffer", Buffer),
        ("draw_clipmaps_buffer", Buffer),
    ]


class ShadowResolveContext(C.Structure):
    _fields_ = [
        ("struct_size", C.c_uint32),
        ("page_size", C.c_int32),
        ("page_table_size", C.c_int32),
        ("physical_page_table_size", C.c_int32),
        ("clipmap_count", C.c_int32),
        ("first_clipmap_width", C.c_float),
        ("clipmap_selection_bias", C.c_float),
        ("virtual_extent", C.c_float),
        ("z_length", C.c_float),
        ("directional_light_dir", C.c_float * 3),
        ("inv_projection_view", C.c_float * 16),
        ("resolution", C.c_float * 2),
        ("depth_attachment", Image),
        ("normal_attachment", Buffer),
        ("vsm_clipmaps_buffer", Buffer),
        ("virtual_page_table", Buffer),
        ("physical_page_image", Image),
        ("resolved_shadows_attachment", Image),
    ]


class ContactShadowsContext(C.Structure):
    _fields_ = [
        ("struct_size", C.c_uint32),
        ("inv_projection_view", C.c_float * 16),
        ("view", C.c_float * 16),
        ("projection", C.c_float * 16),
        ("near_clip", C.c_float),
        ("sun_dir", C.c_float * 3),
        ("steps", C.c_uint32),
        ("thickness", C.c_float),
        ("shadow_length", C.c_float),
        ("depth_attachment", Image),
        ("contact_shadows_attachment", Image),
    ]


class AmbientOcclusionContext(C.Structure):
    _fields_ = [
        ("struct_size", C.c_uint32),
        ("view", C.c_float * 16),
        ("projection", C.c_float * 16),
        ("resolution", C.c_float * 2),
        ("far_clip", C.c_float),
        ("thickness", C.c_float),
        ("slice_count", C.c_uint32),
        ("samples_per_slice_side", C.c_uint32),
        ("effect_radius", C.c_float),
        ("noise_index", C.c_uint32),
        ("final_power", C.c_float),
        ("depth_attachment", Image),
        ("normal_attachment", Buffer),
        ("hilbert_noise", Buffer),
        ("prefiltered_depth", Image),
        ("depth_differences", Buffer),
        ("noisy_occlusion", Buffer),
        ("ambient_occlusion_attachment", Buffer),
    ]


EXPORTS = [
    "oxc_abi_version",
    "oxc_create",
    "oxc_destroy",
    "oxc_last_error",
    "oxc_reserve",
    "oxc_generate_hiz",
    "oxc_cull_geometry",
    "oxc_cull_geometry_batch",
    "oxc_join_triangles",
    "oxc_seed_meshlet_instances",
    "oxc_read_counters",
    "oxc_stream_read_probe",
    "oxc_debug_decode_bounds",
    "oxc_debug_raster_stats",
    "oxc_profile_begin",
    "oxc_profile_end",
    "oxc_build_meshlet_bounds",
    "oxc_quantize_vertex_streams",
    "oxc_mesh_blob_layout_of",
    "oxc_mesh_blob_finalize",
    "oxc_mesh_build_create",
    "oxc_mesh_build_lod_count",
    "oxc_mesh_build_lod",
    "oxc_mesh_build_destroy",
    "oxc_mesh_vertex_fetch_remap",
    "oxc_generate_hpb",
    "oxc_update_virtual_shadowmap",
    "oxc_cull_terrain",
    "oxc_draw_visbuffer",
    "oxc_draw_physical_pages",
    "oxc_debug_vsm_draw_stats",
    "oxc_resolve_shadowmap",
    "oxc_debug_vsm_resolve_stats",
    "oxc_contact_shadows",
    "oxc_debug_contact_shadows_stats",
    "oxc_generate_ambient_occlusion",
    "oxc_debug_ambient_occlusion_stats",
    "oxc_comm_unique_id",
    "oxc_comm_init",
    "oxc_comm_destroy",
    "oxc_pack_counters",
    "oxc_pack_counters_batch",
    "oxc_exchange_counts",
    "oxc_broadcast_hiz",
    "oxc_broadcast_hiz_levels",
    "oxc_debug_read_u32",
    "oxc_debug_shared_tests_mode",
    "oxc_debug_tri_loads_mode",
    "oxc_debug_set_tuning",
    "oxc_debug_count_occlusion_candidates",
    "oxc_debug_project_aabb",
]


def build(force: bool = False) -> str:
    if force:
        subprocess.check_call(["make", "-C", CSRC_DIR, "clean"], stdout=subprocess.DEVNULL)
    subprocess.check_call(["make", "-C", CSRC_DIR], stdout=subprocess.DEVNULL)
    return LIB_PATH


_libs = {}


def load(path: str = None) -> C.CDLL:
    path = os.path.abspath(path or os.environ.get("OXC_LIB_PATH") or LIB_PATH)
    if path in _libs:
        return _libs[path]
    if not os.path.exists(path):
        raise RuntimeError(
            f"{path} is missing: build it with `python -c 'import __graft_entry__ as g; g.build()'` "
            "(there is no CPU fallback for the cull path)"
        )
    lib = C.CDLL(path)
    lib.oxc_abi_version.restype = C.c_uint32
    if lib.oxc_abi_version() != ABI_VERSION:
        raise RuntimeError(f"{path}: ABI version {lib.oxc_abi_version()} != {ABI_VERSION} (stale build: run __graft_entry__.build())")
    vp = C.c_void_p
    lib.oxc_abi_version.restype = C.c_uint32
    lib.oxc_create.argtypes = [C.c_int, C.POINTER(vp)]
    lib.oxc_destroy.argtypes = [vp]
    lib.oxc_destroy.restype = None
    lib.oxc_last_error.argtypes = [vp]
    lib.oxc_last_error.restype = C.c_char_p
    lib.oxc_reserve.argtypes = [vp, C.c_uint32, C.c_uint32]
    lib.oxc_generate_hiz.argtypes = [vp, C.POINTER(MainGeometryContext), vp]
    lib.oxc_cull_geometry.argtypes = [vp, C.POINTER(PreparedFrame), C.POINTER(CullGeometryContext), vp]
    lib.oxc_cull_geometry_batch.argtypes = [vp, C.c_uint32, C.POINTER(PreparedFrame), C.POINTER(CullGeometryContext), vp]
    lib.oxc_join_triangles.argtypes = [vp, vp]
    lib.oxc_seed_meshlet_instances.argtypes = [vp, C.POINTER(CullGeometryContext), C.c_uint32, vp]
    lib.oxc_read_counters.argtypes = [vp, C.POINTER(CullGeometryContext), C.POINTER(Counters), vp]
    lib.oxc_stream_read_probe.argtypes = [vp, vp, C.c_uint64, vp]
    lib.oxc_debug_decode_bounds.argtypes = [vp, vp, C.c_uint32, vp, vp]
    lib.oxc_profile_begin.argtypes = [vp]
    lib.oxc_profile_end.argtypes = [vp, C.POINTER(KernelTimes)]
    lib.oxc_build_meshlet_bounds.argtypes = [vp, C.POINTER(MeshletBoundsDesc), vp]
    lib.oxc_quantize_vertex_streams.argtypes = [vp, C.POINTER(VertexStreamsDesc), vp]
    lib.oxc_mesh_blob_layout_of.argtypes = [C.POINTER(MeshBlobDesc), C.POINTER(MeshBlobLayout)]
    lib.oxc_mesh_blob_finalize.argtypes = [C.POINTER(MeshBlobDesc), C.POINTER(MeshBlobLayout), C.c_uint64, vp, C.c_uint64, C.POINTER(C.c_float * 6), vp]
    lib.oxc_mesh_build_create.argtypes = [C.POINTER(MeshBuildDesc), C.POINTER(vp)]
    lib.oxc_mesh_build_lod_count.argtypes = [vp]
    lib.oxc_mesh_build_lod_count.restype = C.c_uint32
    lib.oxc_mesh_build_lod.argtypes = [vp, C.c_uint32, C.POINTER(MeshLodView)]
    lib.oxc_mesh_build_destroy.argtypes = [vp]
    lib.oxc_mesh_build_destroy.restype = None
    lib.oxc_mesh_vertex_fetch_remap.argtypes = [vp, C.c_uint64, C.c_uint32, vp, vp]
    lib.oxc_generate_hpb.argtypes = [vp, Buffer, C.POINTER(ImageArrayU8), vp]
    lib.oxc_update_virtual_shadowmap.argtypes = [vp, C.POINTER(VsmUpdateContext), vp]
    lib.oxc_cull_terrain.argtypes = [vp, C.POINTER(TerrainContext), vp]
    lib.oxc_debug_read_u32.argtypes = [vp, vp, C.c_uint32, vp, vp]
    lib.oxc_debug_shared_tests_mode.argtypes = [vp]
    lib.oxc_debug_shared_tests_mode.restype = C.c_uint32
    lib.oxc_debug_tri_loads_mode.argtypes = [vp]
    lib.oxc_debug_tri_loads_mode.restype = C.c_uint32
    lib.oxc_debug_raster_stats.argtypes = [vp, vp, vp]
    lib.oxc_debug_set_tuning.argtypes = [vp, C.c_uint32, C.c_uint32]
    lib.oxc_debug_count_occlusion_candidates.argtypes = [vp, vp]
    lib.oxc_comm_unique_id.argtypes = [vp, vp]
    lib.oxc_comm_init.argtypes = [vp, vp, C.c_uint32, C.c_uint32]
    lib.oxc_comm_destroy.argtypes = [vp]
    lib.oxc_pack_counters.argtypes = [vp, C.POINTER(CullGeometryContext), vp, vp]
    lib.oxc_pack_counters_batch.argtypes = [vp, C.c_uint32, C.POINTER(CullGeometryContext), vp, vp]
    lib.oxc_exchange_counts.argtypes = [vp, vp, vp, vp]
    lib.oxc_broadcast_hiz.argtypes = [vp, C.POINTER(Image), C.c_uint64, C.c_uint32, vp]
    lib.oxc_broadcast_hiz_levels.argtypes = [vp, C.POINTER(Image), C.c_uint32, C.c_uint64, C.c_uint32, vp]
    lib.oxc_debug_project_aabb.argtypes = [vp, C.POINTER(C.c_float), C.c_float, vp, C.c_uint32, vp, vp]
    lib.oxc_draw_visbuffer.argtypes = [vp, C.POINTER(PreparedFrame), C.POINTER(DrawContext), vp]
    lib.oxc_draw_physical_pages.argtypes = [vp, C.POINTER(PreparedFrame), C.POINTER(VsmDrawContext), vp]
    lib.oxc_debug_vsm_draw_stats.argtypes = [vp, vp, vp]
    lib.oxc_resolve_shadowmap.argtypes = [vp, C.POINTER(ShadowResolveContext), vp]
    lib.oxc_debug_vsm_resolve_stats.argtypes = [vp, vp, vp]
    lib.oxc_contact_shadows.argtypes = [vp, C.POINTER(ContactShadowsContext), vp]
    lib.oxc_debug_contact_shadows_stats.argtypes = [vp, vp, vp]
    lib.oxc_generate_ambient_occlusion.argtypes = [vp, C.POINTER(AmbientOcclusionContext), vp]
    lib.oxc_debug_ambient_occlusion_stats.argtypes = [vp, vp, vp]
    for name in EXPORTS:
        if name not in ("oxc_abi_version", "oxc_destroy", "oxc_last_error", "oxc_mesh_build_lod_count", "oxc_mesh_build_destroy"):
            getattr(lib, name).restype = C.c_int
    _libs[path] = lib
    return lib


class MeshBuildDesc(C.Structure):
    _fields_ = [("struct_size", C.c_uint32), ("vertex_count", C.c_uint32), ("index_count", C.c_uint32), ("max_lods", C.c_uint32), ("max_vertices", C.c_uint32),
                ("max_triangles", C.c_uint32), ("positions", C.c_void_p), ("normals", C.c_void_p), ("indices", C.c_void_p)]


class MeshLodView(C.Structure):
    _fields_ = [("indices", C.c_void_p), ("meshlets", C.c_void_p), ("indirect_vertex_indices", C.c_void_p), ("local_triangle_indices", C.c_void_p),
                ("indices_count", C.c_uint32), ("meshlet_count", C.c_uint32), ("indirect_vertex_indices_count", C.c_uint32),
                ("local_triangle_indices_count", C.c_uint32), ("error", C.c_float), ("_pad", C.c_uint32)]


class KernelTimes(C.Structure):
    _fields_ = [("total_ms", C.c_double * 16), ("launches", C.c_uint32 * 16), ("empty_pair_ms", C.c_double)]


KERNEL_NAMES = ["prepare_instances", "cull_meshes_scan", "cull_meshes_expand", "cull_meshlets_test", "cull_meshlets_emit",
                "cull_triangles_test", "cull_triangles_emit", "hiz", "cull_meshlets_test_late", "cull_meshlets_emit_late",
                "cull_triangles_test_late", "cull_triangles_emit_late", "draw_visbuffer", "build_meshlet_bounds",
                "multiview_setup", "vsm_update"]


class OxcError(RuntimeError):
    def __init__(self, status: int, msg: str):
        super().__init__(f"oxcull status {status}: {msg}")
        self.status = status
```

Baseline: 20.05 billion meshlets/s.

## Cache projected HiZ tap rectangles from early cull for late-pass reuse

During the early occlusion pass the shared-test kernel now projects each surviving meshlet AABB into a compact 12-byte HiZ tap record (max depth, mip, texel origin, extent codes) and writes it to a new per-lane buffer. When the late pass sees identical inputs and HiZ dimensions, a new RECTS kernel variant reads these records and only re-samples the rebuilt HiZ, skipping bounds loads, dequantization and the 8-corner projection. This adds global writes in the early pass and a buffer of N*12 bytes, and the early pass now computes the projection for all frustum survivors rather than only previously-visible ones.

```diff
diff --git a/include/oxcull_debug.h b/include/oxcull_debug.h
--- a/include/oxcull_debug.h
+++ b/include/oxcull_debug.h
@@ -42,6 +42,7 @@
 
 oxc_status oxc_debug_read_u32(oxc_ctx* ctx, const void* dptr, uint32_t n, uint32_t* host_out, void* hip_stream);
 uint32_t oxc_debug_shared_tests_mode(const oxc_ctx* ctx);
+uint32_t oxc_debug_shared_rects_mode(const oxc_ctx* ctx);
 uint32_t oxc_debug_tri_loads_mode(const oxc_ctx* ctx);
 
 enum { OXC_TUNE_ASYNC_MTEST_BLOCKS_PER_CU = 0, OXC_TUNE_ASYNC_TRI_BLOCKS_PER_CU = 1, OXC_TUNE_RASTER_BIG_CAPACITY = 2,
diff --git a/oxylus_amd/csrc/oxcull_abi.cpp b/oxylus_amd/csrc/oxcull_abi.cpp
--- a/oxylus_amd/csrc/oxcull_abi.cpp
+++ b/oxylus_amd/csrc/oxcull_abi.cpp
@@ -47,6 +47,7 @@
     uint32_t* m_tickets_late = nullptr;
     uint64_t* camera_test_bits = nullptr;
     uint2* step_info = nullptr;
+    uint32_t* rects = nullptr;
     uint64_t* tri_masks = nullptr;
     uint32_t* t_chunk_counts = nullptr;
     uint32_t* t_supers = nullptr;
@@ -112,6 +113,8 @@
     uint32_t* late_slot = nullptr;
     uint32_t* late_t_supers = nullptr;
     InstCache* rows = nullptr;
+    bool rects = false;
+    uint32_t hiz_w = 0, hiz_h = 0, hiz_levels = 0;
     bool same_inputs(const SharedTests& o) const {
       return N == o.N && n_host == o.n_host && M == o.M && flags == o.flags && mask_bits == o.mask_bits && meshlet_instances == o.meshlet_instances && mask == o.mask && meshes == o.meshes &&
              transforms == o.transforms && mesh_instances == o.mesh_instances && vis == o.vis && std::memcmp(&camera, &o.camera, sizeof camera) == 0;
@@ -119,6 +122,7 @@
   };
   SharedTests shared;
   uint32_t last_share_mode = 0;
+  uint32_t last_rects_mode = 0;
   uint32_t last_tri_loads = 0;
   uint64_t call_seq = 0;
   uint32_t async_mtest_per_cu = kAsyncMeshletBlocksPerCU, async_tri_per_cu = kAsyncTriangleBlocksPerCU;
@@ -220,6 +224,7 @@
   const uint64_t o_mtick_late = carve((uint64_t)kTicketCounters * 4 * kSuperStride);
   const uint64_t o_fb = carve((uint64_t)cdiv(N, 64) * 8);
   const uint64_t o_si = carve((uint64_t)m_chunks * 8);
+  const uint64_t o_rects = carve(lane_index == 0 ? (uint64_t)cdiv(N, kMeshletChunk) * kMeshletChunk * 12 : 0);
   const uint64_t o_tm = carve((uint64_t)N * 16);
   const uint64_t o_tcc = carve((uint64_t)t_chunks * 4);
   const uint64_t o_tsup = carve((uint64_t)cdiv(t_chunks, kChunksPerSuper) * 4 * kSuperStride);
@@ -250,6 +255,7 @@
   L->m_tickets_late = reinterpret_cast<uint32_t*>(b + o_mtick_late);
   L->camera_test_bits = reinterpret_cast<uint64_t*>(b + o_fb);
   L->step_info = reinterpret_cast<uint2*>(b + o_si);
+  L->rects = lane_index == 0 ? reinterpret_cast<uint32_t*>(b + o_rects) : nullptr;
   L->tri_masks = reinterpret_cast<uint64_t*>(b + o_tm);
   L->t_chunk_counts = reinterpret_cast<uint32_t*>(b + o_tcc);
   L->t_supers = reinterpret_cast<uint32_t*>(b + o_tsup);
@@ -525,6 +531,7 @@
   if (st != OXC_OK) return st;
   OXC_ORDER(ctx, hip_stream);
   ctx->last_share_mode = 0;
+  ctx->last_rects_mode = 0;
   ctx->last_tri_loads = 0;
   if (do_meshes) ctx->shared.valid = false;
 
@@ -570,6 +577,7 @@
   }
   uint32_t share_mode = 0;
   bool armed_late = false, arm_late = false;
+  bool share_rects = false;
   uint32_t* m_supers = L0.m_supers;
   uint32_t* m_tickets = L0.m_tickets;
   const uint32_t mask_bits = (uint32_t)std::min<uint64_t>(f->meshlet_instance_visibility_mask_buffer.bytes / 4u * 32u, 0xFFFFFFFEull);
@@ -593,6 +601,8 @@
       share_mode = 1u;
       arm_late = c->async_triangles == 0;
       now.valid = true;
+      now.rects = share_rects = c->hiz_attachment.width <= 65535u && c->hiz_attachment.height <= 65535u;
+      now.hiz_w = c->hiz_attachment.width, now.hiz_h = c->hiz_attachment.height, now.hiz_levels = c->hiz_attachment.levels;
       if (arm_late) {
         now.armed_for_call = call_no + 1;
         now.capture_id = stream_capture_id(s);
@@ -603,6 +613,8 @@
       ctx->shared = now;
     } else if (!do_meshes && !c->init_cull_meshes && ctx->shared.valid && ctx->shared.same_inputs(now)) {
       share_mode = 2u;
+      share_rects = ctx->shared.rects && ctx->shared.hiz_w == c->hiz_attachment.width && ctx->shared.hiz_h == c->hiz_attachment.height &&
+                    ctx->shared.hiz_levels == c->hiz_attachment.levels;
       if (ctx->shared.armed_for_call == call_no && c->async_triangles == 0 && ctx->shared.capture_id == stream_capture_id(s)) {
         armed_late = true;
         slot = ctx->shared.late_slot;
@@ -752,8 +764,10 @@
       ta.share = share_mode;
       ta.camera_test_bits = ctx->lane[0].camera_test_bits;
       ta.step_info = ctx->lane[0].step_info;
+      ta.rects = (share_rects && !(share_mode == 2u && ta.dbg_occlusion)) ? ctx->lane[0].rects : nullptr;
     }
     ctx->last_share_mode = armed_late ? 3u : ta.share;
+    ctx->last_rects_mode = ta.rects ? ta.share : 0u;
     if (unord_meshlets) {
       ta.out = static_cast<uint32_t*>(f->visible_meshlet_instances_indices_buffer.dptr);
       ta.count_a = tri_cmd;
@@ -2127,6 +2141,7 @@
 }
 
 uint32_t oxc_debug_shared_tests_mode(const oxc_ctx* ctx) { return ctx ? ctx->last_share_mode : 0u; }
+uint32_t oxc_debug_shared_rects_mode(const oxc_ctx* ctx) { return ctx ? ctx->last_rects_mode : 0u; }
 uint32_t oxc_debug_tri_loads_mode(const oxc_ctx* ctx) { return ctx ? ctx->last_tri_loads : 0u; }
 
 oxc_status oxc_debug_set_tuning(oxc_ctx* ctx, uint32_t knob, uint32_t value) {
diff --git a/oxylus_amd/csrc/oxcull_device.hpp b/oxylus_amd/csrc/oxcull_device.hpp
--- a/oxylus_amd/csrc/oxcull_device.hpp
+++ b/oxylus_amd/csrc/oxcull_device.hpp
@@ -260,7 +260,7 @@
   asm("v_max_f32 %0, 0, %1" : "=v"(r) : "v"(x));
   return r;
 }
-template <bool TRY_AFFINE = false, bool NEED_Z = true>
+template <bool TRY_AFFINE = false, bool NEED_Z = true, bool NEED_MINZ = true>
 OXC_DEV bool project_aabb(const float* mvp, float near_clip, float cx, float cy, float cz, float ex, float ey, float ez, float* out) {
   float SX[4], SY[4], SZ[4], P[8][4];
   float p0x = cx - ex * 0.5f, p0y = cy - ey * 0.5f, p0z = cz - ez * 0.5f;
@@ -351,7 +351,7 @@
         hi[0] = fmaxf(q.x, hi[0]);
         lo[1] = fminf(q.y, lo[1]);
         hi[1] = fmaxf(q.y, hi[1]);
-        lo[2] = fminf(z, lo[2]);
+        if (NEED_MINZ) lo[2] = fminf(z, lo[2]);
         hi[2] = fmaxf(z, hi[2]);
       }
     }
@@ -368,7 +368,7 @@
 #pragma unroll
       for (int k = 6; k >= 0; k--) {
         float d = P[k][j] / P[k][3];
-        lo = fminf(d, lo);
+        if (NEED_MINZ || j != 2) lo = fminf(d, lo);
         hi = fmaxf(d, hi);
       }
       vmin[j] = lo;
@@ -384,12 +384,15 @@
   return true;
 }
 
-OXC_DEV bool aabb_occluded(const float* mvp, float near_clip, float cx, float cy, float cz, float ex, float ey, float ez,
-                           const HizView& hiz, const uint32_t* level_off, bool active) {
+struct HizTaps {
+  float maxz;
+  uint32_t mip;
+  int32_t x0, y0, x1, y1;
+};
+OXC_DEV bool aabb_project_rect(const float* mvp, float near_clip, float cx, float cy, float cz, float ex, float ey, float ez, const HizView& hiz, HizTaps& r) {
   float sa[6];
-  if (!active) return false;
-  if (!project_aabb(mvp, near_clip, cx, cy, cz, ex, ey, ez, sa)) return false;
-  const float minu = sa[0], minv = sa[1], maxu = sa[3], maxv = sa[4], maxz = sa[5];
+  if (!project_aabb<false, true, false>(mvp, near_clip, cx, cy, cz, ex, ey, ez, sa)) return false;
+  const float minu = sa[0], minv = sa[1], maxu = sa[3], maxv = sa[4];
 
   float sw = (float)hiz.width, sh = (float)hiz.height;
   uint32_t minx = cvt_u32_sat(fmaxf(minu * sw, 0.0f));
@@ -410,8 +413,15 @@
   int32_t bx = cvt_i32_sat(floorf(u * (float)mw - 0.5f));
   int32_t by = cvt_i32_sat(floorf(v * (float)mh - 0.5f));
   int32_t bx1 = (int32_t)((uint32_t)bx + 1u), by1 = (int32_t)((uint32_t)by + 1u);
-  int32_t x0 = min(max(bx, 0), mxx), y0 = min(max(by, 0), mxy);
-  int32_t x1 = min(max(bx1, 0), mxx), y1 = min(max(by1, 0), mxy);
+  r.maxz = sa[5];
+  r.mip = mip;
+  r.x0 = min(max(bx, 0), mxx), r.y0 = min(max(by, 0), mxy);
+  r.x1 = min(max(bx1, 0), mxx), r.y1 = min(max(by1, 0), mxy);
+  return true;
+}
+OXC_DEV bool rect_occluded(const HizTaps& r, const HizView& hiz, const uint32_t* level_off) {
+  const uint32_t mip = r.mip, mw = mip_dim(hiz.width, mip);
+  const int32_t x0 = r.x0, y0 = r.y0, x1 = r.x1, y1 = r.y1;
   float p00, p10, p01, p11;
   if (mip >= hiz.lds_first) {
     const float* lvl = hiz.lds + hiz.lds_off[mip];
@@ -427,7 +437,36 @@
     p11 = lvl[(size_t)y1 * mw + x1];
   }
   float d = fminf(fminf(p00, p10), fminf(p01, p11));
-  return maxz <= d - 1e-7f;
+  return r.maxz <= d - 1e-7f;
+}
+OXC_DEV bool aabb_occluded(const float* mvp, float near_clip, float cx, float cy, float cz, float ex, float ey, float ez,
+                           const HizView& hiz, const uint32_t* level_off, bool active) {
+  HizTaps r;
+  if (!active) return false;
+  if (!aabb_project_rect(mvp, near_clip, cx, cy, cz, ex, ey, ez, hiz, r)) return false;
+  return rect_occluded(r, hiz, level_off);
+}
+
+struct RectEntry {
+  uint32_t w[3];
+};
+OXC_DEV RectEntry pack_rect(bool some, const HizTaps& r) {
+  RectEntry e;
+  const uint32_t cx = r.x1 == r.x0 ? 0u : (r.x1 > r.x0 ? 1u : 2u), cy = r.y1 == r.y0 ? 0u : (r.y1 > r.y0 ? 1u : 2u);
+  e.w[0] = some ? asu(r.maxz) : 0x7FC00000u;
+  e.w[1] = some ? ((uint32_t)r.x0 | ((uint32_t)r.y0 << 16)) : 0u;
+  e.w[2] = some ? (r.mip | (cx << 8) | (cy << 10)) : 0u;
+  return e;
+}
+OXC_DEV HizTaps unpack_rect(const RectEntry& e) {
+  HizTaps r;
+  r.maxz = asf(e.w[0]);
+  r.mip = e.w[2] & 0xFFu;
+  r.x0 = (int32_t)(e.w[1] & 0xFFFFu), r.y0 = (int32_t)(e.w[1] >> 16);
+  const uint32_t cx = (e.w[2] >> 8) & 3u, cy = (e.w[2] >> 10) & 3u;
+  r.x1 = (cx & 2u) ? 0 : r.x0 + (int32_t)cx;
+  r.y1 = (cy & 2u) ? 0 : r.y0 + (int32_t)cy;
+  return r;
 }
 
 struct HpbView {
diff --git a/oxylus_amd/csrc/oxcull_kernels.hip b/oxylus_amd/csrc/oxcull_kernels.hip
--- a/oxylus_amd/csrc/oxcull_kernels.hip
+++ b/oxylus_amd/csrc/oxcull_kernels.hip
@@ -534,13 +534,14 @@
 template <bool OCCL, bool LATE, int G, int SHARE = 0, bool COUNT = false>
 OXC_DEV void meshlets_hiz_body(const MeshletTestArgs& a) {
   static_assert(SHARE == 0 || (OCCL && G == 4 && (SHARE == 1) == !LATE), "sharing: early call writes, late call reads");
+  constexpr bool RECTS = SHARE == 3;
   set_half_denorm_flush();
   constexpr int kWaves = 16 / G;
   constexpr bool OCCL_OR_LATE = OCCL || LATE;
   __shared__ uint32_t s_level_off[13];
   __shared__ uint32_t s_lds_off[13];
   __shared__ float s_hiz_top[kHizLdsTexels];
-  __shared__ uint4 s_strip[OCCL_OR_LATE ? kWaves : 1][G * 64];
+  __shared__ uint4 s_strip[(OCCL_OR_LATE && !RECTS) ? kWaves : 1][(OCCL_OR_LATE && !RECTS) ? G * 64 : 1];
   __shared__ uint32_t s_flags[OCCL_OR_LATE ? kWaves : 1][G * 64];
   const int lane = threadIdx.x & 63, wave = threadIdx.x >> 6;
   const uint32_t N = a.n_host ? a.n_host : min(gptr(a.vis)[0], a.n_cap);
@@ -590,7 +591,7 @@
     uint32_t fbit[G];
 #pragma unroll
     for (int j = 0; j < G; j++) fbit[j] = 0u;
-    if constexpr (SHARE == 2) {
+    if constexpr (SHARE >= 2) {
       uint64_t any = 0;
 #pragma unroll
       for (int j = 0; j < G; j++) {
@@ -621,6 +622,8 @@
         mask_idx[j] = 0;
       }
     }
+    uint32_t rect_off = 0;
+    const size_t rect_base = (size_t)step * (64u * G);
     for (;;) {
       uint32_t mi_u = 0;
       bool found = false;
@@ -643,7 +646,10 @@
       for (int j = 0; j < G; j++) {
         mine[j] = (st[j] & 1u) != 0u && rec[j].x == mi_u;
         const bool fetch = SHARE == 2 ? (mine[j] && (st[j] & 8u) != 0u) : mine[j];
-        bnd[j] = OXC_LOAD_BND(bounds, fetch ? rec[j].y : 0u);
+        if constexpr (RECTS)
+          bnd[j] = make_uint4(0u, 0u, 0u, 0u);
+        else
+          bnd[j] = OXC_LOAD_BND(bounds, fetch ? rec[j].y : 0u);
         mword[j] = 0xFFFFFFFFu;
         if (OCCL) {
           uint32_t mi_bit = vis_offset + (mine[j] ? rec[j].y : 0u);
@@ -667,7 +673,7 @@
         for (int j = 0; j < G; j++) {
           const uint4 b = bnd[j];
           const bool was_visible = (mword[j] & 1u) != 0u;
-          if constexpr (SHARE == 2) {
+          if constexpr (SHARE >= 2) {
             const bool vis = mine[j] & ((st[j] & 8u) != 0u);
             cx[j] = cy[j] = cz[j] = ex[j] = ey[j] = ez[j] = 0.0f;
             need[j] = 0u;
@@ -707,6 +713,7 @@
 #pragma unroll
           for (int j = 0; j < G; j++) {
             slot[j] = base[j] + __builtin_amdgcn_mbcnt_hi((uint32_t)(vb[j] >> 32), __builtin_amdgcn_mbcnt_lo((uint32_t)vb[j], 0u));
+            if constexpr (RECTS) continue;
             if ((vb[j] >> lane) & 1ull) {
               if constexpr (SHARE == 2) {
                 strip[slot[j]] = make_uint4(bnd[j].x, bnd[j].y, bnd[j].z, (bnd[j].w & 0x00FFFFFFu) | (slot[j] << 24));
@@ -718,8 +725,9 @@
             }
           }
           asm volatile("s_waitcnt lgkmcnt(0)" ::: "memory");
-          uint32_t nb = SHARE == 2 ? total : 0u;
-          if constexpr (SHARE != 2) {
+          uint32_t nb = SHARE >= 2 ? total : 0u;
+          uint32_t nbv = 0;
+          if constexpr (SHARE < 2) {
           ConeU cu;
 #pragma unroll
           for (int k = 0; k < 9; k++) cu.nm[k] = asf(row[kRowNm + k]);
@@ -750,18 +758,33 @@
               ok = nc ? cone_ok : ok;
             }
             const bool okv = SHARE == 1 ? (ok && (flg[act ? t : 0u] & 4u) != 0u) : ok;
-            const uint64_t okb = __builtin_amdgcn_ballot_w64(okv);
+            const uint64_t okb = __builtin_amdgcn_ballot_w64(ok);
             const uint32_t rank = __builtin_amdgcn_mbcnt_hi((uint32_t)(okb >> 32), __builtin_amdgcn_mbcnt_lo((uint32_t)okb, 0u));
             if (act) flg[t] = SHARE == 1 ? ((ok ? 1u : 0u) | (okv ? 2u : 0u)) : (ok ? 1u : 0u);
-            if (okv) strip[nb + rank] = make_uint4(b.x, b.y, b.z, (b.w & 0x00FFFFFFu) | (t << 24));
+            if (ok) strip[nb + rank] = make_uint4(b.x, b.y, b.z, (b.w & 0x00FFFFFFu) | (t << 24));
             nb += (uint32_t)__popcll((unsigned long long)okb);
+            if constexpr (SHARE == 1) nbv += (uint32_t)__popcll((unsigned long long)__builtin_amdgcn_ballot_w64(okv));
           }
           }
           asm volatile("s_waitcnt lgkmcnt(0)" ::: "memory");
           if constexpr (COUNT) {
-            if (nb && lane == 0) __hip_atomic_fetch_add(gptr(a.dbg_occlusion) + (step & 255u) * kSuperStride, nb, __ATOMIC_RELAXED, __HIP_MEMORY_SCOPE_AGENT);
+            const uint32_t tested = SHARE == 1 ? nbv : nb;
+            if (tested && lane == 0) __hip_atomic_fetch_add(gptr(a.dbg_occlusion) + (step & 255u) * kSuperStride, tested, __ATOMIC_RELAXED, __HIP_MEMORY_SCOPE_AGENT);
           }
-          if (nb) {
+          if constexpr (RECTS) {
+            const uint32_t __attribute__((address_space(1)))* const rects = gptr(a.rects) + (rect_base + rect_off) * 3u;
+            for (uint32_t u0 = 0; u0 < nb; u0 += 64) {
+              const uint32_t u = u0 + (uint32_t)lane;
+              const bool act = u < nb;
+              const uint32_t at = (act ? u : nb - 1u) * 3u;
+              RectEntry e;
+              e.w[0] = rects[at], e.w[1] = rects[at + 1u], e.w[2] = rects[at + 2u];
+              const bool occluded = rect_occluded(unpack_rect(e), hiz, s_level_off);
+              if (act) flg[u] = occluded ? 0u : 1u;
+            }
+            asm volatile("s_waitcnt lgkmcnt(0)" ::: "memory");
+            rect_off += nb;
+          } else if (nb) {
             float mvp[16];
 #pragma unroll
             for (int k = 0; k < 16; k++) mvp[k] = asf(row[kRowMvp + k]);
@@ -771,10 +794,25 @@
               const uint4 b = strip[act ? u : nb - 1u];
               const float qx = dequantize_half(b.x & 0xFFFFu), qy = dequantize_half(b.x >> 16), qz = dequantize_half(b.y & 0xFFFFu);
               const float rx = dequantize_half(b.z & 0xFFFFu), ry = dequantize_half(b.z >> 16), rz = dequantize_half(b.w & 0xFFFFu);
-              const bool occluded = aabb_occluded(mvp, a.near_clip, qx, qy, qz, rx, ry, rz, hiz, s_level_off, act);
-              if (act && occluded) flg[b.w >> 24] = SHARE == 1 ? 1u : 0u;
+              if constexpr (SHARE == 1) {
+                HizTaps r = {0.0f, 0u, 0, 0, 0, 0};
+                const bool some = aabb_project_rect(mvp, a.near_clip, qx, qy, qz, rx, ry, rz, hiz, r);
+                if (a.rects) {
+                  const RectEntry e = pack_rect(some, r);
+                  uint32_t __attribute__((address_space(1)))* const out = gptr(a.rects) + (rect_base + rect_off + u) * 3u;
+                  if (act) out[0] = e.w[0], out[1] = e.w[1], out[2] = e.w[2];
+                }
+                const uint32_t pos = b.w >> 24;
+                bool occluded = false;
+                if (act && some && (flg[pos] & 2u) != 0u) occluded = rect_occluded(r, hiz, s_level_off);
+                if (occluded) flg[pos] = 1u;
+              } else {
+                const bool occluded = aabb_occluded(mvp, a.near_clip, qx, qy, qz, rx, ry, rz, hiz, s_level_off, act);
+                if (act && occluded) flg[b.w >> 24] = 0u;
+              }
             }
             asm volatile("s_waitcnt lgkmcnt(0)" ::: "memory");
+            if constexpr (SHARE == 1) rect_off += nb;
           }
 #pragma unroll
           for (int j = 0; j < G; j++) {
@@ -1665,9 +1703,10 @@
     meshlets_hiz_body<OCCL, LATE, G>(a);
 }
 __global__ __launch_bounds__(64 * kUnordBlockWaves) void k_cull_meshlets_test_unordered(MeshletTestArgs a) { meshlets_plain_body<(int)kGroupsPerWave, true, kUnordBlockWaves>(a); }
-template <bool LATE>
-__global__ __launch_bounds__(1024 / kHizGroupsPerWave, 5) void k_cull_meshlets_test_shared(MeshletTestArgs a) {
-  meshlets_hiz_body<true, LATE, (int)kHizGroupsPerWave, LATE ? 2 : 1>(a);
+constexpr int kHizRectsWaves = 8;
+template <bool LATE, bool RECTS = false>
+__global__ __launch_bounds__(1024 / kHizGroupsPerWave, RECTS ? kHizRectsWaves : 5) void k_cull_meshlets_test_shared(MeshletTestArgs a) {
+  meshlets_hiz_body<true, LATE, (int)kHizGroupsPerWave, LATE ? (RECTS ? 3 : 2) : 1>(a);
 }
 template <bool LATE, int SHARE>
 __global__ __launch_bounds__(1024 / kHizGroupsPerWave, 4) void k_cull_meshlets_test_counting(MeshletTestArgs a) {
@@ -2119,7 +2158,10 @@
   if (!hiz) {
     hipLaunchKernelGGL((k_cull_meshlets_test<false, false, false>), dim3(grid * (4 / kPlainBlockWaves)), dim3(64 * kPlainBlockWaves), 0, s, a);
   } else if (occl && a.share) {
-    if (a.share == 2) {
+    if (a.share == 2 && a.rects) {
+      static const uint32_t cap = resident_grid(k_cull_meshlets_test_shared<true, true>, hb, num_cus);
+      hipLaunchKernelGGL((k_cull_meshlets_test_shared<true, true>), dim3(std::min(grid, cap)), dim3(hb), 0, s, a);
+    } else if (a.share == 2) {
       static const uint32_t cap = resident_grid(k_cull_meshlets_test_shared<true>, hb, num_cus);
       hipLaunchKernelGGL((k_cull_meshlets_test_shared<true>), dim3(std::min(grid, cap)), dim3(hb), 0, s, a);
     } else {
diff --git a/oxylus_amd/csrc/oxcull_kernels.hpp b/oxylus_amd/csrc/oxcull_kernels.hpp
--- a/oxylus_amd/csrc/oxcull_kernels.hpp
+++ b/oxylus_amd/csrc/oxcull_kernels.hpp
@@ -73,6 +73,7 @@
   uint32_t* dbg_occlusion;
   uint64_t* camera_test_bits;
   uint2* step_info;
+  uint32_t* rects;
   const float* hiz_data;
   uint32_t hiz_level_off[13];
   uint32_t hiz_w, hiz_h, hiz_levels;
diff --git a/oxylus_amd/lib.py b/oxylus_amd/lib.py
--- a/oxylus_amd/lib.py
+++ b/oxylus_amd/lib.py
@@ -392,6 +392,7 @@
     "oxc_broadcast_hiz_levels",
     "oxc_debug_read_u32",
     "oxc_debug_shared_tests_mode",
+    "oxc_debug_shared_rects_mode",
     "oxc_debug_tri_loads_mode",
     "oxc_debug_set_tuning",
     "oxc_debug_count_occlusion_candidates",
@@ -457,6 +458,8 @@
     lib.oxc_debug_read_u32.argtypes = [vp, vp, C.c_uint32, vp, vp]
     lib.oxc_debug_shared_tests_mode.argtypes = [vp]
     lib.oxc_debug_shared_tests_mode.restype = C.c_uint32
+    lib.oxc_debug_shared_rects_mode.argtypes = [vp]
+    lib.oxc_debug_shared_rects_mode.restype = C.c_uint32
     lib.oxc_debug_tri_loads_mode.argtypes = [vp]
     lib.oxc_debug_tri_loads_mode.restype = C.c_uint32
     lib.oxc_debug_raster_stats.argtypes = [vp, vp, vp]
```

Measured after the change: 19.98 billion meshlets/s. No clear change (-0.4%).
